# google-deepmind/meltingpot

Measured on AMD Instinct MI355X. Metric: agent-steps/sec (env_batch x players / wall s), clean_up @4096 worlds, higher is better.
Workload: dtype u8

## Files before the change

include/mp_engine.h:

```cpp
#ifndef MP_ENGINE_H_
#define MP_ENGINE_H_

#include <stdint.h>

#ifdef __cplusplus
extern "C" {
#endif
#pragma GCC visibility push(default)

#define MP_ABI_VERSION 8

enum {
  MP_OK = 0,
  MP_ERR_INVALID = -1,
  MP_ERR_PACK = -2,
  MP_ERR_NO_DEVICE = -3,
  MP_ERR_HIP = -4,
  MP_ERR_UNSUPPORTED = -5
};

typedef enum {
  MP_EVENT_ZAP = 1,
  MP_EVENT_EDIBLE_CONSUMED = 2,
  MP_EVENT_PLAYER_CLEANED = 3,
  MP_EVENT_CLAIMED_RESOURCE = 4,
  MP_EVENT_DESTROYED_RESOURCE = 5,
  MP_EVENT_SANCTIONING = 6,
  MP_EVENT_REMOVAL_DUE_TO_SANCTIONING = 7,
  MP_EVENT_SET_SANCTIONING_LEVEL = 8,
  MP_EVENT_AVATAR_STARTED = 9,
  MP_EVENT_COIN_CONSUMED = 10,
  MP_EVENT_INTERACTION = 11,
  MP_EVENT_COLLECTED_RESOURCE = 12,
  MP_EVENT_MINING = 13,
  MP_EVENT_EXTRACTION = 14,
  MP_EVENT_EXTRACTION_PAIR = 15,
  MP_EVENT_RECEIVER_ACCEPTED_ITEM = 17,
  MP_EVENT_ITEM_DROPPED_INTO_POT = 18,
  MP_EVENT_COOKED_FOOD_COLLECTED = 19,
  MP_EVENT_EATING_MUSHROOM = 20,
  MP_EVENT_GIFT = 16
} MpEventType;
#define MP_EVENT_ROWS 128

typedef enum {
  MP_OBS_RGB = 0,
  MP_OBS_WORLD_RGB = 1,
  MP_OBS_REWARD = 2,
  MP_OBS_READY_TO_SHOOT = 3,
  MP_OBS_AUX0 = 4,
  MP_OBS_STEP_TYPE = 5,
  MP_OBS_DISCOUNT = 6,
  MP_OBS_COLLECTIVE_REWARD = 7,
  MP_OBS_POSITION = 8,
  MP_OBS_ORIENTATION = 9,
  MP_OBS_EVENTS = 10,
  MP_OBS_AUX1 = 11,
  MP_OBS_AUX2 = 12,
  MP_OBS_AUX3 = 13,
  MP_OBS_AUX4 = 14,
  MP_OBS_ZAP_MATRIX = 15,
  MP_OBS_LAYER = 16,
  MP_OBS_INVENTORY = 17,
  MP_OBS_INTERACTION_INVENTORIES = 18,
  MP_OBS_MATRIX_CUMULANTS = 19,
  MP_OBS_INTERACTION_REWARDS = 20,
  MP_OBS_RGB_POOL2 = 21,
  MP_OBS_RGB_POOL4 = 22,
  MP_OBS_RGB_POOL8 = 23,
  MP_OBS_KINDS = 24
} MpObsKind;

typedef struct MpEngine MpEngine;

typedef struct {
  uint32_t struct_size;
  int32_t batch_worlds;
  int32_t waves;
  int32_t feeders;
  int32_t max_groups;
  int32_t scratch_cells;
  int32_t no_composite_cache;
  int32_t max_composites;
  int32_t verbose;
  int32_t late_feeder_prio;
  int32_t ring_batches;
  int32_t static_pct;
  int32_t world_waves;
  int32_t store_sc1;
  int32_t head;
  int32_t no_next_orders;
  int32_t record_pad;
  int32_t pace;
  int32_t team;
  int32_t generic_kernel;
} MpDevOptions;

typedef struct {
  uint32_t struct_size;
  int32_t device;
  int32_t num_worlds;
  int32_t auto_reset;
  uint64_t world_offset;
  uint64_t base_seed;
  void* stream;
  int32_t num_players;
  int32_t debug_observations;
  int32_t unfused;
  int32_t literal_base_seed;
  const MpDevOptions* dev;
  const int32_t* roles;
  int32_t world_pool;
} MpConfig;

typedef struct {
  int32_t abi_version;
  int32_t substrate;
  int32_t num_worlds, num_players, num_actions;
  int32_t map_h, map_w, num_layers, sprite_size;
  int32_t view_h, view_w;
  int32_t max_frames;
  int32_t world_state_bytes;
  int32_t fused;
  int32_t num_resources;
  int32_t num_action_fields;
  int32_t plan_batch_worlds, plan_ring_batches, plan_owned_batches, plan_pooled_batches,
          plan_groups, plan_store_sc1 ;
  int32_t plan_feeders, plan_waves;
  int32_t ring_slots, ring_next;
  int32_t plan_pace, visible_layers;
  int32_t plan_team, plan_late_priority;
  int64_t retired_va_bytes, retired_va_limit;
} MpInfo;

int mp_abi_version(void);

const char* mp_last_error(void);

int mp_create(const void* pack, uint64_t pack_len, const MpConfig* cfg,
              MpEngine** out);

void mp_destroy(MpEngine* eng);

int mp_info(const MpEngine* eng, MpInfo* out);

enum { MP_KERNEL_GENERIC = 0, MP_KERNEL_STOCK = 1 };
typedef struct {
  uint32_t struct_size;
  int32_t variant;
  const void* pack;
  uint64_t pack_len;
  const MpConfig* cfg;
  char* fields;
  uint64_t fields_cap;
} MpKernelVariant;

int mp_set_stream(MpEngine* eng, void* stream);

int mp_bind_output(MpEngine* eng, MpObsKind kind, void* device_ptr);

int mp_bind_output_ring(MpEngine* eng, MpObsKind kind, void* base,
                        uint64_t slot_stride_bytes, int32_t slots);

int mp_reset(MpEngine* eng, const uint64_t* seeds, const uint8_t* mask);

int mp_step(MpEngine* eng, const int32_t* actions_device);

int mp_step_host(MpEngine* eng, const int32_t* actions_host);

int mp_step_fields(MpEngine* eng, const int32_t* fields_device);

int mp_step_fields_host(MpEngine* eng, const int32_t* fields_host);

int mp_observe(MpEngine* eng, MpObsKind kind, void* dst_device);

uint64_t mp_obs_bytes(const MpEngine* eng, MpObsKind kind);

int mp_dump(MpEngine* eng, uint8_t* grid, int32_t* avat, int32_t* glob);

uint64_t mp_snapshot_bytes(const MpEngine* eng);
int mp_snapshot(MpEngine* eng, void* host_buf, uint64_t bytes);
int mp_restore(MpEngine* eng, const void* host_buf, uint64_t bytes);

enum { MP_STATES_FINGERPRINT = 1, MP_STATES_SAVE = 2, MP_STATES_LOAD = 3 };
typedef struct {
  uint32_t struct_size;
  int32_t op;
  uint64_t fingerprint;
  const int32_t* worlds;
  const int32_t* src;
  void* bank;
  uint64_t bank_bytes;
  int32_t count;
  int32_t bank_rows;
} MpWorldStates;

typedef struct {
  uint32_t struct_size;
  int32_t kind;
  uint64_t fingerprint;
  const void* bank;
  const int32_t* rows;
  void* dst;
  uint64_t dst_bytes;
  int32_t bank_rows;
  int32_t count;
  uint64_t reserved;
} MpStatesObserve;

typedef struct {
  char name[16];
  int32_t offset;
  int32_t elem_bytes;
  int32_t count;
  int32_t reserved;
} MpStateField;
typedef struct {
  uint32_t struct_size;
  uint32_t layout_version;
  const void* pack;
  uint64_t pack_len;
  const MpConfig* cfg;
  int32_t map_h, map_w, num_layers, num_players, num_states;
  int32_t grid_planes, grid_bytes, grid_pad, world_stride, tail_bytes;
  int32_t max_frames, avatar_layer, substrate, player_block;
  int32_t reserved[2];
  uint64_t fingerprint;
  MpStateField* fields;
  int32_t fields_cap;
  int32_t num_fields;
} MpStateLayout;

enum { MP_CHECK_ROWS = 1, MP_CHECK_HOST = 2, MP_CHECK_FILTER = 3 };
typedef struct {
  uint32_t struct_size;
  int32_t op;
  uint64_t fingerprint;
  const void* pack;
  uint64_t pack_len;
  const MpConfig* cfg;
  const void* bank;
  int32_t bank_rows;
  int32_t count;
  const int32_t* rows;
  void* out;
  uint64_t out_bytes;
  uint64_t reserved;
} MpStatesCheck;
// ... 77 lines not shown
```

meltingpot_amd/csrc/frame_kernel.h:

```cpp
#pragma once
#include <stdlib.h>
#include <string.h>

#include <type_traits>

#include "../../include/mp_pack.h"
#include "step_clean_up.h"
#include "step_coins.h"
#include "step_commons.h"
#include "step_coop.h"
#include "step_gift.h"
#include "step_mushroom.h"
#include "step_cook.h"
#include "step_matrix.h"
#include "step_territory.h"
#include "step_load.h"

template <bool kStep> constexpr bool nt_stores() { return kStep; }

namespace {

constexpr int kMaxLayers = 12;
constexpr int kSpriteStride = 272;
constexpr int kHeadBytes = 64;
// ... 560 lines not shown
          dst[ch] = (uint8_t)((sum[ch] + (uint32_t)(kPool * kPool / 2)) / (uint32_t)(kPool * kPool));
      }
      if (!arrive_and_wait(&ctrl->blob_waves, 2u * (uint32_t)n_render_waves)) return;
    } else if constexpr (kWPool != 0) {
      auto pool_atlas = [&](auto kp_tag, uint8_t* ptab) {
        constexpr int kP = decltype(kp_tag)::value;
        constexpr int kN = 8 / kP, kQ = kN * kN;
        const int items = t.n_images * kQ;
        for (int i = tid; i < items; i += n_render_waves * 64) {
          const int img = i / kQ, q = i - img * kQ, qy = q / kN, qx = q - qy * kN;
          const uint8_t* src = atlas + img * kSpriteStride + qy * kP * 32 + qx * kP * 3;
          uint32_t sum[3] = {0u, 0u, 0u};
#pragma unroll
          for (int y = 0; y < kP; ++y)
#pragma unroll
            for (int x = 0; x < kP * 3; ++x) sum[x % 3] += src[y * 32 + x];
          uint8_t* dst = ptab + img * pool_img_bytes(kP) + q * 3;
#pragma unroll
          for (int ch = 0; ch < 3; ++ch)
            dst[ch] = (uint8_t)((sum[ch] + (uint32_t)(kP * kP / 2)) / (uint32_t)(kP * kP));
        }
      };
      uint8_t* ptab = smem + lo.scratch + (uint32_t)kWaves * (uint32_t)pool_scratch_bytes<kPool, kWPool>(t);
      if constexpr (kPool != 0) pool_atlas(std::integral_constant<int, kPool>(), ptab);
      if constexpr (kWPool != 0 && kWPool != kPool)
        pool_atlas(std::integral_constant<int, kWPool>(), ptab + (kPool ? pool_tab_bytes(t, kPool) : 0));
      if (!arrive_and_wait(&ctrl->blob_waves, 2u * (uint32_t)n_render_waves)) return;
    }
  }
  FRAME_STAGE(3, npb);

  auto batch_first_world = [&](int k, bool& stalled) -> int {
    if (k < ks) {
      const int w0 = w_first + k * kstep;
      return w0 < w_end ? w0 : -1;
    }
    const int ring = k % kClaimRing, chain = k % A;
    uint64_t wait_t0 = 0;
    for (uint32_t polls = 0;; ++polls) {
      if (lds_acquire(&ctrl->claim_tag[ring]) == (uint32_t)(k + 1)) {
        const uint32_t w0 = ctrl->claim_w[ring];
        return w0 == kNoBatch ? -1 : (int)w0;
      }
      if (lds_acquire(&ctrl->chain_end[chain]) <= (uint32_t)k) return -1;
      if (waited_too_long(polls, wait_t0)) {
        report_stall(t, lane, FAULT_CLAIM, (uint32_t)wave, (uint32_t)k,
                     lds_acquire(&ctrl->claim_tag[ring]), (uint32_t)(k + 1));
        stalled = true;
        return -1;
      }
      __builtin_amdgcn_s_sleep(1);
    }
  };
  auto all_chains_ended = [&](int k) -> bool {
    uint32_t last = 0;
    for (int ch = 0; ch < A; ++ch) {
      const uint32_t e = lds_acquire(&ctrl->chain_end[ch]);
      last = e > last ? e : last;
    }
    return last <= (uint32_t)k;
  };

  const int role_wave = wave;
  if (role_wave >= kWaves - F) {
    const int f = wave - (kWaves - F);
    struct { int32_t B, NB, F, ks, N, nbt, A, pool_first, b_mod_f, wstride, pool, parity,
                     late_prio, records, step_tables, recs, w_first, kstep, w_end;
             uint32_t npb_all; } fc = {
        B, NB, F, ks, N, nbt, A, pool_first, kc.b_mod_f, wstride, plan.pool, plan.parity,
        plan.late_prio, lo.records, lo.step_tables, lo.recs, w_first, kstep, w_end, npb_all};
    pin_scalars(fc);
    auto batch_first_world = [&](int k, bool& stalled) -> int {
      if (k < fc.ks) {
        const int w0 = fc.w_first + k * fc.kstep;
        return w0 < fc.w_end ? w0 : -1;
      }
      const int ring = k % kClaimRing, chain = k % fc.A;
      uint64_t wait_t0 = 0;
      for (uint32_t polls = 0;; ++polls) {
        if (lds_acquire(&ctrl->claim_tag[ring]) == (uint32_t)(k + 1)) {
          const uint32_t w0 = ctrl->claim_w[ring];
          return w0 == kNoBatch ? -1 : (int)w0;
        }
        if (lds_acquire(&ctrl->chain_end[chain]) <= (uint32_t)k) return -1;
        if (waited_too_long(polls, wait_t0)) {
          report_stall(t, lane, FAULT_CLAIM, (uint32_t)wave, (uint32_t)k,
                       lds_acquire(&ctrl->claim_tag[ring]), (uint32_t)(k + 1));
          stalled = true;
          return -1;
        }
        __builtin_amdgcn_s_sleep(1);
      }
    };
    auto all_chains_ended = [&](int k) -> bool {
      uint32_t last = 0;
      for (int ch = 0; ch < fc.A; ++ch) {
        const uint32_t e = lds_acquire(&ctrl->chain_end[ch]);
        last = e > last ? e : last;
      }
      return last <= (uint32_t)k;
    };
    __builtin_amdgcn_s_setprio(3);
    uint8_t* my_scratch = smem + lo.step_scratch + f * plan.slot_scratch;
    FRAME_STAGE(10, 0);
    bool first_world = true;
    int kb = 0, gen = 0, r0 = 0, m = 0;
    auto next_batch = [&]() {
      ++kb; r0 += fc.B; m += fc.b_mod_f;
      if (m >= fc.F) m -= fc.F;
      if (kb == fc.NB) { kb = 0; r0 = 0; m = 0; ++gen; }
    };
    for (int k = 0;; ++k, next_batch()) {
      const int mine = f >= m ? f - m : f - m + fc.F;
      if (mine >= fc.B) continue;
      FRAME_STAGE(4, k);
      bool stalled = false;
      const int w0 = batch_first_world(k, stalled);
      if (stalled) return;
      if (w0 < 0) {
        if (all_chains_ended(k)) break;
        __builtin_amdgcn_s_sleep(8);
        continue;
      }
      int nw = fc.N - w0;
      if (nw > fc.B) nw = fc.B;
      uint64_t wait_t0 = 0;
      for (uint32_t polls = 0;
           gen > 0 && lds_acquire(&ctrl->done[kb]) < (uint32_t)gen * fc.npb_all; ++polls) {
        if (waited_too_long(polls, wait_t0)) {
          report_stall(t, lane, FAULT_BUFFER_FREE, (uint32_t)wave, (uint32_t)k,
                       lds_acquire(&ctrl->done[kb]), (uint32_t)gen * fc.npb_all);
          return;
        }
        __builtin_amdgcn_s_sleep(2);
      }
      for (int sl = mine; sl < fc.B; sl += fc.F) {
        FRAME_STAGE(5, sl);
        const bool claims = sl == 0 && k + fc.A >= fc.ks && fc.pool > 0;
        uint32_t claimed = 0;
        if (claims && lane == 0)
          claimed = __hip_atomic_fetch_add(&t.claim[fc.parity], 1u, __ATOMIC_RELAXED,
                                           __HIP_MEMORY_SCOPE_AGENT);
        const int w = w0 + sl;
        if (sl < nw) {
          uint8_t* rec = smem + fc.records + (r0 + sl) * fc.wstride;
          if constexpr (kStep) {
            int lane_w = lane;
            asm volatile("" : "+v"(lane_w));
            stepk::World wd = stepk::make_world(t, rec, smem + fc.step_tables, my_scratch,
                                                args.state, w, lane_w);
            wd.publish = &ctrl->slot_batch[r0 + sl];
            wd.publish_value = (uint32_t)(k + 1);
            wd.next_orders = args.next_orders;
            bool have_rec = false;
            if (head_pending) {
              head_pending = false;
              dma_wait();
              have_rec = w == pre_w && r0 + sl == pre_slot;
              if (!arrive_and_wait(&ctrl->table_waves, (uint32_t)fc.F)) return;
              FRAME_STAGE(11, sl);
            }
            int act_id;
            if (have_rec && args.mode == STEP_MODE_STEP)
              act_id = lane_w < P ? reinterpret_cast<const int*>(smem + fc.recs + wave * 64 * 16)[lane_w] : 0;
            else
              act_id = stepk::fetch_action_id(t, args.actions, args.mode, w, lane_w);
            if (!have_rec) stepk::load_record(t, rec, wd.gw, lane_w);
            FRAME_STAGE(12, sl);
            if (claims) {
              if (lane == 0) {
                const uint32_t id = (uint32_t)fc.pool_first + claimed;
                const int kn = k + fc.A, ring = kn % kClaimRing;
                const bool have = id < (uint32_t)fc.nbt;
                ctrl->claim_w[ring] = have ? id * (uint32_t)fc.B : kNoBatch;
                if (!have)
                  __hip_atomic_store(&ctrl->chain_end[kn % fc.A], (uint32_t)kn, __ATOMIC_RELEASE,
                                     __HIP_MEMORY_SCOPE_WORKGROUP);
                __hip_atomic_store(&ctrl->claim_tag[ring], (uint32_t)(kn + 1), __ATOMIC_RELEASE,
                                   __HIP_MEMORY_SCOPE_WORKGROUP);
              }
            }
            stepk::begin_step(wd.sc, lane_w);
            stepk::wsync();
            const stepk::Action act = stepk::lookup_action(t, wd, act_id, args.mode);
            stepk::step_or_load(t, c, sites, wd, act, args);
            if (args.out.layer) {
              stepk::wsync();
              stepk::write_layer(t, rec, args.out, w, lane_w);
            }
          } else {
            stepk::load_record(t, rec, args.state + (size_t)w * fc.wstride, lane);
          }
        }
        if (claims && (!kStep || sl >= nw)) {
          if (lane == 0) {
            const uint32_t id = (uint32_t)fc.pool_first + claimed;
            const int kn = k + fc.A, ring = kn % kClaimRing;
            const bool have = id < (uint32_t)fc.nbt;
            ctrl->claim_w[ring] = have ? id * (uint32_t)fc.B : kNoBatch;
            if (!have)
              __hip_atomic_store(&ctrl->chain_end[kn % fc.A], (uint32_t)kn, __ATOMIC_RELEASE,
                                 __HIP_MEMORY_SCOPE_WORKGROUP);
            __hip_atomic_store(&ctrl->claim_tag[ring], (uint32_t)(kn + 1), __ATOMIC_RELEASE,
                               __HIP_MEMORY_SCOPE_WORKGROUP);
          }
        }
        __builtin_amdgcn_fence(__ATOMIC_RELEASE, "workgroup");
        if (lane == 0)
          __hip_atomic_store(&ctrl->slot_batch[r0 + sl], (uint32_t)(k + 1), __ATOMIC_RELEASE,
                             __HIP_MEMORY_SCOPE_WORKGROUP);
        FRAME_STAGE(6, sl);
        if (first_world) {
          first_world = false;
          switch (fc.late_prio) {
            case 0: __builtin_amdgcn_s_setprio(0); break;
            case 1: __builtin_amdgcn_s_setprio(1); break;
            case 2: __builtin_amdgcn_s_setprio(2); break;
            default: break;
          }
        }
      }
    }
    FRAME_STAGE(15, 0);
    return;
  }

  uint8_t* __restrict__ out = wv ? out_w : out_a;
  CellRec* recs = reinterpret_cast<CellRec*>(smem + lo.recs) + wave * 64;
  uint8_t* ovlist = smem + lo.ovlist + wave * 64;
  int nsprites = t.nsprites;
  asm volatile("" : "+s"(nsprites));
  const uint32_t magic_rows = kv.magic_rows;
  const uint32_t magic_p = kc.magic_p;
  const uint32_t magic_spw = kv.magic_spw;
  const int py = lane & 7, sub = lane >> 3;
  uint8_t* atlas_row = atlas + py * 32;
  const uint32_t scratch_off =
      (kPool || kWPool) ? (uint32_t)(lo.scratch - lo.atlas) + (uint32_t)(wave * pool_scratch_bytes<kPool, kWPool>(t))
            : (uint32_t)(lo.scratch - lo.atlas) + (uint32_t)(wave * t.scratch_cells) * 256u;
  constexpr int kPN = kPool ? 8 / kPool : 1;
  constexpr int kWPN = kWPool ? 8 / kWPool : 1;
  const uint32_t vpn = (kWPool != 0 && wv) ? (uint32_t)kWPN : (uint32_t)kPN;
  const uint32_t prow = (uint32_t)row_cells * (vpn * 3u), pstrip = prow * vpn;
  const uint32_t my_poff = (uint32_t)sr * pstrip + cx * (vpn * 3u);
  const uint8_t* ptab = smem + lo.scratch + (uint32_t)kWaves * (uint32_t)pool_scratch_bytes<kPool, kWPool>(t) +
                        ((kWPool != 0 && wv && kWPool != kPool && kPool != 0) ? (uint32_t)pool_tab_bytes(t, kPool) : 0u);

  const uint32_t span_bytes = (uint32_t)R * 8u * row_bytes;
  const int n_iters = (int)((span_bytes + 1023u) >> 10);
  const int n_full = (int)(span_bytes >> 10);
  uint32_t keys[12];
#pragma unroll
  for (int it = 0; it < 12; ++it) {
    uint32_t kk = 0;
#pragma unroll
    for (int h = 0; h < 2; ++h) {
      const uint32_t pp = (uint32_t)(it * 64 + lane) * 16u + 8u * h;
      uint32_t key = 63u << 8;
      if (pp < span_bytes) {
        const uint32_t row = fast_div(pp, row_bytes, 1.0f / (float)row_bytes);
        const uint32_t colb = pp - row * row_bytes;
        const uint32_t ccx = fast_div(colb, 24u, 1.0f / 24.0f);
        key = (((row >> 3) * (uint32_t)row_cells + ccx) << 8) | ((row & 7u) * 32u + (colb - ccx * 24u));
      }
      kk |= key << (16 * h);
    }
    keys[it] = kk;
  }


  auto render_pass = [&](const uint32_t s0, const uint32_t nstrips, const uint8_t* wlds,
                         uint8_t* out_block) {
    uint8_t* const g0 = (kPool || kWPool) ? out_block + (size_t)s0 * pstrip : nullptr;
    uint8_t* const pst = (kPool || kWPool) ? atlas + scratch_off + ((uint32_t)(uintptr_t)g0 & 15u) : nullptr;
    int n_partial, n_ov;
    {
      const uint32_t strip = s0 + sr;
      const bool live = sr < R && strip < nstrips;
      const uint32_t sidx = live ? strip : 0u;
      const uint32_t img = magic_div(sidx, magic_rows);
      const uint32_t cy = sidx - img * strip_rows;
      uint32_t lw = img, viewer = P, vo = 0;
      if (!wv) {
        lw = magic_div(img, magic_p);
        viewer = img - lw * P;
      }
      const uint8_t* grid = wlds + lw * wstride;
      const uint8_t* head = grid + t.grid_pad;
      int cell;
      uint32_t oob_img = 0;
      if (wv) {
        cell = (int)(cy * W + cx);
      } else {
        const uint32_t alive = head[48 + viewer], ori = head[32 + viewer];
        const int hx = head[viewer], hy = head[16 + viewer];
        oob_img = oobimg[viewer];
        const bool on_grid = alive != 0u;
        vo = on_grid ? ori : 0u;
        const int dx = (int)cx - t.vl, dy = (int)cy - t.vf;
        const int ax = vo == 0u ? dx : vo == 1u ? -dy : vo == 2u ? -dx : dy;
        const int ay = vo == 0u ? dy : vo == 1u ? dx : vo == 2u ? -dy : -dx;
        int x = hx + ax, y = hy + ay;
        bool inside;
        if (t.topology == 1) {
          x += x < 0 ? W : 0; x -= x >= W ? W : 0;
          y += y < 0 ? H : 0; y -= y >= H ? H : 0;
          inside = true;
        } else {
          inside = x >= 0 && x < W && y >= 0 && y < H;
        }
        cell = on_grid && inside ? y * W + x : -1;
      }
      const uint16_t* rinfo_v = rinfo + viewer * (uint32_t)nsprites;
      CellRec r;
      r.base = 0; r.ov0 = 0; r.ov1 = 0; r.ov2 = 0;
      uint32_t base_img = 0;
      bool done = !live || cell < 0;
      if (cell == -1) base_img = oob_img;
      const uint16_t* tf = stab + (((0u - vo) & 3u) << 8);
      const uint8_t* gp = grid + (cell >= 0 ? cell : 0);
      uint32_t base_e = base_img;
      auto resolve = [&](auto nv_tag) {
        constexpr int NV = decltype(nv_tag)::value;
        uint32_t offs[6] = {kv.plane_off[0], kv.plane_off[1], kv.plane_off[2],
                            kv.plane_off[3], kv.plane_off[4], kv.plane_off[5]};
        uint32_t avp = kv.av_planes;
#pragma unroll
        for (int i = 0; i < (NV + 1) / 2; ++i) asm volatile("" : "+s"(offs[i]));
        asm volatile("" : "+s"(avp));
        uint32_t ent[NV];
        uint32_t seen = 0;
#pragma unroll
        for (int k = 0; k < NV; ++k) ent[k] = gp[(offs[k >> 1] >> (16 * (k & 1))) & 0xffffu];
#pragma unroll
        for (int k = 0; k < NV; ++k) { ent[k] = tf[ent[k]]; seen |= ent[k]; }
// ... 480 lines not shown
```

meltingpot_amd/csrc/mp_engine.hip:

```cpp
#include <chrono>
#include <map>
#include <mutex>
#include "../../include/mp_engine.h"

#include <stdarg.h>
#include <stddef.h>
#include <sys/types.h>
#include <stdio.h>
#include <string.h>

#include <algorithm>
#include <string>
#include <vector>

#include "pack_decode.h"
#include "stock.h"
#include "step_common.h"
#include "step_many.h"
#include "state_obs.h"
#include "state_check.h"

void launch_step(const DevTables& t, const SubstrateTables& s, const stepk::StepArgs& args,
                 hipStream_t stream);
int prepare_step();
void launch_layer_view(const DevTables& t, const uint8_t* state, int32_t* out, int num_worlds,
                       hipStream_t stream);

constexpr int kFaultWords = 64 + 4 * 16 * 64 * 2;
FramePlan plan_frame(const DevTables& t, const SubstrateTables& s, int num_worlds,
                     bool with_step, int views, int num_cus, const MpDevOptions* dev,
                     int pool_k = 1,
                     int world_k = 1);
int frame_lds_bytes(const DevTables& t, const FramePlan& p, int pool_k = 1, int world_k = 1,
                    int views = 2);
int render_blob_bytes(const DevTables& t);
int prepare_frame();
void build_render_blob(const DevTables& t, const uint8_t* images, const uint16_t* img_slot,
                       const uint32_t* pair_table, const int32_t* state_sprite,
                       const int8_t* state_player, const int32_t* view_sprite_map,
                       const uint8_t* sprite_flags8, const int32_t* state_orient,
                       uint8_t* blob);
uint32_t render_visible_layers(const DevTables& t, const uint8_t* blob, const int32_t* state_layer);
void launch_frame(const DevTables& t, const SubstrateTables* s, const stepk::StepArgs& args,
                  uint8_t* out_a, uint8_t* out_w, const FramePlan& p, hipStream_t stream,
                  int pool_k = 1, int world_k = 1);

thread_local std::string g_error;

int fail(int code, const char* fmt, ...) {
  char buf[512];
  va_list ap;
  va_start(ap, fmt);
  vsnprintf(buf, sizeof buf, fmt, ap);
  va_end(ap);
  g_error = buf;
  return code;
}

#define HIP_TRY(expr)                                                       \
  do {                                                                      \
    hipError_t e_ = (expr);                                                 \
    if (e_ != hipSuccess)                                                   \
      return fail(MP_ERR_HIP, "%s failed: %s", #expr, hipGetErrorString(e_)); \
  } while (0)

struct MpEngine {
  int device = 0;
  int N = 0;
  int auto_reset = 0;
  hipStream_t stream = nullptr;
  int substrate = 0;
  DevTables t{};
  SubstrateTables sub{};
  int inventory_types() const {
    return substrate == MPK_SUBSTRATE_THE_MATRIX ? sub.mx.R
           : substrate == MPK_SUBSTRATE_GIFT_REFINEMENTS ? sub.gr.ntypes : 0;
  }
  std::vector<uint8_t> pack;
  uint8_t* d_pack = nullptr;
  uint8_t* d_extra = nullptr;
  uint8_t* d_stepblob = nullptr;
  uint8_t* d_debug = nullptr;
  uint32_t* h_fault = nullptr;
  uint8_t* d_state = nullptr;
  uint8_t* d_scalars = nullptr;
  size_t scalars_bytes = 0, debug_bytes = 0;
  StepOutputs own{};
  void* bound[MP_OBS_KINDS] = {};
  struct RingKind { uint8_t* base = nullptr; uint64_t stride = 0; };
  RingKind ring[MP_OBS_KINDS];
  int ring_slots = 0;
  uint64_t ring_cursor = 0;
  bool ring_hold = false;
  bool layer_hold = false;
  std::vector<FramePlan> ring_plan[3];
  void point_ring(int slot, bool pixels_only = false) {
    for (int k = 0; k < MP_OBS_KINDS; ++k)
      if (ring[k].base && (!pixels_only || is_pixel_kind(k)))
        bound[k] = ring[k].base + (uint64_t)slot * ring[k].stride;
  }
  bool ring_has_pixels() const {
    for (int k = 0; k < MP_OBS_KINDS; ++k)
      if (ring[k].base && is_pixel_kind(k)) return true;
    return false;
  }
  static int pool_of(int kind) {
    return kind == MP_OBS_RGB_POOL2 ? 2 : kind == MP_OBS_RGB_POOL4 ? 4 : kind == MP_OBS_RGB_POOL8 ? 8 : 1;
  }
  static bool is_pixel_kind(int kind) {
    return kind == MP_OBS_RGB || kind == MP_OBS_WORLD_RGB || pool_of(kind) > 1;
  }
  int agent_kind() const {
    for (int k : {MP_OBS_RGB_POOL2, MP_OBS_RGB_POOL4, MP_OBS_RGB_POOL8})
      if (bound[k]) return k;
    return MP_OBS_RGB;
  }
  uint8_t* agent_view() const { return (uint8_t*)bound[agent_kind()]; }
  int pool_k() const { return pool_of(agent_kind()); }
  int world_pool = 1;
  FramePlan pool_plan[3][2][3] = {};
  bool pool_ok[3] = {};
  static int pool_index(int k) { return k == 2 ? 0 : k == 4 ? 1 : 2; }
  FramePlan& frame_plan(int stepping, int views, int k) {
    return k > 1 ? pool_plan[pool_index(k)][stepping][views] : plan[stepping][views];
  }
  int32_t* d_actions = nullptr;
  int32_t* d_fields = nullptr;
  uint8_t* d_mask = nullptr;
  uint64_t* d_seeds = nullptr;
  unsigned long long* d_ctr = nullptr;
  static constexpr int kHostSlots = 4;
  int32_t* h_actions[kHostSlots] = {};
  hipEvent_t h_copied[kHostSlots] = {};
  uint64_t host_steps = 0;
  FramePlan plan[2][3] = {};
  int frame_launches = 0;
  uint32_t* d_claim = nullptr;
  int num_cus = 0;
  int next_orders = 1;
  bool has_dev = false;
  bool touched = false;
  bool has_state = false;
  uint64_t fingerprint = 0;
  int unfused = 0;
  bool fuse(bool world_view) const {
    (void)world_view;
    return unfused != 1;
  }
  uint8_t* d_atlas = nullptr;
  uint8_t* d_obs_rows = nullptr;
  uint64_t obs_rows_bytes = 0;
  uint8_t* d_obs_stash = nullptr;
  uint64_t obs_stash_bytes = 0;
  int32_t* d_layer_lut = nullptr;
  state_check::CheckTables check = {};
  state_check::CheckTables* d_check = nullptr;
  StepOutputs outputs() const {
    StepOutputs o = own;
    if (bound[MP_OBS_REWARD]) o.reward = (double*)bound[MP_OBS_REWARD];
    if (bound[MP_OBS_READY_TO_SHOOT]) o.ready = (double*)bound[MP_OBS_READY_TO_SHOOT];
    if (bound[MP_OBS_AUX0]) o.aux0 = (double*)bound[MP_OBS_AUX0];
    if (bound[MP_OBS_STEP_TYPE]) o.step_type = (int32_t*)bound[MP_OBS_STEP_TYPE];
    if (bound[MP_OBS_DISCOUNT]) o.discount = (double*)bound[MP_OBS_DISCOUNT];
    if (bound[MP_OBS_COLLECTIVE_REWARD]) o.collective = (double*)bound[MP_OBS_COLLECTIVE_REWARD];
    if (bound[MP_OBS_POSITION]) o.position = (int32_t*)bound[MP_OBS_POSITION];
    if (bound[MP_OBS_ORIENTATION]) o.orientation = (int32_t*)bound[MP_OBS_ORIENTATION];
    if (bound[MP_OBS_EVENTS]) o.events = (int32_t*)bound[MP_OBS_EVENTS];
    for (int k = 0; k < 4; ++k)
      if (bound[MP_OBS_AUX1 + k]) o.dbg[k] = (double*)bound[MP_OBS_AUX1 + k];
    if (bound[MP_OBS_ZAP_MATRIX]) o.zap_matrix = (double*)bound[MP_OBS_ZAP_MATRIX];
    if (bound[MP_OBS_INVENTORY]) o.inventory = (double*)bound[MP_OBS_INVENTORY];
    if (bound[MP_OBS_INTERACTION_INVENTORIES])
      o.interaction = (double*)bound[MP_OBS_INTERACTION_INVENTORIES];
    if (bound[MP_OBS_MATRIX_CUMULANTS]) o.cumulants = (double*)bound[MP_OBS_MATRIX_CUMULANTS];
    if (bound[MP_OBS_INTERACTION_REWARDS])
      o.interaction_rewards = (double*)bound[MP_OBS_INTERACTION_REWARDS];
    if (bound[MP_OBS_LAYER] && !layer_hold) { o.layer = (int32_t*)bound[MP_OBS_LAYER]; o.layer_lut = d_layer_lut; }
    return o;
  }
};

namespace {

__global__ __launch_bounds__(1024) void k_box_fill(uint8_t* out, uint64_t bytes, uint64_t own,
                                                   uint32_t span, int order) {
  __shared__ uint32_t next;
  if (threadIdx.x == 0) next = 0;
  __syncthreads();
  const uint32_t lane = threadIdx.x & 63u;
  const uint64_t g = blockIdx.x, G = gridDim.x;
  typedef uint32_t u32x4 __attribute__((ext_vector_type(4)));
  for (;;) {
    uint32_t t = 0;
    if (lane == 0) t = atomicAdd(&next, 1u);
    t = (uint32_t)__builtin_amdgcn_readfirstlane((int)t);
    uint64_t begin, end;
    if (order == 0) {
      uint64_t lim = (g + 1) * own;
      if (lim > bytes) lim = bytes;
      begin = g * own + (uint64_t)t * span;
      if (begin >= lim) break;
      end = begin + span < lim ? begin + span : lim;
    } else {
      begin = ((uint64_t)t * G + g) * span;
      if (begin >= bytes) break;
      end = begin + span < bytes ? begin + span : bytes;
    }
    const uint64_t sp = reinterpret_cast<uint64_t>(out + begin);
    uint8_t* base = reinterpret_cast<uint8_t*>(
        ((uint64_t)(uint32_t)__builtin_amdgcn_readfirstlane((uint32_t)(sp >> 32)) << 32) |
        (uint64_t)(uint32_t)__builtin_amdgcn_readfirstlane((uint32_t)sp));
    const uint32_t n = (uint32_t)(end - begin);
    for (uint32_t off = lane * 16u; off < n; off += 1024u)
      asm volatile("global_store_dwordx4 %0, %1, %2 nt" :: "v"(off), "v"(u32x4{t, off, 2u, 3u}), "s"(base));
  }
}

__global__ void k_probe_actions(int32_t* actions, int n, int nact, uint32_t salt) {
  const int i = blockIdx.x * blockDim.x + threadIdx.x;
  if (i >= n) return;
  uint32_t x = (uint32_t)i * 2654435761u + salt;
  x ^= x >> 16; x *= 0x7feb352du; x ^= x >> 15; x *= 0x846ca68bu; x ^= x >> 16;
  actions[i] = (int32_t)(x % (uint32_t)nact);
}

__global__ void k_set_seeds(uint8_t* state, int stride, int grid_pad, int n,
                            const uint64_t* seeds, const uint8_t* mask) {
  const int w = blockIdx.x * blockDim.x + threadIdx.x;
  if (w >= n || (mask && !mask[w])) return;
  WorldTail* tail = reinterpret_cast<WorldTail*>(state + (size_t)w * stride + grid_pad);
  tail->seed = seeds[w];
  tail->episode = 0;
  tail->orders_step = 0;
}

__global__ void k_sum_counters(const uint8_t* state, int stride, int grid_pad, int n,
                               unsigned long long* out) {
  unsigned long long acc[MP_CTR_COUNT];
  for (int k = 0; k < MP_CTR_COUNT; ++k) acc[k] = 0;
  for (int w = blockIdx.x * blockDim.x + threadIdx.x; w < n; w += gridDim.x * blockDim.x) {
    const WorldTail* tail = reinterpret_cast<const WorldTail*>(state + (size_t)w * stride + grid_pad);
    for (int k = 0; k < MP_CTR_COUNT; ++k) acc[k] += tail->ctr[k];
    acc[MP_CTR_REWARD_SUM] += (unsigned long long)(long long)tail->reward_fx;
  }
  for (int k = 0; k < MP_CTR_COUNT; ++k) {
    for (int off = 32; off > 0; off >>= 1) acc[k] += __shfl_xor(acc[k], off);
    if ((threadIdx.x & 63) == 0 && acc[k]) atomicAdd(&out[k], acc[k]);
  }
}

__global__ __launch_bounds__(256) void k_save_worlds(DevTables t, const uint8_t* __restrict__ state, int n,
                                                     const int32_t* __restrict__ worlds, int count,
                                                     uint8_t* __restrict__ dst) {
  const int lane = threadIdx.x & 63;
  const int row = blockIdx.x * 4 + __builtin_amdgcn_readfirstlane((int)threadIdx.x >> 6);
  if (row >= count) return;
  const int w = worlds ? __builtin_amdgcn_readfirstlane(worlds[row]) : row;
  if (w < 0 || w >= n) {
    if (lane == 0) {
      t.fault[FAULT_STATE_INDEX + 1] = (uint32_t)w;
      t.fault[FAULT_STATE_INDEX + 2] = 2u;
      t.fault[FAULT_STATE_INDEX] = (uint32_t)row + 1u;
    }
    return;
  }
  const int nvec = t.world_stride >> 4;
  const uint4* src = reinterpret_cast<const uint4*>(state + (size_t)w * t.world_stride);
  uint4* out = reinterpret_cast<uint4*>(dst + (size_t)row * t.world_stride);
  for (int i0 = 0; i0 < nvec; i0 += 8 * 64) {
    uint4 v[8];
#pragma unroll
    for (int k = 0; k < 8; ++k) {
      const int i = i0 + k * 64 + lane;
      v[k] = src[i < nvec ? i : nvec - 1];
    }
#pragma unroll
    for (int k = 0; k < 8; ++k) stepk::issued(v[k]);
#pragma unroll
    for (int k = 0; k < 8; ++k) {
      const int i = i0 + k * 64 + lane;
      if (i < nvec) out[i] = v[k];
    }
  }
}

int sync_and_check(MpEngine* e, const char* who) {
  HIP_TRY(hipStreamSynchronize(e->stream));
  const volatile uint32_t* f = e->h_fault;
  if (f[0] != 0)
    return fail(MP_ERR_HIP,
                "%s: the frame kernel's pipeline stalled (site %u, workgroup %u, wave %u, batch %u, "
                "seen %u, wanted %u); its outputs are incomplete",
                who, f[0], f[1], f[2], f[3], f[4], f[5]);
  if (f[8] != 0) {
    const uint32_t world = f[8] - 1;
    e->h_fault[8] = 0;
    return fail(MP_ERR_HIP,
                "%s: world %u paid an interaction reward outside every resultIndicatorColorInterval "
                "(the reference asserts there, the_matrix/components.lua:282-290); the indicator "
                "shows the first colour", who, world);
  }
  if (f[kFaultCheckWorld] != 0) {
    const uint32_t world = f[kFaultCheckWorld] - 1, row = f[kFaultCheckWorld + 1], rule = f[kFaultCheckWorld + 2],
                   offset_word = f[kFaultCheckWorld + 3];
    e->h_fault[kFaultCheckWorld] = 0;
    if ((f[FAULT_STATE_INDEX + 2] & 255u) == kFaultCheckRefused) e->h_fault[FAULT_STATE_INDEX] = 0;
    return fail(MP_ERR_INVALID,
                "%s: checked MP_STATES_LOAD: row %d, which src[%u] names, is not a well-formed record "
                "(rule %u, offset word 0x%x); world %u was left as it was", who, (int)row, world, rule,
                offset_word, world);
  }
  if (f[FAULT_STATE_INDEX] != 0) {
    const uint32_t at = f[FAULT_STATE_INDEX] - 1, index = f[FAULT_STATE_INDEX + 1];
    const bool load = f[FAULT_STATE_INDEX + 2] == 1;
    const bool observe = f[FAULT_STATE_INDEX + 2] == kFaultObserveRow;
    const uint32_t what = f[FAULT_STATE_INDEX + 2];
    e->h_fault[FAULT_STATE_INDEX] = 0;
    if (what == kFaultCheckRow)
      return fail(MP_ERR_INVALID,
                  "%s: MpStatesCheck: rows[%u] = %d is not a row of the bank; element %u of out is (-1, %d)",
                  who, at, (int)index, at, (int)index);
    if (observe)
      return fail(MP_ERR_INVALID,
                  "%s: MpStatesObserve: rows[%u] = %d is not a row of the bank; element %u of the "
                  "destination was left as it was", who, at, (int)index, at);
    return load ? fail(MP_ERR_INVALID,
                       "%s: MP_STATES_LOAD: src[%u] = %d is neither -1 nor a row of the bank; world %u "
                       "was left as it was", who, at, (int)index, at)
                : fail(MP_ERR_INVALID,
                       "%s: MP_STATES_SAVE: worlds[%u] = %d is not a world of this engine; row %u was "
                       "left as it was", who, at, (int)index, at);
  }
  return MP_OK;
}

void draw(MpEngine* e, uint8_t* rgb, uint8_t* wrgb, int pool_k = 1) {
  stepk::StepArgs args = {};
  args.state = e->d_state; args.num_worlds = e->N;
  FramePlan p = e->frame_plan(0, rgb && wrgb ? 2 : wrgb ? 1 : 0, rgb ? pool_k : 1);
  p.parity = e->frame_launches++ & 1;
  launch_frame(e->t, nullptr, args, rgb, wrgb, p, e->stream, rgb ? pool_k : 1, e->world_pool);
}

int submit(MpEngine* e, int mode, const int32_t* actions, const uint8_t* mask,
           const uint8_t* bank = nullptr, const int32_t* src = nullptr, int bank_rows = 0,
           const StepManyLaunch* many = nullptr) {
  stepk::StepArgs args;
  args.state = e->d_state; args.actions = actions; args.reset_mask = mask;
  args.bank = bank; args.src = src; args.bank_rows = bank_rows;
  args.mode = mode; args.auto_reset = e->auto_reset; args.num_worlds = e->N;
  args.next_orders = e->next_orders;
  const bool ringing = e->ring_slots > 0 && !e->ring_hold;
  const int slot = e->ring_slots > 0 ? (int)(e->ring_cursor % (uint64_t)e->ring_slots) : 0;
  if (ringing) { e->point_ring(slot); ++e->ring_cursor; }
  args.out = e->outputs();
  uint8_t* rgb = e->agent_view();
  uint8_t* wrgb = (uint8_t*)e->bound[MP_OBS_WORLD_RGB];
  const int pk = rgb ? e->pool_k() : 1;
  const int views = rgb && wrgb ? 2 : wrgb ? 1 : 0;
  if (many || (!rgb && !wrgb) || !e->fuse(rgb == nullptr)) {
    if (many)
      launch_step_many(e->t, e->sub, args, *many, e->stream);
    else
      launch_step(e->t, e->sub, args, e->stream);
    if (rgb) draw(e, rgb, nullptr, pk);
    if (wrgb) draw(e, nullptr, wrgb);
  } else {
    FramePlan p = ringing && e->ring_plan[views].size() == (size_t)e->ring_slots
                      ? e->ring_plan[views][(size_t)slot] : e->frame_plan(1, views, pk);
    p.parity = e->frame_launches++ & 1;
    launch_frame(e->t, &e->sub, args, rgb, wrgb, p, e->stream, pk, e->world_pool);
  }
  HIP_TRY(hipGetLastError());
  return MP_OK;
}

void retired_va(int64_t* bytes, int64_t* limit);
bool in_mapped_view(const void* p);

int check_bank(MpEngine* e, const void* ptr, uint64_t bytes, const char* who);

int check_device_pointer(MpEngine* e, const void* ptr, const char* who) {
  if (in_mapped_view(ptr)) return MP_OK;
  hipPointerAttribute_t attr = {};
  const hipError_t rc = hipPointerGetAttributes(&attr, ptr);
  if (rc != hipSuccess) {
    (void)hipGetLastError();
    hipDeviceptr_t base = nullptr;
    size_t size = 0;
    if (hipMemGetAddressRange(&base, &size, (hipDeviceptr_t)ptr) == hipSuccess && base && size) return MP_OK;
    (void)hipGetLastError();
    return fail(MP_ERR_INVALID, "%s: %p is not memory the device can write (%s); bind a device buffer",
                who, ptr, hipGetErrorString(rc));
  }
  if (attr.type == hipMemoryTypeUnregistered)
    return fail(MP_ERR_INVALID, "%s: %p is plain host memory; bind a device buffer", who, ptr);
  if ((attr.type == hipMemoryTypeDevice || attr.type == hipMemoryTypeArray) && attr.device != e->device)
    return fail(MP_ERR_INVALID, "%s: %p lives on device %d, the engine on device %d", who, ptr,
                attr.device, e->device);
  return MP_OK;
}

int check_bank(MpEngine* e, const void* ptr, uint64_t bytes, const char* who) {
  if (int rc = check_device_pointer(e, ptr, who)) return rc;
  if (in_mapped_view(ptr)) {
    if (!in_mapped_view((const char*)ptr + bytes - 1))
      return fail(MP_ERR_INVALID, "%s: [%p, +%llu bytes) leaves the mapped view it starts in", who, ptr,
                  (unsigned long long)bytes);
    return MP_OK;
  }
  hipPointerAttribute_t attr = {};
  const hipError_t rc = hipPointerGetAttributes(&attr, ptr);
  (void)hipGetLastError();
  if (rc == hipSuccess && attr.type == hipMemoryTypeHost)
    return fail(MP_ERR_INVALID, "%s: %p is host memory; world states live in device memory", who, ptr);
  hipDeviceptr_t base = nullptr;
  size_t size = 0;
  if (hipMemGetAddressRange(&base, &size, (hipDeviceptr_t)ptr) != hipSuccess || !base) {
    (void)hipGetLastError();
    return fail(MP_ERR_INVALID, "%s: %p is not in a device allocation the runtime knows", who, ptr);
  }
  if ((uint64_t)((const char*)ptr - (const char*)base) + bytes > (uint64_t)size)
    return fail(MP_ERR_INVALID, "%s: [%p, +%llu bytes) runs past the end of its allocation (%p, %zu bytes)",
                who, ptr, (unsigned long long)bytes, base, size);
  return MP_OK;
}

int check_agent_view(MpEngine* e, int kind, const void* ptr, const char* who) {
  if (kind != MP_OBS_RGB && MpEngine::pool_of(kind) == 1) return MP_OK;
  for (int k : {MP_OBS_RGB, MP_OBS_RGB_POOL2, MP_OBS_RGB_POOL4, MP_OBS_RGB_POOL8})
    if (k != kind && e->bound[k])
      return fail(MP_ERR_INVALID, "%s: kind %d is bound; one per-agent view (MP_OBS_RGB or one "
                  "MP_OBS_RGB_POOL*) at a time — unbind it first", who, k);
  if (MpEngine::pool_of(kind) > 1 && ((uintptr_t)ptr & 15) != 0)
    return fail(MP_ERR_INVALID, "%s: a pooled view's buffer must be 16-byte aligned (%p)", who, ptr);
  return MP_OK;
}

int check_world_view(MpEngine* e, int kind, const void* ptr, const char* who) {
  if (kind == MP_OBS_WORLD_RGB && e->world_pool > 1 && ((uintptr_t)ptr & 15) != 0)
    return fail(MP_ERR_INVALID, "%s: a pooled WORLD.RGB buffer (MpConfig.world_pool = %d) must be "
                "16-byte aligned (%p)", who, e->world_pool, ptr);
  return MP_OK;
}

void drop_ring_kind(MpEngine* e, int kind) {
  if (!e->ring[kind].base) return;
  e->ring[kind] = MpEngine::RingKind();
  for (auto& v : e->ring_plan) v.clear();
  bool any = false;
  for (int k = 0; k < MP_OBS_KINDS; ++k) any = any || e->ring[k].base;
  if (!any) { e->ring_slots = 0; e->ring_cursor = 0; }
}

uint64_t state_fingerprint(const std::vector<uint8_t>& pack, const DevTables& t) {
  uint64_t h = 0xcbf29ce484222325ull;
  auto mix = [&](const void* p, size_t n) {
    for (size_t i = 0; i < n; ++i) { h ^= ((const uint8_t*)p)[i]; h *= 0x100000001b3ull; }
  };
  const uint32_t words[4] = {MP_RECORD_LAYOUT_VERSION, (uint32_t)t.P, (uint32_t)t.grid_pad,
                             (uint32_t)t.world_stride};
  mix(words, sizeof(words));
  const uint64_t n = pack.size();
  mix(&n, sizeof(n));
  mix(pack.data(), pack.size());
  return h;
}

#define DEV_ALLOC(ptr, bytes) HIP_TRY(hipMalloc((void**)&(ptr), (bytes)))

int upload_pack(MpEngine* e, const MpConfig& cfg, DecodedPack* d) {
  DEV_ALLOC(e->d_pack, e->pack.size());
  if (int rc = decode_pack(e->pack, cfg, e->d_pack, d)) return rc;
  HIP_TRY(hipMemcpy(e->d_pack, e->pack.data(), e->pack.size(), hipMemcpyHostToDevice));
  DEV_ALLOC(e->d_extra, d->extra.size());
  HIP_TRY(hipMemcpy(e->d_extra, d->extra.data(), d->extra.size(), hipMemcpyHostToDevice));
  DEV_ALLOC(e->d_stepblob, d->step_blob.size());
  HIP_TRY(hipMemcpy(e->d_stepblob, d->step_blob.data(), d->step_blob.size(), hipMemcpyHostToDevice));
  e->t = d->t;
  e->sub = d->sub;
  e->substrate = d->sub.substrate;
  e->t.sprite_flags8 = e->d_extra;
  e->t.step_blob = e->d_stepblob;
  return MP_OK;
}

int alloc_fault_words(MpEngine* e) {
  HIP_TRY(hipHostMalloc((void**)&e->h_fault, kFaultWords * sizeof(uint32_t), hipHostMallocMapped));
  memset(e->h_fault, 0, kFaultWords * sizeof(uint32_t));
  HIP_TRY(hipHostGetDevicePointer((void**)&e->t.fault, e->h_fault, 0));
  DEV_ALLOC(e->d_claim, (2 + 2 * 1024) * sizeof(uint32_t));
  HIP_TRY(hipMemset(e->d_claim, 0, (2 + 2 * 1024) * sizeof(uint32_t)));
  e->t.claim = e->d_claim;
  return MP_OK;
}

int init_state(MpEngine* e, const MpConfig& cfg) {
  const DevTables& t = e->t;
  const size_t state_bytes = (size_t)e->N * t.world_stride;
  DEV_ALLOC(e->d_state, state_bytes);
  std::vector<uint8_t> init(state_bytes, 0);
  for (int w = 0; w < e->N; ++w) {
    WorldTail* tail = reinterpret_cast<WorldTail*>(init.data() + (size_t)w * t.world_stride + t.grid_pad);
    const uint64_t gw = cfg.world_offset + (uint64_t)w;
// ... 212 lines not shown
  for (const Stack& sk : stacks)
    for (int f = 0; f < 4; ++f) {
      int base = sk.l[0].sprite < 0 ? 0 : a.slots[(size_t)sk.l[0].sprite * 4 + ((f + sk.l[0].orient) & 3)];
      for (int k = 1; k < sk.n; ++k) {
        const int ov = a.slots[(size_t)sk.l[k].sprite * 4 + ((f + sk.l[k].orient) & 3)];
        int comp = a.lookup((uint32_t)base, (uint32_t)ov);
        if (comp < 0) {
          if (k < sk.n - 1 || a.n_composites >= max_composites || a.used_slots >= kPairSlots / 2 ||
              a.count >= 1023)
            break;
          uint8_t img[256];
          a.blend(base, ov, (flags[sk.l[k].sprite] & MPK_SPRITE_PARTIAL) != 0, img);
          const int before = a.count;
          comp = a.add_image(img, 0);
          a.n_composites += a.count - before;
          a.insert((uint32_t)base, (uint32_t)ov, (uint32_t)comp);
          ++a.used_slots;
        }
        base = comp;
      }
    }
}

int build_atlas(MpEngine* e, const MpDevOptions* dev, const DecodedPack& d) {
  DevTables& t = e->t;
  const int32_t* flags = table<int32_t>(e->pack.data(), "sprite_flags");
  Atlas a;
  a.add_sprites(table<uint8_t>(e->pack.data(), "sprite_rgba"), flags, t.nsprites * 4);
  t.scratch_cells = (dev && dev->scratch_cells > 0) ? dev->scratch_cells : 8;
  if (!(dev && dev->no_composite_cache)) fill_composites(e, dev, flags, collect_stacks(e, flags), a);
  if (a.count > 1023) return fail(MP_ERR_PACK, "mp_create: %d distinct sprite images", a.count);
  t.n_images = a.count;
  t.pair_probe = a.pair_probe;
  const void* hp = e->pack.data();
  const int nimg = t.nsprites * 4;
  const size_t img_bytes = (size_t)a.count * 256, slot_bytes = ((size_t)nimg * 2 + 15) & ~(size_t)15,
               pair_bytes = (size_t)kPairSlots * 4, blob_bytes = (size_t)render_blob_bytes(t);
  std::vector<uint8_t> flags8((size_t)t.nsprites);
  for (int s = 0; s < t.nsprites; ++s)
    flags8[(size_t)s] = (uint8_t)(((flags[s] & MPK_SPRITE_OPAQUE) ? 1 : 0) |
                                  ((flags[s] & MPK_SPRITE_PARTIAL) ? 2 : 0) |
                                  ((flags[s] & MPK_SPRITE_EMPTY) ? 4 : 0));
  const int8_t* splayer = reinterpret_cast<const int8_t*>(d.extra.data() + 256);
  const int32_t* vmap = table<int32_t>(hp, "view_sprite_map");
  std::vector<int32_t> vmap_p((size_t)(t.P + 1) * t.nsprites);
  for (int v = 0; v <= t.P; ++v)
    memcpy(vmap_p.data() + (size_t)v * t.nsprites,
           vmap + (size_t)(v < t.P ? v : t.P_pack) * t.nsprites, (size_t)t.nsprites * 4);
  std::vector<uint8_t> buf(img_bytes + slot_bytes + pair_bytes + blob_bytes, 0);
  memcpy(buf.data(), a.images.data(), img_bytes);
  memcpy(buf.data() + img_bytes, a.slots.data(), (size_t)nimg * 2);
  memcpy(buf.data() + img_bytes + slot_bytes, a.pair_table.data(), pair_bytes);
  uint8_t* blob = buf.data() + img_bytes + slot_bytes + pair_bytes;
  build_render_blob(t, a.images.data(), a.slots.data(), a.pair_table.data(),
                    table<int32_t>(hp, "state_sprite"), splayer, vmap_p.data(), flags8.data(),
                    table<int32_t>(hp, "state_orient"), blob);
  t.vis_layers = render_visible_layers(t, blob, table<int32_t>(hp, "state_layer"));
  HIP_TRY(hipMalloc((void**)&e->d_atlas, buf.size()));
  HIP_TRY(hipMemcpy(e->d_atlas, buf.data(), buf.size(), hipMemcpyHostToDevice));
  t.atlas_compact = e->d_atlas;
  t.img_slot = reinterpret_cast<const uint16_t*>(e->d_atlas + img_bytes);
  t.pair_table = reinterpret_cast<const uint32_t*>(e->d_atlas + img_bytes + slot_bytes);
  t.render_blob = e->d_atlas + img_bytes + slot_bytes + pair_bytes;
  if (dev && dev->verbose)
    fprintf(stderr, "mp_engine: composite cache: %d images, %d table entries, probe %d\n",
            a.n_composites, a.used_slots, a.pair_probe);
  return MP_OK;
}

int upload_layer_lut(MpEngine* e) {
  const DevTables& t = e->t;
  const void* hp = e->pack.data();
  const int32_t* ssprite = table<int32_t>(hp, "state_sprite");
  const int32_t* vmap = table<int32_t>(hp, "view_sprite_map");
  std::vector<int32_t> lut((size_t)t.P * kLayerLutRow, 0);
  for (int p = 0; p < t.P; ++p) {
    const int32_t* remap = vmap + (size_t)p * t.nsprites;
    int32_t* row = lut.data() + (size_t)p * kLayerLutRow;
    for (int s = 1; s < t.nstates && s < 256; ++s)
      row[s] = ssprite[s] >= 0 ? 1 + remap[ssprite[s]] : 0;
    row[256] = 1 + remap[0];
  }
  HIP_TRY(hipMalloc((void**)&e->d_layer_lut, lut.size() * 4));
  HIP_TRY(hipMemcpy(e->d_layer_lut, lut.data(), lut.size() * 4, hipMemcpyHostToDevice));
  return MP_OK;
}

uint64_t pack_hash(const std::vector<uint8_t>& pack) {
  uint64_t h = 0xcbf29ce484222325ull;
  for (uint8_t b : pack) { h ^= b; h *= 0x100000001b3ull; }
  return h;
}

int select_kernels(const std::vector<uint8_t>& pack, const DecodedPack& d, const MpDevOptions* dev) {
  if (dev && dev->generic_kernel) return MP_KERNEL_GENERIC;
  if (d.sub.substrate == MPK_SUBSTRATE_CLEAN_UP && pack_hash(pack) == MP_STOCK_CLEAN_UP_PACK_HASH &&
      StockCleanUp::matches(d.t, d.sub.cu))
    return MP_KERNEL_STOCK;
  return MP_KERNEL_GENERIC;
}

int plan_views(MpEngine* e, const MpDevOptions* dev) {
  const DevTables& t = e->t;
  for (int v = 0; v < 6; ++v) {
    FramePlan& pl = e->plan[v & 1][v >> 1];
    pl = plan_frame(t, e->sub, e->N, (v & 1) != 0, v >> 1, e->num_cus, dev);
    if (frame_lds_bytes(t, pl) > 160 * 1024)
      return fail(MP_ERR_PACK, "mp_create: renderer needs %d B of LDS", frame_lds_bytes(t, pl));
  }
  if (e->world_pool > 1)
    for (int v = 2; v < 6; ++v) {
      FramePlan& pl = e->plan[v & 1][v >> 1];
      pl = plan_frame(t, e->sub, e->N, (v & 1) != 0, v >> 1, e->num_cus, dev, 1, e->world_pool);
      const int need = frame_lds_bytes(t, pl, 1, e->world_pool, v >> 1);
      if (need > 160 * 1024)
        return fail(MP_ERR_UNSUPPORTED, "mp_create: WORLD.RGB pooled by %d (MpConfig.world_pool) needs "
                    "%d B of LDS", e->world_pool, need);
    }
  for (int i = 0; i < 3; ++i) {
    const int k = 2 << i;
    e->pool_ok[i] = t.sprite_size == 8;
    for (int v = 0; v < 6 && e->pool_ok[i]; ++v) {
      if ((v >> 1) == 1) continue;
      FramePlan& pl = e->pool_plan[i][v & 1][v >> 1];
      pl = plan_frame(t, e->sub, e->N, (v & 1) != 0, v >> 1, e->num_cus, dev, k, e->world_pool);
      if (frame_lds_bytes(t, pl, k, e->world_pool, v >> 1) > 160 * 1024) e->pool_ok[i] = false;
    }
  }
  if (step_worlds_per_group(t, e->sub) < 1)
    return fail(MP_ERR_PACK, "mp_create: the step kernels need %d B of LDS", step_lds_bytes(t, e->sub, 1));
  if (int rc = prepare_frame())
    return fail(MP_ERR_HIP, "mp_create: hipFuncSetAttribute(max dynamic LDS) failed: %d", rc);
  if (int rc = prepare_step())
    return fail(MP_ERR_HIP, "mp_create: hipFuncSetAttribute(max dynamic LDS) of the step kernels failed: %d", rc);
  if (int rc = prepare_step_many())
    return fail(MP_ERR_HIP, "mp_create: hipFuncSetAttribute(max dynamic LDS) of the K-step kernels failed: %d", rc);
  if (dev && dev->verbose)
    for (int v = 0; v < 6; ++v) {
      const FramePlan& pl = e->plan[v & 1][v >> 1];
      fprintf(stderr, "mp_engine: %d sprite images; frame plan %s, %s: %d buffers x %d worlds, %d of %d waves feed"
              " (%d draw the world view), %d groups own %d batches each + %d pooled, %d B LDS\n",
              t.n_images, (v & 1) ? "stepping + drawing" : "drawing",
              (v >> 1) == 0 ? "agents view" : (v >> 1) == 1 ? "world view" : "both views",
              pl.NB, pl.B, pl.feeders, pl.nwaves, pl.world_waves, pl.groups, pl.ks, pl.pool,
              frame_lds_bytes(t, pl, 1, e->world_pool, v >> 1));
    }
  return MP_OK;
}

int create_on_device(MpEngine* e, const MpConfig& cfg, DecodedPack* d) {
  const MpDevOptions* dev = cfg.dev;
  e->has_dev = dev != nullptr;
  e->next_orders = !(dev && dev->no_next_orders);
  e->device = cfg.device;
  e->N = cfg.num_worlds;
  e->auto_reset = cfg.auto_reset;
  e->stream = (hipStream_t)cfg.stream;
  e->unfused = cfg.unfused;
  e->world_pool = cfg.world_pool > 1 ? cfg.world_pool : 1;
  int cus = 0;
  if (hipDeviceGetAttribute(&cus, hipDeviceAttributeMultiprocessorCount, cfg.device) != hipSuccess ||
      cus <= 0)
    return fail(MP_ERR_NO_DEVICE, "mp_create: device %d does not report its compute units", cfg.device);
  e->num_cus = cus;
  int rc;
  if ((rc = upload_pack(e, cfg, d))) return rc;
  e->sub.stock = select_kernels(e->pack, *d, dev);
  if ((rc = alloc_fault_words(e)) || (rc = init_state(e, cfg)) ||
      (rc = alloc_outputs(e, cfg)) || (rc = build_atlas(e, dev, *d)) || (rc = upload_layer_lut(e)))
    return rc;
  return plan_views(e, dev);
}

int upload_check_tables(MpEngine* e) {
  HIP_TRY(hipMalloc((void**)&e->d_check, sizeof(state_check::CheckTables)));
  HIP_TRY(hipMemcpy(e->d_check, &e->check, sizeof(state_check::CheckTables), hipMemcpyHostToDevice));
  return MP_OK;
}

struct HostStage {
  MpConfig cfg = {};
  MpDevOptions dev = {};
  std::vector<uint8_t> pack;
  DecodedPack d;
};

int host_stage(const void* pack, uint64_t pack_len, const MpConfig* cfg, HostStage* h) {
  if (!cfg || (cfg->struct_size != sizeof(MpConfig) && cfg->struct_size != offsetof(MpConfig, world_pool)))
    return fail(MP_ERR_INVALID, "mp_create: bad MpConfig (struct_size)");
  memcpy(&h->cfg, cfg, cfg->struct_size);
  if (cfg->struct_size < sizeof(MpConfig)) h->cfg.world_pool = 1;
  cfg = &h->cfg;
  if (cfg->dev) {
    if (cfg->dev->struct_size != sizeof(MpDevOptions) &&
        cfg->dev->struct_size != offsetof(MpDevOptions, generic_kernel))
      return fail(MP_ERR_INVALID, "mp_create: bad MpDevOptions (struct_size)");
    memcpy(&h->dev, cfg->dev, cfg->dev->struct_size);
    h->dev.struct_size = sizeof(MpDevOptions);
    h->cfg.dev = &h->dev;
  }
  if (cfg->num_worlds <= 0)
    return fail(MP_ERR_INVALID, "mp_create: num_worlds must be positive");
  if (cfg->unfused < 0 || cfg->unfused > 2)
    return fail(MP_ERR_INVALID, "mp_create: MpConfig.unfused must be 0, 1 or 2 (got %d)", cfg->unfused);
  if (cfg->world_pool != 0 && cfg->world_pool != 1 && cfg->world_pool != 2 && cfg->world_pool != 4 &&
      cfg->world_pool != 8)
    return fail(MP_ERR_INVALID, "mp_create: MpConfig.world_pool must be 0, 1, 2, 4 or 8 (got %d)",
                cfg->world_pool);
  const int32_t* hdr = nullptr;
  if (int rc = check_header(pack, pack_len, *cfg, &hdr)) return rc;
  h->pack.assign((const uint8_t*)pack, (const uint8_t*)pack + pack_len);
  if (int rc = apply_roles(h->pack, *cfg)) return rc;
  if (int rc = decode_pack(h->pack, *cfg, h->pack.data(), &h->d)) return rc;
  if (cfg->world_pool > 1 && h->d.t.sprite_size != 8)
    return fail(MP_ERR_UNSUPPORTED, "mp_create: MpConfig.world_pool needs 8 x 8 sprites (the pack's are %d x %d)",
                h->d.t.sprite_size, h->d.t.sprite_size);
  return MP_OK;
}

void literal(std::string* out, int32_t v) { *out += std::to_string(v); }
void literal(std::string* out, uint32_t v) { *out += std::to_string(v) + "u"; }
void literal(std::string* out, uint64_t v) {
  char b[32];
  snprintf(b, sizeof b, "0x%llxull", (unsigned long long)v);
  *out += b;
}
void literal(std::string* out, double v) {
  char b[48];
  snprintf(b, sizeof b, "%a", v);
  *out += b;
}

}

extern "C" {

int mp_abi_version(void) { return MP_ABI_VERSION; }

const char* mp_last_error(void) { return g_error.c_str(); }

uint64_t mp_obs_bytes(const MpEngine* e, MpObsKind kind) {
  if (!e) return 0;
  const uint64_t N = (uint64_t)e->N, P = (uint64_t)e->t.P, S = (uint64_t)e->t.sprite_size;
  switch (kind) {
    case MP_OBS_RGB:
      return N * P * (e->t.vf + e->t.vb + 1) * S * (e->t.vl + e->t.vr + 1) * S * 3;
    case MP_OBS_WORLD_RGB: {
      const uint64_t k = (uint64_t)e->world_pool;
      return N * (e->t.H * S / k) * (e->t.W * S / k) * 3;
    }
    case MP_OBS_RGB_POOL2: case MP_OBS_RGB_POOL4: case MP_OBS_RGB_POOL8: {
      const uint64_t k = (uint64_t)MpEngine::pool_of(kind);
      if (!e->pool_ok[MpEngine::pool_index((int)k)]) return 0;
      return N * P * ((e->t.vf + e->t.vb + 1) * S / k) * ((e->t.vl + e->t.vr + 1) * S / k) * 3;
    }
    case MP_OBS_REWARD: case MP_OBS_READY_TO_SHOOT: case MP_OBS_AUX0: return N * P * 8;
    case MP_OBS_STEP_TYPE: return N * 4;
    case MP_OBS_DISCOUNT: case MP_OBS_COLLECTIVE_REWARD: return N * 8;
    case MP_OBS_POSITION: return N * P * 8;
    case MP_OBS_ORIENTATION: return N * P * 4;
    case MP_OBS_EVENTS: return N * MP_EVENT_ROWS * 16;
    case MP_OBS_AUX1: case MP_OBS_AUX2: case MP_OBS_AUX3: case MP_OBS_AUX4:
      return e->substrate == MPK_SUBSTRATE_CLEAN_UP ? N * P * 8 : 0;
    case MP_OBS_ZAP_MATRIX:
      return (e->substrate == MPK_SUBSTRATE_CLEAN_UP ||
              e->substrate == MPK_SUBSTRATE_COMMONS_HARVEST) ? N * P * P * 8 : 0;
    case MP_OBS_LAYER:
      return N * P * (e->t.vf + e->t.vb + 1) * (e->t.vl + e->t.vr + 1) * e->t.L * 4;
    case MP_OBS_INVENTORY:
      return N * P * e->inventory_types() * 8;
    case MP_OBS_INTERACTION_INVENTORIES:
      return e->substrate == MPK_SUBSTRATE_THE_MATRIX ? N * P * 2 * e->sub.mx.R * 8 : 0;
    case MP_OBS_MATRIX_CUMULANTS:
      return e->substrate == MPK_SUBSTRATE_THE_MATRIX ? N * P * (1 + 3 * e->sub.mx.R) * 8 : 0;
    case MP_OBS_INTERACTION_REWARDS:
      return e->substrate == MPK_SUBSTRATE_THE_MATRIX ? N * P * 2 * 8 : 0;
    default: return 0;
  }
}

int mp_create(const void* pack, uint64_t pack_len, const MpConfig* cfg,
              MpEngine** out) {
  if (!out) return fail(MP_ERR_INVALID, "mp_create: out is NULL");
  *out = nullptr;
  HostStage h;
  if (int rc = host_stage(pack, pack_len, cfg, &h)) return rc;
  cfg = &h.cfg;
  std::vector<uint8_t>& copy = h.pack;
  DecodedPack& d = h.d;

  int ndev = 0;
  if (hipGetDeviceCount(&ndev) != hipSuccess || ndev <= 0)
    return fail(MP_ERR_NO_DEVICE,
                "mp_create: no HIP device; the engine has no CPU path");
  if (cfg->device < 0 || cfg->device >= ndev)
    return fail(MP_ERR_INVALID, "mp_create: device %d out of range (%d devices)",
                cfg->device, ndev);
  HIP_TRY(hipSetDevice(cfg->device));

  MpEngine* e = new MpEngine();
  build_check_tables(d, &e->check);
  e->pack = std::move(copy);
  int rc = create_on_device(e, *cfg, &d);
  if (rc == MP_OK) rc = upload_check_tables(e);
  if (rc != MP_OK) {
    mp_destroy(e);
    return rc;
  }
  e->fingerprint = state_fingerprint(e->pack, e->t);
  *out = e;
  return MP_OK;
}

void mp_destroy(MpEngine* e) {
  if (!e) return;
  (void)hipSetDevice(e->device);
  (void)hipStreamSynchronize(e->stream);
  if (e->h_fault) (void)hipHostFree(e->h_fault);
  void* bufs[] = {e->d_pack, e->d_extra, e->d_stepblob, e->d_debug, e->d_state, e->d_scalars,
                  e->d_actions, e->d_fields, e->d_mask, e->d_seeds, e->d_atlas, e->d_ctr, e->d_claim,
                  e->d_layer_lut, e->d_obs_rows, e->d_obs_stash, e->d_check};
  for (void* b : bufs)
    if (b) (void)hipFree(b);
  for (int i = 0; i < MpEngine::kHostSlots; ++i)
    if (e->h_actions[i]) { (void)hipHostFree(e->h_actions[i]); (void)hipEventDestroy(e->h_copied[i]); }
  delete e;
}

int mp_info(const MpEngine* e, MpInfo* out) {
  if (!e || !out) return fail(MP_ERR_INVALID, "mp_info: NULL argument");
  memset(out, 0, sizeof *out);
  out->abi_version = MP_ABI_VERSION;
  out->substrate = e->substrate;
  out->num_worlds = e->N; out->num_players = e->t.P; out->num_actions = e->t.nact;
  out->map_h = e->t.H; out->map_w = e->t.W; out->num_layers = e->t.L;
  out->sprite_size = e->t.sprite_size;
  out->view_h = e->t.vf + e->t.vb + 1; out->view_w = e->t.vl + e->t.vr + 1;
  out->max_frames = e->t.max_frames;
  out->world_state_bytes = e->t.world_stride;
  out->fused = e->fuse(!e->agent_view() && e->bound[MP_OBS_WORLD_RGB]) ? 1 : 0;
  out->num_resources = e->inventory_types();
  out->num_action_fields = e->t.nfields;
  {
    const bool a = e->agent_view() != nullptr, w = e->bound[MP_OBS_WORLD_RGB] != nullptr;
    const int views = a && w ? 2 : w ? 1 : 0;
    const FramePlan& p = e->ring_slots > 0 && e->ring_plan[views].size() == (size_t)e->ring_slots
                             ? e->ring_plan[views][(size_t)(e->ring_cursor % (uint64_t)e->ring_slots)]
// ... 1433 lines not shown
```

meltingpot_amd/csrc/step_clean_up.h:

```cpp
#ifndef MP_STEP_CLEAN_UP_H_
#define MP_STEP_CLEAN_UP_H_

#include "step_common.h"

#ifdef MP_STEP_TIMING
#include <stdio.h>
#define TSTAMP(i) ts_[i] = __builtin_readcyclecounter()
#else
#define TSTAMP(i)
#endif

namespace stepk {

constexpr int kSiteRegs = 4;

struct CleanUpSites { int apple[kSiteRegs], dirt[kSiteRegs], water[kSiteRegs]; };

__device__ inline CleanUpSites load_sites(const CleanUpTables& c, int lane) {
  CleanUpSites s;
#pragma unroll
  for (int k = 0; k < kSiteRegs; ++k) {
    const int i = k * 64 + lane;
    s.apple[k] = i < c.n_apple ? c.apple_cells[i] : -1;
    s.dirt[k] = i < c.n_dirt ? c.dirt_cells[i] : -1;
    s.water[k] = i < c.n_water ? c.water_cells[i] : -1;
  }
  return s;
}

__device__ inline void step_world(const DevTables& t, const CleanUpTables& c,
                                  const CleanUpSites& sites, const World& wd, const Action& act,
                                  const StepArgs& args) {
  const int lane = wd.lane, w = wd.w;
  const StepOutputs& out = args.out;
#ifdef MP_STEP_TIMING
  unsigned long long ts_[12] = {0};
#endif
  TSTAMP(0);
  Scratch* sc = wd.sc;
  uint8_t* mark = wd.mark;
  uint8_t* grid = wd.rec;
  WorldTail* tail = reinterpret_cast<WorldTail*>(wd.rec + t.grid_pad);
  const int P = t.P, HW = t.H * t.W, W = t.W;
  const bool is_av = lane < P;
  auto at = [&](int layer, int cell) -> uint8_t& { return grid[layer * HW + cell]; };

  const OrderStreams kOrders = {RS_SHUFFLE_MOVE, RS_SHUFFLE_ZAP, RS_SHUFFLE_RESPAWN, 0, 3};

  const int what = dispatch(t, tail, lane, w, args.reset_mask, args.mode, args.auto_reset, out);
  if (what == 0) return;
  TSTAMP(1);

  Av a;
  double aux0 = 0.0;
  double dbg_cleaned = 0.0, dbg_ate = 0.0, dbg_zapped = 0.0, dbg_others_ate = 0.0;
  int step_type;
  const int alive_state = is_av ? t.alive_state[lane] : 0;
  double* zmat = out.zap_matrix ? out.zap_matrix + (size_t)w * P * P : nullptr;
  if (zmat) for (int i = lane; i < P * P; i += 64) zmat[i] = 0.0;

  if (what == 1) {
    const uint32_t k0 = (uint32_t)tail->seed, k1 = (uint32_t)(tail->seed >> 32);
    const uint32_t ep = tail->episode;
    wsync();
    const int gvec = t.grid_pad >> 4;
    for (int i = lane; i < gvec; i += 64)
      reinterpret_cast<uint4*>(grid)[i] = reinterpret_cast<const uint4*>(t.init_grid)[i];
    if (lane == 0) {
      tail->episode = ep + 1;
      tail->step = 0; tail->frame = 1; tail->done = 0; tail->cont = 1;
      tail->started = 1;
      tail->aux_count = c.n_dirt_init;
      tail->group_change = 0;
      tail->ctr[2]++;
    }
    if (lane < MP_MAX_PLAYERS) { tail->flag0[lane] = 0; tail->flag1[lane] = 0; }
    wsync();
    apply_map_choices(t, grid, lane, ep, k0, k1);
    spawn_avatars(t, grid, lane, ep, k0, k1, a);
    if (is_av) push_event(sc, MP_EVENT_AVATAR_STARTED, 0, 0);
#pragma unroll
    for (int q = 0; q < kSiteRegs; ++q) {
      if (sites.water[q] < 0) continue;
      const uint32_t k = philox_bounded(
          philox4x32_10((uint32_t)(q * 64 + lane), RS_ANIM_START, 0u, ep, k0, k1), 4u);
      at(c.water_layer, sites.water[q]) = (uint8_t)(c.s_water_packed >> (8u * k));
    }
    step_type = 0;
  } else {
    const uint32_t k0 = (uint32_t)tail->seed, k1 = (uint32_t)(tail->seed >> 32);
    const uint32_t ep = tail->episode - 1;
    const int step = tail->step + 1, frame = tail->frame;
    const int dirt_count0 = tail->aux_count;
    const uint64_t apple_thr = c.apple_thr[dirt_count0];
    int flag0 = 0, flag1 = 0;
    load_avatars(tail, lane, a);
    if (lane < MP_MAX_PLAYERS) { flag0 = tail->flag0[lane]; flag1 = tail->flag1[lane]; }
    wsync();
    auto draw = [&](int stream, uint32_t index) {
      return philox4x32_10(index, (uint32_t)stream, (uint32_t)step, ep, k0, k1);
    };
    const int a_move = act.move, a_turn = act.turn, a_zap = act.fire0, a_clean = act.fire1,
              bad = act.bad;
    clear_bytes(grid, c.zap.layer * HW, HW, lane);
    clear_bytes(grid, c.clean_layer * HW, HW, lane);
    TSTAMP(2);

    if (step > c.dirt_delay) {
      const Philox4 d = draw(RS_DIRT_SPAWN, 0);
      if (philox_u53(d) < c.thr_dirt_spawn) {
        unsigned long long m[kSiteRegs];
        int n = 0;
#pragma unroll
        for (int q = 0; q < kSiteRegs; ++q) {
          m[q] = __ballot(sites.dirt[q] >= 0 &&
                          at(c.dirt_wait_layer, sites.dirt[q] >= 0 ? sites.dirt[q] : 0) == c.s_dirt_wait);
          n += __popcll(m[q]);
        }
        if (n > 0) {
          const int k = (int)philox_bounded(d, (uint32_t)n);
          const int site = kth_site(m[0], m[1], m[2], m[3], k);
          const int q = site >> 6;
          const int cell = rdlane(q == 0 ? sites.dirt[0] : q == 1 ? sites.dirt[1]
                                  : q == 2 ? sites.dirt[2] : sites.dirt[3], site & 63);
          if (lane == 0 && at(c.dirt_layer, cell) == 0) {
            at(c.dirt_wait_layer, cell) = 0;
            at(c.dirt_layer, cell) = (uint8_t)c.s_dirt;
          }
        }
      }
    }
    TSTAMP(3);
    if (apple_thr != 0) {
#pragma unroll
      for (int q = 0; q < kSiteRegs; ++q) {
        const int cell = sites.apple[q];
        if (cell < 0) continue;
        if (philox_u53(draw(RS_APPLE_GROW, (uint32_t)(q * 64 + lane))) < apple_thr)
          if (at(c.apple_layer, cell) == 0) at(c.apple_layer, cell) = (uint8_t)c.s_apple;
      }
    }

    TSTAMP(4);
    int orders[4];
    step_orders(tail, lane, P, kOrders, (uint32_t)step, ep, k0, k1, orders);
    const int order_move = orders[0], order_zap = orders[1], order_resp = orders[2];
    bool fire_zap = false, fire_clean = false, want_respawn = false;
    if (is_av) {
      if (a.alive && c.zap.cooldown >= 0) {
        if (a.ztimer > 0) a.ztimer--;
        else if (a_zap == 1) { a.ztimer = c.zap.cooldown; fire_zap = true; }
      }
      if (a.alive && c.clean_cooldown >= 0) {
        if (a.ctimer > 0) a.ctimer--;
        else if (a_clean == 1) { a.ctimer = c.clean_cooldown; fire_clean = true; }
      }
      want_respawn = !a.alive && (frame - a.achange) >= c.zap.respawn_frames;
    }
    const bool water_advance = (frame - tail->group_change) >= c.anim_frames;
    int cont = tail->cont;
    if (frame >= c.ee_min_frames && (step + 1) % c.ee_interval == 0)
      if (philox_u53(draw(RS_EPISODE_END, 0)) < c.thr_episode_end) cont = 0;
    {
      const int total = __popcll(__ballot(is_av && flag0 != 0));
      aux0 = (double)(total - (flag0 != 0 ? 1 : 0));
      const int total_ate = __popcll(__ballot(is_av && flag1 != 0));
      dbg_others_ate = (double)(total_ate - (flag1 != 0 ? 1 : 0));
    }
    int cleaned = 0, ate = 0;

    TSTAMP(5);
    const bool wants = resolve_moves(t, wd, a, a_move, a_turn, order_move, alive_state);
    int ate_cell = -1;
    if (wants && at(c.apple_layer, a.y * W + a.x) == c.s_apple) {
      a.reward += c.eat_reward; ate = 1; ate_cell = a.y * W + a.x;
      push_event(sc, MP_EVENT_EDIBLE_CONSUMED, lane + 1, 0);
    }
    wsync();

    TSTAMP(6);
    int nzapped = 0, ncleaned = 0;
    fire_beams(t, wd, tail, a, fire_zap, beam_lane(c.zap.shape, lane), c.zap.hit, true,
               c.zap.layer, c.zap.s_hit, c.zap.remove_hit != 0,
               [](int, int) { return 0; },
               [](int, int, int, bool, int, bool) {}, -1, zmat, &nzapped);
    zap_rewards(t, sc, lane, a, fire_zap, order_zap, c.zap.shape.n, c.zap.penalty,
                c.zap.reward);
    TSTAMP(7);
    const BeamLane clean_lane = beam_lane(c.clean_shape, lane);
    fire_beams(t, wd, tail, a, fire_clean, clean_lane, c.clean_hit, false,
               c.clean_layer, c.s_clean_hit, false,
               [&](int s, int) { return s == c.s_dirt ? 3 : 0; },
               [&](int b0, int per, int nc, bool reached, int cell, bool dhit) {
                 (void)reached;
                 if (dhit) {
                   mark[cell] = 1;
                   push_event(sc, MP_EVENT_PLAYER_CLEANED, b0 + clean_lane.bl + 1, 0);
                 }
                 const unsigned long long db = __ballot(dhit);
                 if (db == 0) return;
                 if (lane == 0) tail->ctr[5] += __popcll(db);
                 if (lane >= b0 && lane < b0 + per && lane < P) {
                   const int n = __popcll((db >> ((lane - b0) * nc)) & ((1ull << nc) - 1ull));
                   ncleaned += n;
                   if (n) cleaned = 1;
                 }
               });

    TSTAMP(8);
    const int rcell = resolve_respawns(t, wd, tail, a, want_respawn, order_resp, alive_state,
                                       (uint32_t)step, frame, ep, k0, k1);
    if (rcell >= 0 && at(c.apple_layer, rcell) == c.s_apple) {
      a.reward += c.eat_reward; ate = 1; ate_cell = rcell;
      push_event(sc, MP_EVENT_EDIBLE_CONSUMED, lane + 1, 0);
    }
    if (water_advance) {
#pragma unroll
      for (int q = 0; q < kSiteRegs; ++q) {
        const int cell = sites.water[q];
        if (cell < 0) continue;
        const uint32_t s = at(c.water_layer, cell);
        uint32_t k = 0;
#pragma unroll
        for (uint32_t f = 1; f < 4; ++f) if (s == ((c.s_water_packed >> (8u * f)) & 255u)) k = f;
        at(c.water_layer, cell) = (uint8_t)(c.s_water_packed >> (8u * ((k + 1u) & 3u)));
      }
    }
    wsync();

    TSTAMP(9);
    if (ate_cell >= 0) at(c.apple_layer, ate_cell) = 0;
    apply_zapped(t, wd, a, rcell >= 0, frame);
    wsync();
    int dirt_count = 0;
    {
#pragma unroll
      for (int q = 0; q < kSiteRegs; ++q) {
        if (q * 64 >= c.n_dirt) break;
        bool dirty = false;
        const int cell = sites.dirt[q];
        if (cell >= 0) {
          if (mark[cell]) {
            mark[cell] = 0;
            if (at(c.dirt_layer, cell) == c.s_dirt && at(c.dirt_wait_layer, cell) == 0) {
              at(c.dirt_layer, cell) = 0;
              at(c.dirt_wait_layer, cell) = (uint8_t)c.s_dirt_wait;
            }
          }
          dirty = at(c.dirt_layer, cell) == c.s_dirt;
        }
        dirt_count += __popcll(__ballot(dirty));
      }
    }
    const unsigned long long badb = __ballot(bad != 0);
    const int done = !(cont && step < t.max_frames);
    if (lane == 0) {
      tail->step = step;
      tail->frame = frame + 1;
      tail->cont = cont;
      tail->done = done;
      tail->aux_count = dirt_count;
      if (water_advance) tail->group_change = frame;
      tail->ctr[0]++; tail->ctr[1] += (uint32_t)P; tail->ctr[7] += __popcll(badb);
    }
    if (lane < MP_MAX_PLAYERS) { tail->flag0[lane] = (uint8_t)cleaned; tail->flag1[lane] = (uint8_t)ate; }
    step_type = done ? 2 : 1;
    dbg_cleaned = (double)ncleaned; dbg_ate = (double)ate; dbg_zapped = (double)nzapped;
  }

  TSTAMP(10);
  if (is_av) {
    const size_t o = (size_t)w * P + lane;
    if (out.dbg[0]) out.dbg[0][o] = dbg_cleaned;
    if (out.dbg[1]) out.dbg[1][o] = dbg_ate;
    if (out.dbg[2]) out.dbg[2][o] = dbg_zapped;
    if (out.dbg[3]) out.dbg[3][o] = dbg_others_ate;
  }
  finish(t, wd, tail, a, aux0, c.zap.cooldown, step_type, out, kOrders);
  TSTAMP(11);
#ifdef MP_STEP_TIMING
  if (lane == 0 && (w == 7 || w == 2000) && what == 2)
    printf("w %d: dispatch %llu clear %llu dirt %llu apple %llu upd %llu moves %llu zap %llu clean %llu resp %llu flush2 %llu finish %llu total %llu\n",
           w, ts_[1] - ts_[0], ts_[2] - ts_[1], ts_[3] - ts_[2], ts_[4] - ts_[3], ts_[5] - ts_[4],
           ts_[6] - ts_[5], ts_[7] - ts_[6], ts_[8] - ts_[7], ts_[9] - ts_[8], ts_[10] - ts_[9],
           ts_[11] - ts_[10], ts_[11] - ts_[0]);
#endif
}

}

#endif
```

meltingpot_amd/csrc/step_common.h:

```cpp
#ifndef MP_STEP_COMMON_H_
#define MP_STEP_COMMON_H_

#include "mp_common.h"

namespace stepk {


__device__ inline void wsync() {
  __builtin_amdgcn_fence(__ATOMIC_RELEASE, "workgroup");
  __builtin_amdgcn_wave_barrier();
  __builtin_amdgcn_fence(__ATOMIC_ACQUIRE, "workgroup");
}

__device__ inline int rdlane(int v, int l) { return __builtin_amdgcn_readlane(v, l); }
__device__ inline double rdlane(double v, int l) {
  const unsigned long long u = (unsigned long long)__double_as_longlong(v);
  const unsigned lo = (unsigned)__builtin_amdgcn_readlane((int)(unsigned)u, l);
  const unsigned hi = (unsigned)__builtin_amdgcn_readlane((int)(unsigned)(u >> 32), l);
  return __longlong_as_double((long long)(((unsigned long long)hi << 32) | lo));
}

__device__ inline int dir_dx(int o) { return (o == 1) - (o == 3); }
__device__ inline int dir_dy(int o) { return (o == 2) - (o == 0); }

struct BeamLane { int nc, lat, fw; uint32_t pred; int per, bl, j; };
__device__ inline BeamLane beam_lane(const BeamShape& shape, int lane) {
  BeamLane r;
  r.nc = shape.n; r.per = shape.per;
  r.bl = (int)(((uint32_t)lane * shape.magic) >> 16);
  const int j = lane - r.bl * r.nc;
  r.j = j;
  uint32_t v = 0;
#pragma unroll
  for (int q = 0; q < 16; ++q) v |= shape.cell[q] & (0u - (uint32_t)(j == q));
  r.lat = (int)(int8_t)(v & 255u); r.fw = (int)(int8_t)((v >> 8) & 255u); r.pred = v >> 16;
  return r;
}

constexpr int kSinfoBytes = 256 * 4;
__host__ __device__ inline int spawn_bytes(int n_spawn) { return (n_spawn * 2 + 15) & ~15; }
__host__ __device__ inline int tables_bytes(const DevTables& t) {
  return kSinfoBytes + spawn_bytes(t.n_spawn) + ((t.nact * 4 + 15) & ~15);
}

struct Scratch {
  int8_t victim[MP_MAX_PLAYERS][16];
  uint32_t zapped_mask;
  uint32_t ev_count;
  uint32_t ev[MP_EVENT_ROWS - 1];
  uint32_t flags[2];
  uint32_t pad[1];
};
static_assert(sizeof(Scratch) % 16 == 0, "Scratch keeps mark[] 16-byte aligned");

__host__ __device__ inline int mark_bytes(const DevTables& t) { return (t.H * t.W + 15) & ~15; }
__host__ __device__ inline int scratch_bytes(const DevTables& t) {
  return (int)sizeof(Scratch) + mark_bytes(t);
}
struct World {
  uint8_t* rec;
  const uint32_t* sinfo;
  const uint16_t* spawn;
  const int8_t* action_rows;
  Scratch* sc;
  uint8_t* mark;
  uint8_t* extra;
  uint8_t* gw;
  int w, lane;
  uint32_t* publish;
  uint32_t publish_value;
  int next_orders;
};

__device__ inline World make_world(const DevTables& t, uint8_t* rec, const uint8_t* tables,
                                   uint8_t* scratch, uint8_t* state, int w, int lane) {
  World wd;
  wd.rec = rec;
  wd.sinfo = reinterpret_cast<const uint32_t*>(tables);
  wd.spawn = reinterpret_cast<const uint16_t*>(tables + kSinfoBytes);
  wd.action_rows = reinterpret_cast<const int8_t*>(tables + kSinfoBytes + spawn_bytes(t.n_spawn));
  wd.sc = reinterpret_cast<Scratch*>(scratch);
  wd.mark = scratch + sizeof(Scratch);
  wd.extra = wd.mark + mark_bytes(t);
  wd.gw = state + (size_t)w * t.world_stride;
  wd.w = w; wd.lane = lane;
  wd.publish = nullptr; wd.publish_value = 0; wd.next_orders = 0;
  return wd;
}

__device__ inline void push_event(Scratch* sc, int type, int a, int b) {
  const uint32_t i = atomicAdd(&sc->ev_count, 1u);
  if (i < MP_EVENT_ROWS - 1) sc->ev[i] = ((uint32_t)type << 16) | ((uint32_t)a << 8) | (uint32_t)b;
}

struct Av {
  int x = 0, y = 0, ori = 0, alive = 0, ztimer = 0, ctimer = 0, achange = 0;
  double reward = 0.0;
};

__device__ inline bool step_cell(const DevTables& t, int& x, int& y, int dx, int dy) {
  x += dx; y += dy;
  if (t.topology == 1) {
    x = ((x % t.W) + t.W) % t.W; y = ((y % t.H) + t.H) % t.H;
    return true;
  }
  return x >= 0 && x < t.W && y >= 0 && y < t.H;
}

__device__ inline int kth_site(unsigned long long m0, unsigned long long m1,
                               unsigned long long m2, unsigned long long m3, int k) {
  int base = 0;
  unsigned long long m = m0;
  int pc = __popcll(m0);
  if (k >= pc) { k -= pc; m = m1; base = 64; pc = __popcll(m1);
    if (k >= pc) { k -= pc; m = m2; base = 128; pc = __popcll(m2);
      if (k >= pc) { k -= pc; m = m3; base = 192; } } }
  for (int i = 0; i < k; ++i) m &= m - 1;
  return base + __ffsll((long long)m) - 1;
}

struct Action { int move = 0, turn = 0, fire0 = 0, fire1 = 0, bad = 0; };
constexpr int kFieldsTag = 0x40000000;
__device__ inline int fetch_action_id(const DevTables& t, const int32_t* actions, int mode,
                                      int w, int lane) {
  if ((mode & 1) || lane >= t.P) return 0;
  if (mode == STEP_MODE_FIELDS) {
    const int32_t* f = actions + ((size_t)w * t.P + lane) * t.nfields;
    int v[4];
#pragma unroll
    for (int a = 0; a < 4; ++a) v[a] = a < t.nfields ? f[a] : 0;
    uint32_t row = 0;
    bool ok = true;
#pragma unroll
    for (int a = 0; a < 4; ++a) {
      const int lo = (int)(int8_t)(t.field_lo >> (8 * a)), hi = (int)(int8_t)(t.field_hi >> (8 * a));
      ok = ok && (a >= t.nfields || (v[a] >= lo && v[a] <= hi));
      row |= ((uint32_t)v[a] & 255u) << (8 * a);
    }
    return ok ? (int)(row & 0x3fffffffu) | kFieldsTag : -1;
  }
  return actions[(size_t)w * t.P + lane];
}
__device__ inline Action lookup_action(const DevTables& t, const World& wd, int act, int mode) {
  Action r;
  if ((mode & 1) || wd.lane >= t.P) return r;
  uint32_t row;
  if (mode == STEP_MODE_FIELDS) {
    if (act < 0) { r.bad = 1; return r; }
    row = (uint32_t)act & 0x3fffffffu;
  } else {
    if (act < 0 || act >= t.nact) { act = 0; r.bad = 1; }
    row = *reinterpret_cast<const uint32_t*>(wd.action_rows + 4 * act);
  }
  r.move = (int)(int8_t)(row & 255u); r.turn = (int)(int8_t)((row >> 8) & 255u);
  r.fire0 = (int)(int8_t)((row >> 16) & 255u); r.fire1 = (int)(int8_t)(row >> 24);
  return r;
}

__device__ inline void shuffled_orders(int lane, int P, int s0, int s1, int s2, int s3, int n,
                                       uint32_t step, uint32_t ep, uint32_t k0, uint32_t k1,
                                       int (&out)[4]) {
  const int g = lane >> 4, pos = lane & 15;
  const int stream = g == 0 ? s0 : g == 1 ? s1 : g == 2 ? s2 : s3;
  int j = pos;
  if (g < n && pos + 1 < P)
    j = pos + (int)philox_bounded(
        philox4x32_10((uint32_t)pos, (uint32_t)stream, step, ep, k0, k1), (uint32_t)(P - pos));
  unsigned long long perm = 0xFEDCBA9876543210ull;
  const int row = lane & 48;
  int ji = __shfl(j, row);
  for (int i = 0; i + 1 < P; ++i) {
    const int jn = __shfl(j, row | ((i + 1) & 15));
    const unsigned long long x = ((perm >> (4 * i)) ^ (perm >> (4 * ji))) & 15ull;
    perm ^= (x << (4 * i)) | (x << (4 * ji));
    ji = jn;
  }
  const int mine = (int)((perm >> (4 * pos)) & 15ull);
#pragma unroll
  for (int q = 0; q < 4; ++q) out[q] = __shfl(mine, 16 * q + pos);
}

struct OrderStreams { int s0, s1, s2, s3, n; };

__device__ inline void step_orders(const WorldTail* tail, int lane, int P, const OrderStreams& os,
                                   uint32_t step, uint32_t ep, uint32_t k0, uint32_t k1,
                                   int (&out)[4]) {
  if (step != 0u && __builtin_amdgcn_readfirstlane((int)tail->orders_step) == (int)step) {
    const uint32_t v = tail->next_orders[lane & 15];
#pragma unroll
    for (int q = 0; q < 4; ++q) out[q] = (int)((v >> (4 * q)) & 15u);
    return;
  }
  shuffled_orders(lane, P, os.s0, os.s1, os.s2, os.s3, os.n, step, ep, k0, k1, out);
}

__device__ inline void issued(uint4& v) {
  asm volatile("" : "+v"(v.x), "+v"(v.y), "+v"(v.z), "+v"(v.w));
}

__device__ inline void load_record(const DevTables& t, uint8_t* rec, const uint8_t* gw, int lane) {
  const int nvec = t.world_stride >> 4;
  const uint4* src = reinterpret_cast<const uint4*>(gw);
  uint4* dst = reinterpret_cast<uint4*>(rec);
  for (int i0 = 0; i0 < nvec; i0 += 8 * 64) {
    uint4 v[8];
#pragma unroll
    for (int k = 0; k < 8; ++k) {
      const int i = i0 + k * 64 + lane;
      v[k] = src[i < nvec ? i : nvec - 1];
    }
#pragma unroll
    for (int k = 0; k < 8; ++k) issued(v[k]);
#pragma unroll
    for (int k = 0; k < 8; ++k) {
      const int i = i0 + k * 64 + lane;
      if (i < nvec) dst[i] = v[k];
    }
  }
}

__device__ inline void load_tables(const DevTables& t, uint8_t* tables, int tid, int nthreads) {
  const int nvec = tables_bytes(t) >> 4;
  for (int i = tid; i < nvec; i += 2 * nthreads) {
    uint4 a = reinterpret_cast<const uint4*>(t.step_blob)[i];
    uint4 b = reinterpret_cast<const uint4*>(t.step_blob)[min(i + nthreads, nvec - 1)];
    issued(a); issued(b);
    reinterpret_cast<uint4*>(tables)[i] = a;
    if (i + nthreads < nvec) reinterpret_cast<uint4*>(tables)[i + nthreads] = b;
  }
}

__device__ inline void clear_marks(const DevTables& t, uint8_t* mark, int lane) {
  const int nvec = mark_bytes(t) >> 4;
  for (int i = lane; i < nvec; i += 64) reinterpret_cast<uint4*>(mark)[i] = uint4{0, 0, 0, 0};
}

__device__ inline void begin_step(Scratch* sc, int lane) {
  if (lane == 0) { sc->ev_count = 0; sc->zapped_mask = 0; sc->flags[0] = 0; sc->flags[1] = 0; }
}

__device__ inline void clear_bytes(uint8_t* rec, int off, int n, int lane) {
  if (((off | n) & 1) == 0) {
    for (int i = 2 * lane; i < n; i += 128) *reinterpret_cast<uint16_t*>(rec + off + i) = 0;
  } else {
    for (int i = lane; i < n; i += 64) rec[off + i] = 0;
  }
}

__device__ inline void load_avatars(const WorldTail* tail, int lane, Av& a) {
  if (lane < MP_MAX_PLAYERS) {
    a.x = tail->ax[lane]; a.y = tail->ay[lane]; a.ori = tail->aori[lane];
    a.alive = tail->aalive[lane]; a.ztimer = tail->ztimer[lane];
    a.ctimer = tail->ctimer[lane]; a.achange = tail->achange[lane];
  }
}

__device__ inline void apply_map_choices(const DevTables& t, uint8_t* grid, int lane,
                                         uint32_t ep, uint32_t k0, uint32_t k1) {
  const int HW = t.H * t.W;
  for (int i = lane; i < t.n_optional; i += 64) {
    const int4 o = reinterpret_cast<const int4*>(t.optional)[i];
    grid[(o.y & 255) * HW + o.x] = 0;
  }
  wsync();
  for (int i = lane; i < t.n_optional; i += 64) {
    const int4 o = reinterpret_cast<const int4*>(t.optional)[i];
    const int cid = o.z & 0xffff, base = o.z >> 16;
    int n = t.choice_n[cid];
    uint32_t epw = ep;
    if (n < 0) { n = -n; epw = 0xffffffffu; }
    const int k = (int)philox_bounded(
        philox4x32_10((uint32_t)cid, RS_MAP_CHOICE, 0u, epw, k0, k1), (uint32_t)n) - base;
    if (k >= 0 && k < 32 && ((o.w >> k) & 1)) grid[(o.y & 255) * HW + o.x] = (uint8_t)(o.y >> 8);
  }
  wsync();
}

__device__ inline void spawn_avatars(const DevTables& t, uint8_t* grid, int lane,
                                     uint32_t ep, uint32_t k0, uint32_t k1, Av& a,
                                     int alive_state = -1) {
  const int P = t.P, HW = t.H * t.W;
  const bool is_av = lane < P;
  const int my_group = is_av ? t.avatar_init_group[lane] : -1;
  int my_cell = 0;
  for (int g = 0; g < t.n_init_groups; ++g) {
    const int base = t.init_spawn_ptr[g];
    int ns = t.init_spawn_ptr[g + 1] - base;
    const unsigned long long members = __ballot(my_group == g);
    const int want = __popcll(members);
    int item = lane < ns ? t.init_spawn_cells[base + lane] : 0;
    int item_hi = 64 + lane < ns ? t.init_spawn_cells[base + 64 + lane] : 0;
    if (t.optional_spawn) {
      bool present = false;
      if (lane < ns)
        for (int l = 0; l < t.L; ++l) {
          const int s = grid[l * HW + item];
          if (s != 0 && (t.state_groups[s] & t.init_spawn_mask[g]) != 0) present = true;
        }
      const unsigned long long pm = __ballot(present);
      const int dst = __popcll(pm & ((1ull << lane) - 1ull));
      int packed = 0;
      for (int i = 0; i < ns; ++i) {
        const int ci = __shfl(item, i), di = __shfl(dst, i);
        if (((pm >> i) & 1ull) && lane == di) packed = ci;
      }
      item = packed;
      ns = __popcll(pm);
    }
    int j = lane;
    if (lane < want && lane < ns)
      j = lane + (int)philox_bounded(
          philox4x32_10((uint32_t)(lane + 256 * g), RS_START_SPAWN, 0u, ep, k0, k1),
          (uint32_t)(ns - lane));
    for (int i = 0; i < want; ++i) {
      const int ji = __shfl(j, i);
      const int vi = __shfl(item, i);
      const int vj = ji < 64 ? __shfl(item, ji) : __shfl(item_hi, ji - 64);
      if (ji == i) continue;
      if (lane == i) item = vj;
      if (ji < 64) { if (lane == ji) item = vi; }
      else if (lane == ji - 64) item_hi = vi;
    }
    const int rank = __popcll(members & ((1ull << lane) - 1ull));
    const int got = __shfl(item, my_group == g ? rank : 0);
    if (my_group == g) my_cell = got;
  }
  a = Av();
  if (is_av) {
    a.ori = (int)philox_bounded(
        philox4x32_10((uint32_t)lane, RS_START_ORIENT, 0u, ep, k0, k1), 4u);
    a.x = my_cell % t.W; a.y = my_cell / t.W; a.alive = 1;
    grid[t.avatar_layer * HW + my_cell] =
        (uint8_t)(alive_state >= 0 ? alive_state : t.alive_state[lane]);
  }
}

__device__ inline bool resolve_moves(const DevTables& t, const World& wd, Av& a, int a_move,
                                     int a_turn, int order_move, int alive_state,
                                     int follow_layer = -1, bool has_follower = true) {
  uint8_t* grid = wd.rec;
  const int lane = wd.lane;
  const int P = t.P, HW = t.H * t.W, W = t.W;
  const bool is_av = lane < P;
  if (is_av && a_turn != 0) a.ori = (a.ori + a_turn + 4) & 3;
  const bool wants = is_av && a.alive && a_move != 0;
  int tx = a.x, ty = a.y;
  bool target_free = false;
  wsync();
  if (wants) {
    const int dir = (a.ori + a_move - 1) & 3;
    if (step_cell(t, tx, ty, dir_dx(dir), dir_dy(dir))) {
      const int s = grid[t.avatar_layer * HW + ty * W + tx];
      target_free = s == 0 || (wd.sinfo[s] >> 24) != 0;
      if (follow_layer >= 0 && has_follower && s == 0 && grid[follow_layer * HW + ty * W + tx] != 0)
        target_free = false;
    }
  }
  const int old_cell = a.y * W + a.x;
  bool moved = false;
  const int try_move = (int)(wants && target_free);
  if (__ballot(try_move != 0) != 0) {
    for (int r = 0; r < P; ++r) {
      const int p = rdlane(order_move, r);
      if (rdlane(try_move, p) == 0) continue;
      const int ptx = rdlane(tx, p), pty = rdlane(ty, p);
      const bool occupied = __ballot(is_av && a.alive && a.x == ptx && a.y == pty) != 0;
      if (lane == p && !occupied) { a.x = ptx; a.y = pty; moved = true; }
    }
  }
  int follower = 0;
  const bool follows = moved && follow_layer >= 0 && has_follower;
  if (follows) follower = grid[follow_layer * HW + old_cell];
  if (moved) {
    grid[t.avatar_layer * HW + old_cell] = 0;
    if (follows) grid[follow_layer * HW + old_cell] = 0;
  }
  wsync();
  if (moved) {
    grid[t.avatar_layer * HW + a.y * W + a.x] = (uint8_t)alive_state;
    if (follows) grid[follow_layer * HW + a.y * W + a.x] = (uint8_t)follower;
  }
  wsync();
  return wants;
}

template <class ExtraBlock, class OnCells>
__device__ inline void fire_beams(const DevTables& t, const World& wd, WorldTail* tail,
                                  const Av& a, bool fire, const BeamLane& shape, int hit,
                                  bool zap, int beam_layer, int s_beam, bool remove_hit,
                                  ExtraBlock extra_block, OnCells on_cells, int only = -1,
                                  double* zmat = nullptr, int* nzapped = nullptr) {
  uint8_t* grid = wd.rec;
  Scratch* sc = wd.sc;
  const int lane = wd.lane;
  const int P = t.P, HW = t.H * t.W, W = t.W, L = t.L;
  const int nc = shape.nc;
  const int per = shape.per;
  const int firing = (int)(fire && a.alive);
  if (__ballot(firing != 0 && (only < 0 || lane == only)) == 0ull) {
    wsync();
    return;
  }
  for (int b0 = 0; b0 < P; b0 += per) {
    const int bl = shape.bl, j = shape.j, b = b0 + bl;
    const bool lane_ok = bl < per && b < P;
    const int bs = lane_ok ? b : 0;
    const bool bfire = __shfl(firing, bs) != 0 && lane_ok && (only < 0 || b == only);
    const int bx = __shfl(a.x, bs), by = __shfl(a.y, bs), bo = __shfl(a.ori, bs);
    const int lat = shape.lat, fw = shape.fw;
    const int rdir = (bo + 1) & 3;
    int x = bx, y = by;
    const bool inb = step_cell(t, x, y, lat * dir_dx(rdir) + fw * dir_dx(bo),
                               lat * dir_dy(rdir) + fw * dir_dy(bo));
    const int cell = inb ? y * W + x : 0;
    bool blocked = false, extra_hit = false;
    int hit_player = -1;
    if (bfire && inb) {
      for (int l0 = 0; l0 < L; l0 += 4) {
        uint32_t st[4], info[4];
#pragma unroll
        for (int k = 0; k < 4; ++k) st[k] = l0 + k < L ? grid[(l0 + k) * HW + cell] : 0u;
#pragma unroll
        for (int k = 0; k < 4; ++k) info[k] = wd.sinfo[st[k]];
#pragma unroll
        for (int k = 0; k < 4; ++k) {
          const int s = (int)st[k];
          if (s == 0) continue;
          if ((info[k] >> hit) & 1u) blocked = true;
          const int pl = (int)(info[k] >> 24) - 1;
          if (pl >= 0 && zap) { hit_player = pl; blocked = true; }
          const int xb = extra_block(s, cell);
          if (xb & 1) blocked = true;
          if (xb & 2) extra_hit = true;
          if (xb >> 8) hit_player = (xb >> 8) - 1;
        }
      }
    }
    const unsigned long long stops = __ballot(bfire && (!inb || blocked));
    const uint32_t mine = (uint32_t)(stops >> (bl * nc)) & ((1u << nc) - 1u);
    const bool reached = bfire && inb && (mine & shape.pred) == 0;
    if (reached) grid[beam_layer * HW + cell] = (uint8_t)s_beam;
    const bool zhit = reached && hit_player >= 0;
    if (zhit && remove_hit) atomicOr(&sc->zapped_mask, 1u << hit_player);
    if (zhit && zap) push_event(sc, MP_EVENT_ZAP, b + 1, hit_player + 1);
    if (zhit && zap && zmat) zmat[hit_player * P + b] = 1.0;
    if (lane_ok) sc->victim[b][j] = (int8_t)(zhit ? hit_player : -1);
    const unsigned long long zb = __ballot(zhit);
    if (lane == 0 && zb != 0) tail->ctr[4] += __popcll(zb);
    if (nzapped && lane >= b0 && lane < b0 + per && lane < P)
      *nzapped += __popcll((zb >> ((lane - b0) * nc)) & ((1ull << nc) - 1ull));
    on_cells(b0, per, nc, reached, cell, reached && extra_hit);
  }
  wsync();
}

__device__ inline void zap_rewards(const DevTables& t, const Scratch* sc, int lane, Av& a,
                                   bool fire_zap, int order_zap, int nc, double penalty,
                                   double reward) {
  if (penalty == 0.0 && reward == 0.0) return;
  const int firing = (int)fire_zap;
  for (int r = 0; r < t.P; ++r) {
    const int owner = rdlane(order_zap, r);
    if (rdlane(firing, owner) == 0) continue;
    for (int q = 0; q < nc; ++q) {
      const int victim = sc->victim[owner][q];
      if (victim < 0) continue;
      if (lane == victim) a.reward += penalty;
      if (lane == owner) a.reward += reward;
    }
  }
}

__device__ inline int resolve_respawns(const DevTables& t, const World& wd, WorldTail* tail,
                                       Av& a, bool want_respawn, int order_resp,
                                       int alive_state, uint32_t step, int frame, uint32_t ep,
                                       uint32_t k0, uint32_t k1) {
  uint8_t* grid = wd.rec;
  const int lane = wd.lane;
  const int P = t.P, HW = t.H * t.W, W = t.W;
  const bool is_av = lane < P;
  if (__ballot(want_respawn) == 0) return -1;
  int rcell = 0, rori = 0;
  bool rfree = false;
  if (want_respawn) {
    const Philox4 d = philox4x32_10((uint32_t)lane, RS_RESPAWN, step, ep, k0, k1);
    rcell = wd.spawn[philox_bounded(d, (uint32_t)t.n_spawn)];
    rori = (int)(d.x3 & 3u);
    const int s = grid[t.avatar_layer * HW + rcell];
    rfree = s == 0 || (wd.sinfo[s] >> 24) != 0;
  }
  bool respawned = false;
  const int try_it = (int)(want_respawn && rfree);
  for (int r = 0; r < P; ++r) {
    const int p = rdlane(order_resp, r);
    if (rdlane(try_it, p) == 0) continue;
    const int pc = rdlane(rcell, p);
    const bool occupied = __ballot(is_av && a.alive && a.y * W + a.x == pc) != 0;
    if (lane == p && !occupied) {
      a.alive = 1; a.x = pc % W; a.y = pc / W; a.achange = frame; a.ori = rori;
      respawned = true;
    }
  }
  if (respawned) grid[t.avatar_layer * HW + rcell] = (uint8_t)alive_state;
  const unsigned long long rb = __ballot(respawned);
  if (lane == 0 && rb != 0) tail->ctr[6] += __popcll(rb);
  return respawned ? rcell : -1;
}

__device__ inline void apply_zapped(const DevTables& t, const World& wd, Av& a, bool respawned,
                                    int frame) {
  const uint32_t zapped = wd.sc->zapped_mask;
  if (wd.lane < t.P && a.alive && !respawned && ((zapped >> wd.lane) & 1u)) {
    wd.rec[t.avatar_layer * t.H * t.W + a.y * t.W + a.x] = 0;
    a.alive = 0; a.achange = frame;
  }
}

__device__ inline void finish(const DevTables& t, const World& wd, WorldTail* tail, const Av& a,
                              double aux0, int zap_cooldown, int step_type,
                              const StepOutputs& out, const OrderStreams& os) {
  const int P = t.P, lane = wd.lane, w = wd.w;
  if (lane < MP_MAX_PLAYERS) {
    tail->ax[lane] = (uint8_t)a.x; tail->ay[lane] = (uint8_t)a.y;
    tail->aori[lane] = (uint8_t)a.ori; tail->aalive[lane] = (uint8_t)a.alive;
    tail->ztimer[lane] = (uint8_t)a.ztimer; tail->ctimer[lane] = (uint8_t)a.ctimer;
    tail->achange[lane] = a.achange;
  }
  if (wd.publish) {
    __builtin_amdgcn_fence(__ATOMIC_RELEASE, "workgroup");
    if (lane == 0)
      __hip_atomic_store(wd.publish, wd.publish_value, __ATOMIC_RELEASE, __HIP_MEMORY_SCOPE_WORKGROUP);
  }
  if (lane < P) {
    const size_t o = (size_t)w * P + lane;
    out.reward[o] = a.reward;
    const double v = 1.0 - (double)a.ztimer / (double)zap_cooldown;
    out.ready[o] = a.alive ? (v > 0.0 ? v : 0.0) : 0.0;
    out.aux0[o] = aux0;
    out.position[o * 2 + 0] = a.x;
    out.position[o * 2 + 1] = a.y;
    out.orientation[o] = a.ori;
  }
  double sum = 0.0;
  for (int p = 0; p < P; ++p) sum += rdlane(a.reward, p);
  if (lane == 0) {
    out.collective[w] = sum;
    out.step_type[w] = step_type;
    out.discount[w] = step_type == 1 ? 1.0 : 0.0;
    tail->reward_fx += (int32_t)(sum * 1024.0);
  }
  wsync();
  {
    const Scratch* sc = wd.sc;
    const uint32_t total = sc->ev_count;
    const uint32_t n = total < MP_EVENT_ROWS - 1 ? total : MP_EVENT_ROWS - 1;
    int4* rows = reinterpret_cast<int4*>(out.events) + (size_t)w * MP_EVENT_ROWS;
    if (lane == 0) rows[0] = int4{(int)n, (int)(total - n), 0, 0};
    for (uint32_t i = (uint32_t)lane; i < n; i += 64) {
      const uint32_t e = sc->ev[i];
      rows[1 + i] = int4{(int)(e >> 16), (int)((e >> 8) & 255u), (int)(e & 255u), 0};
    }
  }
  if (wd.next_orders && os.n > 0 && !__builtin_amdgcn_readfirstlane(tail->done)) {
    const uint32_t next = (uint32_t)__builtin_amdgcn_readfirstlane(tail->step) + 1u;
    const uint32_t ep = (uint32_t)__builtin_amdgcn_readfirstlane((int)tail->episode) - 1u;
    const uint64_t seed = tail->seed;
    int o[4];
    shuffled_orders(lane, P, os.s0, os.s1, os.s2, os.s3, os.n, next, ep,
                    (uint32_t)seed, (uint32_t)(seed >> 32), o);
    if (lane < MP_MAX_PLAYERS)
      tail->next_orders[lane] = (uint16_t)(o[0] | (o[1] << 4) | (o[2] << 8) | (o[3] << 12));
    if (lane == 0) tail->orders_step = next;
  } else if (lane == 0) {
    tail->orders_step = 0u;
  }
  wsync();
  const int nvec = t.world_stride >> 4;
  for (int i0 = 0; i0 < nvec; i0 += 8 * 64) {
    uint4 v[8];
#pragma unroll
    for (int k = 0; k < 8; ++k) {
      const int i = i0 + k * 64 + lane;
      v[k] = reinterpret_cast<const uint4*>(wd.rec)[i < nvec ? i : nvec - 1];
    }
#pragma unroll
    for (int k = 0; k < 8; ++k) issued(v[k]);
#pragma unroll
    for (int k = 0; k < 8; ++k) {
      const int i = i0 + k * 64 + lane;
      if (i < nvec) reinterpret_cast<uint4*>(wd.gw)[i] = v[k];
    }
  }
}

__device__ inline uint32_t magic_of(uint32_t d) { return d > 1 ? 0xffffffffu / d + 1u : 0u; }
__device__ inline uint32_t div_by(uint32_t n, uint32_t magic) { return magic ? __umulhi(n, magic) : n; }

__device__ inline void write_layer(const DevTables& t, const uint8_t* rec, const StepOutputs& out,
                                   int w, int lane) {
  const uint32_t L = (uint32_t)t.L, VW = (uint32_t)(t.vl + t.vr + 1), VH = (uint32_t)(t.vf + t.vb + 1);
  const uint32_t n = (uint32_t)t.P * VH * VW * L;
  const uint32_t mL = magic_of(L), mVW = magic_of(VW), mVH = magic_of(VH);
  const uint32_t mW = magic_of((uint32_t)t.W), mH = magic_of((uint32_t)t.H);
  const int ox = t.W * ((t.vl + t.W - 1) / t.W), oy = t.H * ((t.vf + t.H - 1) / t.H);
  const bool torus = t.topology == 1;
  const int W = t.W, H = t.H, HW = t.H * t.W;
  const WorldTail* tail = reinterpret_cast<const WorldTail*>(rec + t.grid_pad);
  const int32_t* lut = out.layer_lut;
  auto value = [&](uint32_t e) -> int32_t {
    const uint32_t cell = div_by(e, mL), l = e - cell * L;
    const uint32_t r = div_by(cell, mVW), vx = cell - r * VW;
    const uint32_t p = div_by(r, mVH), vy = r - p * VH;
    int x = (int)tail->ax[p] + (int)vx - t.vl, y = (int)tail->ay[p] + (int)vy - t.vf;
    bool in;
    if (torus) {
      const uint32_t xx = (uint32_t)(x + ox), yy = (uint32_t)(y + oy);
      x = (int)(xx - div_by(xx, mW) * (uint32_t)W);
      y = (int)(yy - div_by(yy, mH) * (uint32_t)H);
      in = true;
    } else {
      in = x >= 0 && x < W && y >= 0 && y < H;
    }
    const int s = in && tail->aalive[p] ? (int)rec[(int)l * HW + y * W + x] : 256;
    return lut[p * kLayerLutRow + (uint32_t)s];
  };
  int32_t* blk = out.layer + (size_t)w * n;
  const uint32_t mis = (uint32_t)(reinterpret_cast<uintptr_t>(blk) >> 2) & 3u;
  const uint32_t head = ((4u - mis) & 3u) < n ? ((4u - mis) & 3u) : n;
  if ((uint32_t)lane < head) blk[lane] = value((uint32_t)lane);
  const uint32_t nq = (n - head) >> 2;
  int4* q = reinterpret_cast<int4*>(blk + head);
  for (uint32_t c0 = 0; c0 < nq; c0 += 4 * 64) {
    int4 v[4];
#pragma unroll
    for (int k = 0; k < 4; ++k) {
      const uint32_t c = c0 + (uint32_t)(k * 64 + lane);
      const uint32_t e = head + 4u * (c < nq ? c : nq - 1u);
      v[k] = int4{value(e), value(e + 1), value(e + 2), value(e + 3)};
    }
#pragma unroll
    for (int k = 0; k < 4; ++k) {
      const uint32_t c = c0 + (uint32_t)(k * 64 + lane);
      if (c < nq) q[c] = v[k];
    }
  }
  const uint32_t rest = head + 4u * nq + (uint32_t)lane;
  if (rest < n) blk[rest] = value(rest);
}

__device__ inline int dispatch(const DevTables& t, const WorldTail* tail, int lane, int w,
                               const uint8_t* reset_mask, int mode, int auto_reset,
                               const StepOutputs& out) {
  if (mode == STEP_MODE_RESET) return (reset_mask ? reset_mask[w] != 0 : true) ? 1 : 0;
  if (!tail->started) return 0;
  if (tail->done && auto_reset) return 1;
  if (tail->done) {
    if (lane < t.P) out.reward[w * t.P + lane] = 0.0;
    if (lane == 0) {
      out.collective[w] = 0.0; out.step_type[w] = 2; out.discount[w] = 0.0;
      reinterpret_cast<int4*>(out.events)[(size_t)w * MP_EVENT_ROWS] = int4{0, 0, 0, 0};
    }
    return 0;
  }
  return 2;
}

struct StepArgs {
  uint8_t* state;
  const int32_t* actions;
  const uint8_t* reset_mask;
  int mode, auto_reset, num_worlds;
  int next_orders;
  StepOutputs out;
  const uint8_t* bank;
  const int32_t* src;
  int bank_rows;
};

template <class Tables>
__host__ __device__ inline int extra_bytes(const Tables&) { return 0; }
template <class Tables>
__device__ inline void init_extra(const DevTables&, const Tables&, uint8_t*, int) {}

}

#endif
```

meltingpot_amd/csrc/step_kernels.hip:

```cpp
#include "../../include/mp_pack.h"
#include "step_clean_up.h"
#include "step_coins.h"
#include "step_commons.h"
#include "step_coop.h"
#include "step_gift.h"
#include "step_mushroom.h"
#include "step_cook.h"
#include "step_matrix.h"
#include "step_territory.h"
#include "step_load.h"

namespace {

using namespace stepk;

constexpr int kWorldsPerGroup = 4;

template <class Tables, class Sites>
__device__ inline void run_one_world(const DevTables& t, const Tables& c, const StepArgs& args,
                                     int extra) {
  extern __shared__ __attribute__((aligned(16))) uint8_t smem[];
  const int lane = threadIdx.x & 63;
  const int wave = __builtin_amdgcn_readfirstlane((int)threadIdx.x >> 6);
  const int w = blockIdx.x * ((int)blockDim.x >> 6) + wave;
  uint8_t* tables = smem;
  const int per_world = t.world_stride + scratch_bytes(t) + extra;
  uint8_t* mine = smem + tables_bytes(t) + wave * per_world;
  const bool live = w < args.num_worlds;
#ifdef MP_STEP_TIMING
  const unsigned long long t_entry = __builtin_readcyclecounter();
#endif
  World wd = make_world(t, mine, tables, mine + t.world_stride, args.state, live ? w : 0, lane);
  wd.next_orders = args.next_orders;
  int act_id = 0;
  Sites sites = Sites();
  if (live) {
    act_id = fetch_action_id(t, args.actions, args.mode, w, lane);
    sites = load_sites(c, lane);
    load_record(t, wd.rec, wd.gw, lane);
  }
  load_tables(t, tables, (int)threadIdx.x, (int)blockDim.x);
  clear_marks(t, wd.mark, lane);
  begin_step(wd.sc, lane);
  __syncthreads();
  if (!live) return;
#ifdef MP_STEP_TIMING
  if (lane == 0 && (w == 7 || w == 2000) && args.mode == STEP_MODE_STEP)
    printf("w %d: entry -> record in LDS %llu cycles\n", w, __builtin_readcyclecounter() - t_entry);
#endif
  const Action act = lookup_action(t, wd, act_id, args.mode);
  init_extra(t, c, wd.extra, lane);
  step_or_load(t, c, sites, wd, act, args);
  if (args.out.layer) {
    wsync();
    write_layer(t, wd.rec, args.out, w, lane);
  }
}

__global__ __launch_bounds__(kWorldsPerGroup * 64) void k_step_clean_up(DevTables t, CleanUpTables c, StepArgs args) {
  run_one_world<CleanUpTables, CleanUpSites>(t, c, args, 0);
}
__global__ __launch_bounds__(kWorldsPerGroup * 64) void k_step_commons(DevTables t, CommonsTables c, StepArgs args) {
  run_one_world<CommonsTables, CommonsSites>(t, c, args, 0);
}
__global__ __launch_bounds__(kWorldsPerGroup * 64) void k_step_coins(DevTables t, CoinsTables c, StepArgs args) {
  run_one_world<CoinsTables, CoinsSites>(t, c, args, 0);
}
__global__ __launch_bounds__(kWorldsPerGroup * 64) void k_step_coop(DevTables t, CoopTables c, StepArgs args) {
  run_one_world<CoopTables, CoopSites>(t, c, args, 0);
}
__global__ __launch_bounds__(kWorldsPerGroup * 64) void k_step_gift(DevTables t, GiftTables c, StepArgs args) {
  run_one_world<GiftTables, GiftSites>(t, c, args, 0);
}
__global__ __launch_bounds__(kWorldsPerGroup * 64) void k_step_cook(DevTables t, CookTables c, StepArgs args) {
  run_one_world<CookTables, CookSites>(t, c, args, 0);
}
__global__ __launch_bounds__(kWorldsPerGroup * 64) void k_step_mushroom(DevTables t, MushroomTables c, StepArgs args) {
  run_one_world<MushroomTables, MushroomSites>(t, c, args, extra_bytes(c));
}
__global__ __launch_bounds__(kWorldsPerGroup * 64) void k_step_matrix(DevTables t, MatrixTables c, StepArgs args) {
  run_one_world<MatrixTables, MatrixSites>(t, c, args, 0);
}
__global__ __launch_bounds__(kWorldsPerGroup * 64) void k_step_territory(DevTables t, TerritoryTables c, StepArgs args) {
  run_one_world<TerritoryTables, TerritorySites>(t, c, args, extra_bytes(c));
}

__global__ void k_layer_view(DevTables t, const uint8_t* __restrict__ state,
                             int32_t* __restrict__ out, int num_worlds) {
  const int VW = t.vl + t.vr + 1, VH = t.vf + t.vb + 1, HW = t.H * t.W;
  const long long i = (long long)blockIdx.x * blockDim.x + threadIdx.x;
  if (i >= (long long)num_worlds * t.P * VH * VW) return;
  const int vx = (int)(i % VW), vy = (int)((i / VW) % VH);
  const int p = (int)((i / (VW * VH)) % t.P), w = (int)(i / ((long long)VW * VH * t.P));
  const uint8_t* rec = state + (size_t)w * t.world_stride;
  const WorldTail* tail = reinterpret_cast<const WorldTail*>(rec + t.grid_pad);
  const int32_t* remap = t.view_sprite_map + (size_t)p * t.nsprites;
  int32_t* dst = out + (size_t)i * t.L;
  int x = tail->ax[p] + (vx - t.vl), y = tail->ay[p] + (vy - t.vf);
  bool in = true;
  if (t.topology == 1) { x = ((x % t.W) + t.W) % t.W; y = ((y % t.H) + t.H) % t.H; }
  else in = x >= 0 && x < t.W && y >= 0 && y < t.H;
  if (!in || !tail->aalive[p]) {
    for (int l = 0; l < t.L; ++l) dst[l] = 1 + remap[0];
    return;
  }
  for (int l = 0; l < t.L; ++l) {
    const int s = rec[l * HW + y * t.W + x];
    const int sprite = s ? t.state_sprite[s] : -1;
    dst[l] = sprite >= 0 ? 1 + remap[sprite] : 0;
  }
}

}

void launch_layer_view(const DevTables& t, const uint8_t* state, int32_t* out, int num_worlds,
                       hipStream_t stream) {
  const long long n = (long long)num_worlds * t.P * (t.vl + t.vr + 1) * (t.vf + t.vb + 1);
  hipLaunchKernelGGL(k_layer_view, dim3((unsigned)((n + 255) / 256)), dim3(256), 0, stream, t,
                     state, out, num_worlds);
}

int step_lds_bytes(const DevTables& t, const SubstrateTables& s, int wpg) {
  const int extra = s.substrate == MPK_SUBSTRATE_TERRITORY ? stepk::extra_bytes(s.tr)
                    : s.substrate == MPK_SUBSTRATE_EXTERNALITY_MUSHROOMS ? stepk::extra_bytes(s.em) : 0;
  return stepk::tables_bytes(t) + wpg * (t.world_stride + stepk::scratch_bytes(t) + extra);
}

int step_worlds_per_group(const DevTables& t, const SubstrateTables& s) {
  for (int wpg = kWorldsPerGroup; wpg >= 1; wpg >>= 1)
    if (step_lds_bytes(t, s, wpg) <= 160 * 1024) return wpg;
  return 0;
}

int prepare_step() {
  const void* k[9] = {
      reinterpret_cast<const void*>(&k_step_clean_up), reinterpret_cast<const void*>(&k_step_commons),
      reinterpret_cast<const void*>(&k_step_coins), reinterpret_cast<const void*>(&k_step_territory),
      reinterpret_cast<const void*>(&k_step_matrix), reinterpret_cast<const void*>(&k_step_coop),
      reinterpret_cast<const void*>(&k_step_gift), reinterpret_cast<const void*>(&k_step_cook),
      reinterpret_cast<const void*>(&k_step_mushroom)};
  for (const void* f : k)
    if (hipFuncSetAttribute(f, hipFuncAttributeMaxDynamicSharedMemorySize, 160 * 1024) != hipSuccess)
      return 1;
  return 0;
}

void launch_step(const DevTables& t, const SubstrateTables& s, const stepk::StepArgs& args,
                 hipStream_t stream) {
  const int wpg = step_worlds_per_group(t, s);
  const size_t lds = (size_t)step_lds_bytes(t, s, wpg);
  const dim3 grid((args.num_worlds + wpg - 1) / wpg), block(wpg * 64);
  switch (s.substrate) {
    case MPK_SUBSTRATE_CLEAN_UP:
      hipLaunchKernelGGL(k_step_clean_up, grid, block, lds, stream, t, s.cu, args);
      break;
    case MPK_SUBSTRATE_COMMONS_HARVEST:
      hipLaunchKernelGGL(k_step_commons, grid, block, lds, stream, t, s.ch, args);
      break;
    case MPK_SUBSTRATE_COINS:
      hipLaunchKernelGGL(k_step_coins, grid, block, lds, stream, t, s.co, args);
      break;
    case MPK_SUBSTRATE_TERRITORY:
      hipLaunchKernelGGL(k_step_territory, grid, block, lds, stream, t, s.tr, args);
      break;
    case MPK_SUBSTRATE_THE_MATRIX:
      hipLaunchKernelGGL(k_step_matrix, grid, block, lds, stream, t, s.mx, args);
      break;
    case MPK_SUBSTRATE_COOP_MINING:
      hipLaunchKernelGGL(k_step_coop, grid, block, lds, stream, t, s.cm, args);
      break;
    case MPK_SUBSTRATE_GIFT_REFINEMENTS:
      hipLaunchKernelGGL(k_step_gift, grid, block, lds, stream, t, s.gr, args);
      break;
    case MPK_SUBSTRATE_COLLABORATIVE_COOKING:
      hipLaunchKernelGGL(k_step_cook, grid, block, lds, stream, t, s.cc, args);
      break;
    case MPK_SUBSTRATE_EXTERNALITY_MUSHROOMS:
      hipLaunchKernelGGL(k_step_mushroom, grid, block, lds, stream, t, s.em, args);
      break;
  }
}
```

meltingpot_amd/csrc/step_many.hip:

```cpp
#include "../../include/mp_pack.h"
#include "step_clean_up.h"
#include "step_coins.h"
#include "step_commons.h"
#include "step_coop.h"
#include "step_gift.h"
#include "step_mushroom.h"
#include "step_cook.h"
#include "step_matrix.h"
#include "step_territory.h"
#include "step_load.h"
#include "step_many.h"

namespace {

using namespace stepk;

constexpr int kWorldsPerGroup = 4;

template <class T>
__device__ inline T* row_of(uint8_t* base, long long bytes, int k, T* in_place) {
  return base ? reinterpret_cast<T*>(base + (long long)k * bytes) : in_place;
}

template <bool Rows, bool States, class Tables, class Sites>
__device__ inline void run_many(const DevTables& t, const Tables& c, const StepArgs& args0,
                                const ManyArgs& m, const StepRows* rp, int extra,
                                const StateRows* sp = nullptr) {
  extern __shared__ __attribute__((aligned(16))) uint8_t smem[];
  const int lane = threadIdx.x & 63;
  const int wave = __builtin_amdgcn_readfirstlane((int)threadIdx.x >> 6);
  const int w = blockIdx.x * ((int)blockDim.x >> 6) + wave;
  uint8_t* tables = smem;
  const int per_world = t.world_stride + scratch_bytes(t) + extra;
  uint8_t* mine = smem + tables_bytes(t) + wave * per_world;
  const bool live = w < args0.num_worlds;
  World wd = make_world(t, mine, tables, mine + t.world_stride, args0.state, live ? w : 0, lane);
  wd.next_orders = args0.next_orders;
  int act_id = 0;
  Sites sites = Sites();
  if (live) {
    act_id = fetch_action_id(t, args0.actions, args0.mode, w, lane);
    sites = load_sites(c, lane);
    load_record(t, wd.rec, wd.gw, lane);
  }
  load_tables(t, tables, (int)threadIdx.x, (int)blockDim.x);
  clear_marks(t, wd.mark, lane);
  begin_step(wd.sc, lane);
  __syncthreads();
  if (!live) return;
  init_extra(t, c, wd.extra, lane);
  StepArgs args = args0;
  const int K = m.steps;
  for (int k = 0; k < K; ++k) {
    int next_id = 0;
    if (k + 1 < K)
      next_id = fetch_action_id(t, args0.actions + (long long)(k + 1) * m.actions_step, args0.mode, w, lane);
    if (k) {
      wsync();
      begin_step(wd.sc, lane);
      wsync();
    }
    int lane_k = lane;
    asm volatile("" : "+v"(lane_k));
    wd.lane = lane_k;
    if constexpr (Rows) {
      const StepRows& r = *rp;
      const WorldTail* tl = reinterpret_cast<const WorldTail*>(wd.rec + t.grid_pad);
      const bool frozen = __builtin_amdgcn_readfirstlane((int)(tl->started && tl->done)) && !args0.auto_reset;
      const StepOutputs prev = args.out;
      args.out.ready = row_of(r.fin[0], r.fin_bytes[0], k, args0.out.ready);
      args.out.aux0 = row_of(r.fin[1], r.fin_bytes[1], k, args0.out.aux0);
      args.out.position = row_of(r.fin[2], r.fin_bytes[2], k, args0.out.position);
      args.out.orientation = row_of(r.fin[3], r.fin_bytes[3], k, args0.out.orientation);
      if (frozen && lane_k < t.P) {
        const size_t o = (size_t)w * t.P + lane_k;
        if (r.fin[0]) args.out.ready[o] = prev.ready[o];
        if (r.fin[1]) args.out.aux0[o] = prev.aux0[o];
        if (r.fin[2]) {
          args.out.position[o * 2 + 0] = prev.position[o * 2 + 0];
          args.out.position[o * 2 + 1] = prev.position[o * 2 + 1];
        }
        if (r.fin[3]) args.out.orientation[o] = prev.orientation[o];
      }
    }
    args.out.reward = row_of(m.row[0], m.row_bytes[0], k, args0.out.reward);
    args.out.collective = row_of(m.row[1], m.row_bytes[1], k, args0.out.collective);
    args.out.step_type = row_of(m.row[2], m.row_bytes[2], k, args0.out.step_type);
    args.out.discount = row_of(m.row[3], m.row_bytes[3], k, args0.out.discount);
    args.out.events = row_of(m.row[4], m.row_bytes[4], k, args0.out.events);
    const Action act = lookup_action(t, wd, act_id, args0.mode);
    step_world(t, c, sites, wd, act, args);
    act_id = next_id;
    if constexpr (Rows) {
      const StepRows& r = *rp;
      if (States || r.layer || r.n_level) {
        wsync();
        const WorldTail* tl = reinterpret_cast<const WorldTail*>(wd.rec + t.grid_pad);
        if (__builtin_amdgcn_readfirstlane((int)tl->started)) {
          for (int i = 0; i < r.n_level; ++i) {
            const long long n = r.level[i].count;
            const double* src = r.level[i].src + (size_t)w * n;
            double* dst = reinterpret_cast<double*>(r.level[i].row + (long long)k * r.level[i].bytes) + (size_t)w * n;
            for (int j = lane_k; j < n; j += 64) dst[j] = src[j];
          }
          if (r.layer) {
            StepOutputs lo = args0.out;
            lo.layer = reinterpret_cast<int32_t*>(r.layer + (long long)k * r.layer_bytes);
            lo.layer_lut = r.layer_lut;
            write_layer(t, wd.rec, lo, w, lane_k);
          }
          if constexpr (States)
            store_record(t, wd.rec, sp->row + (long long)k * sp->bytes + (size_t)w * t.world_stride, lane_k);
        }
      }
    }
  }
  wsync();
  const WorldTail* tail = reinterpret_cast<const WorldTail*>(wd.rec + t.grid_pad);
  if (__builtin_amdgcn_readfirstlane((int)tail->started)) {
    const size_t o = (size_t)w * t.P + lane;
    if (m.row[0] && lane < t.P) args0.out.reward[o] = args.out.reward[o];
    if (lane == 0) {
      if (m.row[1]) args0.out.collective[w] = args.out.collective[w];
      if (m.row[2]) args0.out.step_type[w] = args.out.step_type[w];
      if (m.row[3]) args0.out.discount[w] = args.out.discount[w];
    }
    if (m.row[4]) {
      const int4* src = reinterpret_cast<const int4*>(args.out.events) + (size_t)w * MP_EVENT_ROWS;
      int4* dst = reinterpret_cast<int4*>(args0.out.events) + (size_t)w * MP_EVENT_ROWS;
      int n = 0;
      if (lane == 0) { const int4 h = src[0]; dst[0] = h; n = h.x; }
      n = __builtin_amdgcn_readfirstlane(n);
      n = n < 0 ? 0 : n > MP_EVENT_ROWS - 1 ? MP_EVENT_ROWS - 1 : n;
      for (int i = lane; i < n; i += 64) dst[1 + i] = src[1 + i];
    }
    if constexpr (Rows) {
      const StepRows& r = *rp;
      if (lane < t.P) {
        if (r.fin[0]) args0.out.ready[o] = args.out.ready[o];
        if (r.fin[1]) args0.out.aux0[o] = args.out.aux0[o];
        if (r.fin[2]) {
          args0.out.position[o * 2 + 0] = args.out.position[o * 2 + 0];
          args0.out.position[o * 2 + 1] = args.out.position[o * 2 + 1];
        }
        if (r.fin[3]) args0.out.orientation[o] = args.out.orientation[o];
      }
    }
  }
  if (args0.out.layer) write_layer(t, wd.rec, args0.out, w, lane);
}

#define MP_STEP_MANY_KERNEL(name, TablesT, SitesT, extra)                                            \
  __global__ __launch_bounds__(kWorldsPerGroup * 64) void name(DevTables t, TablesT c, StepArgs args, \
                                                               ManyArgs m) {                         \
    run_many<false, false, TablesT, SitesT>(t, c, args, m, nullptr, extra);                          \
  }
MP_STEP_MANY_KERNEL(k_step_many_clean_up, CleanUpTables, CleanUpSites, 0)
MP_STEP_MANY_KERNEL(k_step_many_commons, CommonsTables, CommonsSites, 0)
MP_STEP_MANY_KERNEL(k_step_many_coins, CoinsTables, CoinsSites, 0)
MP_STEP_MANY_KERNEL(k_step_many_coop, CoopTables, CoopSites, 0)
MP_STEP_MANY_KERNEL(k_step_many_gift, GiftTables, GiftSites, 0)
MP_STEP_MANY_KERNEL(k_step_many_cook, CookTables, CookSites, 0)
MP_STEP_MANY_KERNEL(k_step_many_mushroom, MushroomTables, MushroomSites, extra_bytes(c))
MP_STEP_MANY_KERNEL(k_step_many_matrix, MatrixTables, MatrixSites, 0)
MP_STEP_MANY_KERNEL(k_step_many_territory, TerritoryTables, TerritorySites, extra_bytes(c))
#undef MP_STEP_MANY_KERNEL

#define MP_STEP_ROWS_KERNEL(name, TablesT, SitesT, extra)                                            \
  __global__ __launch_bounds__(kWorldsPerGroup * 64) void name(DevTables t, TablesT c, StepArgs args, \
                                                               ManyArgs m, StepRows r) {             \
    run_many<true, false, TablesT, SitesT>(t, c, args, m, &r, extra);                                \
  }
MP_STEP_ROWS_KERNEL(k_step_rows_clean_up, CleanUpTables, CleanUpSites, 0)
MP_STEP_ROWS_KERNEL(k_step_rows_commons, CommonsTables, CommonsSites, 0)
MP_STEP_ROWS_KERNEL(k_step_rows_coins, CoinsTables, CoinsSites, 0)
MP_STEP_ROWS_KERNEL(k_step_rows_coop, CoopTables, CoopSites, 0)
MP_STEP_ROWS_KERNEL(k_step_rows_gift, GiftTables, GiftSites, 0)
MP_STEP_ROWS_KERNEL(k_step_rows_cook, CookTables, CookSites, 0)
MP_STEP_ROWS_KERNEL(k_step_rows_mushroom, MushroomTables, MushroomSites, extra_bytes(c))
MP_STEP_ROWS_KERNEL(k_step_rows_matrix, MatrixTables, MatrixSites, 0)
MP_STEP_ROWS_KERNEL(k_step_rows_territory, TerritoryTables, TerritorySites, extra_bytes(c))
#undef MP_STEP_ROWS_KERNEL

#define MP_STEP_STATES_KERNEL(name, TablesT, SitesT, extra)                                          \
  __global__ __launch_bounds__(kWorldsPerGroup * 64) void name(DevTables t, TablesT c, StepArgs args, \
                                                               ManyArgs m, StepRows r, StateRows s) { \
    run_many<true, true, TablesT, SitesT>(t, c, args, m, &r, extra, &s);                             \
  }
MP_STEP_STATES_KERNEL(k_step_states_clean_up, CleanUpTables, CleanUpSites, 0)
MP_STEP_STATES_KERNEL(k_step_states_commons, CommonsTables, CommonsSites, 0)
MP_STEP_STATES_KERNEL(k_step_states_coins, CoinsTables, CoinsSites, 0)
MP_STEP_STATES_KERNEL(k_step_states_coop, CoopTables, CoopSites, 0)
MP_STEP_STATES_KERNEL(k_step_states_gift, GiftTables, GiftSites, 0)
MP_STEP_STATES_KERNEL(k_step_states_cook, CookTables, CookSites, 0)
MP_STEP_STATES_KERNEL(k_step_states_mushroom, MushroomTables, MushroomSites, extra_bytes(c))
MP_STEP_STATES_KERNEL(k_step_states_matrix, MatrixTables, MatrixSites, 0)
MP_STEP_STATES_KERNEL(k_step_states_territory, TerritoryTables, TerritorySites, extra_bytes(c))
#undef MP_STEP_STATES_KERNEL

}

int prepare_step_many() {
  const void* km[27] = {
#define MP_BOTH(level)                                                                             \
  reinterpret_cast<const void*>(&k_step_many_##level), reinterpret_cast<const void*>(&k_step_rows_##level), \
      reinterpret_cast<const void*>(&k_step_states_##level)
      MP_BOTH(clean_up), MP_BOTH(commons), MP_BOTH(coins), MP_BOTH(territory), MP_BOTH(matrix),
      MP_BOTH(coop), MP_BOTH(gift), MP_BOTH(cook), MP_BOTH(mushroom)};
#undef MP_BOTH
  for (const void* f : km)
    if (hipFuncSetAttribute(f, hipFuncAttributeMaxDynamicSharedMemorySize, 160 * 1024) != hipSuccess)
      return 1;
// ... 32 lines not shown
```

meltingpot_amd/engine.py:

```python

from __future__ import annotations

import ctypes
import os
from typing import Dict, Optional, Sequence

import numpy as np

from meltingpot_amd import _build

OBS_RGB = 0
OBS_WORLD_RGB = 1
OBS_REWARD = 2
OBS_READY_TO_SHOOT = 3
OBS_AUX0 = 4
OBS_STEP_TYPE = 5
OBS_DISCOUNT = 6
OBS_COLLECTIVE_REWARD = 7
OBS_POSITION = 8
OBS_ORIENTATION = 9
OBS_EVENTS = 10
OBS_AUX1 = 11
OBS_AUX2 = 12
OBS_AUX3 = 13
OBS_AUX4 = 14
OBS_ZAP_MATRIX = 15
OBS_LAYER = 16
OBS_INVENTORY = 17
OBS_INTERACTION_INVENTORIES = 18
OBS_MATRIX_CUMULANTS = 19
OBS_INTERACTION_REWARDS = 20
OBS_RGB_POOL2 = 21
OBS_RGB_POOL4 = 22
OBS_RGB_POOL8 = 23
OBS_RGB_POOL = {2: OBS_RGB_POOL2, 4: OBS_RGB_POOL4, 8: OBS_RGB_POOL8}
PIXEL_KINDS = (OBS_RGB, OBS_WORLD_RGB, OBS_RGB_POOL2, OBS_RGB_POOL4, OBS_RGB_POOL8)


def pool_rgb(images, k: int) -> np.ndarray:
  a = np.asarray(images)
  if k == 1:
    return a.astype(np.uint8, copy=True)
  *lead, h, w, c = a.shape
  if h % k or w % k:
    raise ValueError(f"an image of {h} x {w} does not pool by {k}")
  s = a.astype(np.uint32).reshape(*lead, h // k, k, w // k, k, c).sum(axis=(-4, -2))
  return ((s + (k * k) // 2) // (k * k)).astype(np.uint8)


def matrix_cumulant_names(num_resources: int):
  names = ["INTERACTED_THIS_STEP"]
  for k in range(1, num_resources + 1):
    names += [f"COLLECTED_RESOURCE_{k}", f"DESTROYED_RESOURCE_{k}",
              f"ARGMAX_INTERACTION_INVENTORY_WAS_{k}"]
  return names
EVENT_ROWS = 128
EVENT_TYPES = {
    1: ("zap", ("source", "target")),
    2: ("edible_consumed", ("player_index",)),
    3: ("player_cleaned", ("player_index",)),
    4: ("claimed_resource", ("player_index",)),
    5: ("destroyed_resource", ("player_index",)),
    6: ("sanctioning", ("source", "target")),
    7: ("removal_due_to_sanctioning", ("source", "target")),
    8: ("set_sanctioning_level", ("player_index", "level")),
    9: ("AvatarStarted", ()),
    10: ("coin_consumed", ("player_index", "types")),
    11: ("interaction", ("row_player_idx", "col_player_idx")),
    12: ("collected_resource", ("player_index", "class")),
    13: ("mining", ("player", "ore_type")),
    14: ("extraction", ("player", "ore_type")),
    15: ("extraction_pair", ("player_a", "player_b", "ore_type")),
    16: ("gift", ("gifter_index", "gifter_role", "receipient_index", "receipient_role",
                  "source_type", "received_amount")),
    20: ("eating_mushroom", ("player_index", "mushroom_type")),
    17: ("receiver_accepted_item", ("player_index", "item")),
    18: ("item_dropped_into_pot", ("player_index", "item")),
    19: ("cooked_food_collected_from_pot", ("player_index", "cooked_item")),
}
COOKING_ITEMS = ("empty", "tomato", "dish", "soup")
MUSHROOM_TYPES = ("fullInternalityZeroExternality", "halfInternalityHalfExternality",
                  "zeroInternalityFullExternality", "negativeInternalityNegativeExternality")

COUNTER_NAMES = ("world_steps", "agent_steps", "episodes", "reward_sum_x1024",
                 "zaps", "aux0", "respawns", "bad_actions")

MP_ERR_INVALID = -1
MP_ERR_NO_DEVICE = -3
MP_ABI_VERSION = 8

ABI_SYMBOLS = (
    "mp_abi_version", "mp_last_error", "mp_create", "mp_destroy", "mp_info",
    "mp_set_stream", "mp_bind_output", "mp_reset", "mp_step", "mp_step_host",
    "mp_step_fields", "mp_step_fields_host",
    "mp_observe", "mp_obs_bytes", "mp_dump", "mp_snapshot_bytes",
    "mp_snapshot", "mp_restore", "mp_counters", "mp_sync", "mp_fault_words",
    "mp_alloc_output", "mp_free_output", "mp_tune", "mp_place_output",
    "mp_bind_output_ring", "mp_set_retired_va_limit",
    "mp_torch_alloc", "mp_torch_free", "mp_box_fill")

KERNEL_GENERIC, KERNEL_STOCK = 0, 1


class MpDevOptions(ctypes.Structure):
  _fields_ = [("struct_size", ctypes.c_uint32)] + [(n, ctypes.c_int32) for n in (
      "batch_worlds", "waves", "feeders", "max_groups", "scratch_cells",
      "no_composite_cache", "max_composites", "verbose", "late_feeder_prio",
      "ring_batches", "static_pct", "world_waves", "store_sc1", "head", "no_next_orders",
      "record_pad", "pace", "team", "generic_kernel")]


class MpConfig(ctypes.Structure):
  _fields_ = [
      ("struct_size", ctypes.c_uint32),
      ("device", ctypes.c_int32),
      ("num_worlds", ctypes.c_int32),
      ("auto_reset", ctypes.c_int32),
      ("world_offset", ctypes.c_uint64),
      ("base_seed", ctypes.c_uint64),
      ("stream", ctypes.c_void_p),
      ("num_players", ctypes.c_int32),
      ("debug_observations", ctypes.c_int32),
      ("unfused", ctypes.c_int32),
      ("literal_base_seed", ctypes.c_int32),
      ("dev", ctypes.POINTER(MpDevOptions)),
      ("roles", ctypes.POINTER(ctypes.c_int32)),
      ("world_pool", ctypes.c_int32),
  ]


class MpInfo(ctypes.Structure):
  _fields_ = [(n, ctypes.c_int32) for n in (
      "abi_version", "substrate", "num_worlds", "num_players", "num_actions",
      "map_h", "map_w", "num_layers", "sprite_size", "view_h", "view_w",
      "max_frames", "world_state_bytes", "fused", "num_resources",
      "num_action_fields", "plan_batch_worlds", "plan_ring_batches", "plan_owned_batches",
      "plan_pooled_batches", "plan_groups", "plan_store_sc1", "plan_feeders", "plan_waves",
      "ring_slots", "ring_next", "plan_pace", "visible_layers", "plan_team", "plan_late_priority")] + [("retired_va_bytes", ctypes.c_int64),
                                      ("retired_va_limit", ctypes.c_int64)]


class MpPlacement(ctypes.Structure):
  _fields_ = [("candidates", ctypes.c_int32), ("picked", ctypes.c_int32),
              ("us", ctypes.c_float * 32), ("stepped", ctypes.c_int32),
              ("requested", ctypes.c_int32), ("out_of_memory", ctypes.c_int32),
              ("early_exit", ctypes.c_int32), ("setup_ms", ctypes.c_float)]


class MpBoxFill(ctypes.Structure):
  _fields_ = [("bytes", ctypes.c_uint64), ("memset_us", ctypes.c_float),
              ("product_order_us", ctypes.c_float), ("front_4k_us", ctypes.c_float),
              ("groups", ctypes.c_int32), ("waves", ctypes.c_int32), ("span_bytes", ctypes.c_uint32)]


MP_STATES_FINGERPRINT, MP_STATES_SAVE, MP_STATES_LOAD = 1, 2, 3


class MpKernelVariant(ctypes.Structure):
  _fields_ = [("struct_size", ctypes.c_uint32), ("variant", ctypes.c_int32),
              ("pack", ctypes.c_void_p), ("pack_len", ctypes.c_uint64),
              ("cfg", ctypes.POINTER(MpConfig)), ("fields", ctypes.c_void_p),
              ("fields_cap", ctypes.c_uint64)]


class MpWorldStates(ctypes.Structure):
  _fields_ = [("struct_size", ctypes.c_uint32), ("op", ctypes.c_int32),
              ("fingerprint", ctypes.c_uint64), ("worlds", ctypes.c_void_p),
              ("src", ctypes.c_void_p), ("bank", ctypes.c_void_p), ("bank_bytes", ctypes.c_uint64),
              ("count", ctypes.c_int32), ("bank_rows", ctypes.c_int32)]


def world_states_request(L, handle, op: int, **fields) -> MpWorldStates:
  req = MpWorldStates(ctypes.sizeof(MpWorldStates), op)
  for k, v in fields.items():
    setattr(req, k, v)
  call = L.mp_restore if op == MP_STATES_LOAD else L.mp_snapshot
  _check(L, call(handle, ctypes.addressof(req), ctypes.sizeof(req)),
         "mp_restore (MP_STATES_LOAD)" if op == MP_STATES_LOAD else "mp_snapshot (MpWorldStates)")
  return req


class MpStatesObserve(ctypes.Structure):
  _fields_ = [("struct_size", ctypes.c_uint32), ("kind", ctypes.c_int32),
              ("fingerprint", ctypes.c_uint64), ("bank", ctypes.c_void_p), ("rows", ctypes.c_void_p),
              ("dst", ctypes.c_void_p), ("dst_bytes", ctypes.c_uint64), ("bank_rows", ctypes.c_int32),
              ("count", ctypes.c_int32), ("reserved", ctypes.c_uint64)]


STATE_OBS_KINDS = PIXEL_KINDS + (OBS_LAYER, OBS_READY_TO_SHOOT, OBS_POSITION, OBS_ORIENTATION,
                                 OBS_INVENTORY)


def states_observe_request(L, handle, **fields) -> MpStatesObserve:
  req = MpStatesObserve(ctypes.sizeof(MpStatesObserve))
  for k, v in fields.items():
    setattr(req, k, v)
  _check(L, L.mp_snapshot(handle, ctypes.addressof(req), ctypes.sizeof(req)),
         "mp_snapshot (MpStatesObserve)")
  return req


class MpStateField(ctypes.Structure):
  _fields_ = [("name", ctypes.c_char * 16), ("offset", ctypes.c_int32), ("elem_bytes", ctypes.c_int32),
              ("count", ctypes.c_int32), ("reserved", ctypes.c_int32)]


_LAYOUT_INTS = ("map_h", "map_w", "num_layers", "num_players", "num_states", "grid_planes", "grid_bytes",
                "grid_pad", "world_stride", "tail_bytes", "max_frames", "avatar_layer", "substrate",
                "player_block")


class MpStateLayout(ctypes.Structure):
  _fields_ = ([("struct_size", ctypes.c_uint32), ("layout_version", ctypes.c_uint32),
               ("pack", ctypes.c_void_p), ("pack_len", ctypes.c_uint64), ("cfg", ctypes.POINTER(MpConfig))] +
              [(n, ctypes.c_int32) for n in _LAYOUT_INTS] + [("reserved", ctypes.c_int32 * 2)] +
              [("fingerprint", ctypes.c_uint64), ("fields", ctypes.POINTER(MpStateField)),
               ("fields_cap", ctypes.c_int32), ("num_fields", ctypes.c_int32)])


MP_CHECK_ROWS, MP_CHECK_HOST, MP_CHECK_FILTER = 1, 2, 3


class MpStatesCheck(ctypes.Structure):
  _fields_ = [("struct_size", ctypes.c_uint32), ("op", ctypes.c_int32), ("fingerprint", ctypes.c_uint64),
              ("pack", ctypes.c_void_p), ("pack_len", ctypes.c_uint64), ("cfg", ctypes.POINTER(MpConfig)),
              ("bank", ctypes.c_void_p), ("bank_rows", ctypes.c_int32), ("count", ctypes.c_int32),
              ("rows", ctypes.c_void_p), ("out", ctypes.c_void_p), ("out_bytes", ctypes.c_uint64),
              ("reserved", ctypes.c_uint64)]


RULE_OK = 0
RULE_STATE_RANGE = 1
RULE_STATE_LAYER = 2
RULE_TAIL_RANGE = 3
RULE_AVATAR_CELL = 4
RULE_AVATAR_STRAY = 5
RULE_ORDERS = 6
RULE_LEVEL = 7
RULE_NAMES = {RULE_OK: "well-formed", RULE_STATE_RANGE: "a plane byte that is no state of the pack",
              RULE_STATE_LAYER: "a state in another layer's plane", RULE_TAIL_RANGE: "a tail value out of range",
              RULE_AVATAR_CELL: "a living avatar that is not where the tail says",
              RULE_AVATAR_STRAY: "an avatar state where the tail does not put that avatar",
              RULE_ORDERS: "the cached visiting orders", RULE_LEVEL: "a level rule"}
LEVEL_BYTE_FIELD = 1
LEVEL_AUX_COUNT = 16
LEVEL_PLANE0, LEVEL_PLANE1 = 17, 18
LEVEL_MARKER_OFF_MAP, LEVEL_MARKER_CELL, LEVEL_FOLLOWER = 19, 20, 21
LEVEL_NAMES = {LEVEL_AUX_COUNT: "aux_count outside the level's table", LEVEL_PLANE0: "a plane byte the level cannot take",
               LEVEL_PLANE1: "a plane byte the level cannot take",
               LEVEL_MARKER_OFF_MAP: "a marker on the map whose position is no cell",
               LEVEL_MARKER_CELL: "a marker on the map whose cell of the marker plane is empty",
               LEVEL_FOLLOWER: "an avatar without its connected piece on its cell"}


def level_offset(sub: int, offset: int) -> int:
  return (int(sub) << 24) | (int(offset) & 0xffffff)


class StateLayout:

  def __init__(self, req: MpStateLayout, fields):
    self.H, self.W, self.L, self.P = req.map_h, req.map_w, req.num_layers, req.num_players
    self.nstates = req.num_states
    for n in _LAYOUT_INTS[5:]:
      setattr(self, n, int(getattr(req, n)))
    self.layout_version = int(req.layout_version)
    self.fingerprint = int(req.fingerprint)
    self.fields = {f.name.decode(): (int(f.offset), int(f.elem_bytes), int(f.count)) for f in fields}

  def field_offset(self, name: str, index: int = 0) -> int:
    off, elem, count = self.fields[name]
    if not 0 <= index < count:
      raise IndexError(f"{name} has {count} elements")
    return self.grid_pad + off + elem * index

  def cell_offset(self, plane: int, x: int, y: int) -> int:
    return (plane * self.H + y) * self.W + x

  def describe(self, rule: int, offset: int) -> str:
    rule, offset = int(rule), int(offset) & 0xffffffff
    if rule == RULE_OK:
      return "well-formed"
    if rule == -1:
      return f"row index {offset - (1 << 32) if offset >= 1 << 31 else offset} is no row of the bank"
    what = RULE_NAMES.get(rule, f"rule {rule}")
    if rule == RULE_LEVEL:
      sub, offset = offset >> 24, offset & 0xffffff
      what = LEVEL_NAMES.get(sub, "a per-avatar byte outside the level's range")
    return f"rule {rule}: {what} at {self.where(offset)}"

  def where(self, offset: int) -> str:
    hw = self.H * self.W
    if offset < self.grid_planes * hw:
      plane, cell = divmod(offset, hw)
      kind = "plane" if plane < self.L else "hidden plane"
      return f"{kind} {plane} cell (x={cell % self.W}, y={cell // self.W})"
    if offset < self.grid_pad:
      return f"byte {offset} (behind the planes)"
    t = offset - self.grid_pad
    for name, (off, elem, count) in self.fields.items():
      if off <= t < off + elem * count:
        return f"{name}[{(t - off) // elem}]" if count > 1 else name
    return f"byte {offset}"


def _layout_request(L, handle, pack_bytes=None, num_players: int = 0, dev=None) -> StateLayout:
  fields = (MpStateField * 64)()
  req = MpStateLayout(ctypes.sizeof(MpStateLayout))
  req.fields = ctypes.cast(fields, ctypes.POINTER(MpStateField))
  req.fields_cap = 64
  keep = None
  if handle is None:
    keep = _host_config(pack_bytes, num_players, dev)
    req.pack, req.pack_len, req.cfg = ctypes.addressof(keep[0]), len(pack_bytes), ctypes.pointer(keep[1])
  _check(L, L.mp_snapshot(handle, ctypes.addressof(req), ctypes.sizeof(req)), "mp_snapshot (MpStateLayout)")
  return StateLayout(req, fields[:req.num_fields])


def _host_config(pack_bytes: bytes, num_players: int = 0, dev=None):
  cfg = MpConfig(ctypes.sizeof(MpConfig), 0, 1, 1, 0, 0, None, int(num_players))
  opts = None
  if dev:
    opts = MpDevOptions(ctypes.sizeof(MpDevOptions), max_composites=-1)
    for k, v in dev.items():
      setattr(opts, k, int(v))
    cfg.dev = ctypes.pointer(opts)
  return ctypes.create_string_buffer(pack_bytes, len(pack_bytes)), cfg, opts


def state_layout(pack_bytes: bytes, *, num_players: int = 0, dev: Optional[Dict[str, int]] = None) -> StateLayout:
  return _layout_request(load_library(), None, pack_bytes, num_players, dev)


def check_states_host(pack_bytes: bytes, rows, *, fingerprint: Optional[int] = None, which=None,
                      num_players: int = 0, dev: Optional[Dict[str, int]] = None) -> np.ndarray:
  L = load_library()
  bank = np.ascontiguousarray(rows, np.uint8)
  if bank.ndim != 2 or bank.shape[0] < 1:
    raise ValueError("check_states_host: rows must be a uint8 array [M, S]")
  keep = _host_config(pack_bytes, num_players, dev)
  layout = _layout_request(L, None, pack_bytes, num_players, dev)
  if bank.shape[1] != layout.world_stride:
    raise ValueError(f"check_states_host: rows of {bank.shape[1]} bytes, the pack's are {layout.world_stride}")
  idx = None if which is None else np.ascontiguousarray(np.asarray(which).reshape(-1), np.int32)
  count = bank.shape[0] if idx is None else int(idx.size)
  if count < 1:
    raise ValueError("check_states_host: no rows to judge")
  out = np.zeros((count, 2), np.int32)
  req = MpStatesCheck(ctypes.sizeof(MpStatesCheck), MP_CHECK_HOST,
                      layout.fingerprint if fingerprint is None else int(fingerprint))
  req.pack, req.pack_len, req.cfg = ctypes.addressof(keep[0]), len(pack_bytes), ctypes.pointer(keep[1])
  req.bank, req.bank_rows, req.count = bank.ctypes.data, int(bank.shape[0]), count
  req.rows = None if idx is None else idx.ctypes.data
  req.out, req.out_bytes = out.ctypes.data, out.nbytes
  _check(L, L.mp_snapshot(None, ctypes.addressof(req), ctypes.sizeof(req)), "mp_snapshot (MpStatesCheck)")
  return out


STEP_MANY_MAX = 4096
STEP_MANY_NAMES = {"reward": OBS_REWARD, "collective_reward": OBS_COLLECTIVE_REWARD,
                   "step_type": OBS_STEP_TYPE, "discount": OBS_DISCOUNT, "events": OBS_EVENTS}
STEP_MANY_KINDS = tuple(STEP_MANY_NAMES)
_STEP_MANY_KIND_OF = STEP_MANY_NAMES


class MpStepMany(ctypes.Structure):
  _fields_ = [("struct_size", ctypes.c_uint32), ("steps", ctypes.c_int32),
              ("fields", ctypes.c_int32), ("reserved", ctypes.c_int32),
              ("actions", ctypes.c_void_p), ("actions_step_bytes", ctypes.c_uint64),
              ("per_step", ctypes.c_void_p * 5), ("per_step_bytes", ctypes.c_uint64 * 5)]


class MpStepRow(ctypes.Structure):
  _fields_ = [("kind", ctypes.c_int32), ("reserved", ctypes.c_int32), ("rows", ctypes.c_void_p),
              ("step_bytes", ctypes.c_uint64)]


class MpStepTrajectory(ctypes.Structure):
  _fields_ = [("struct_size", ctypes.c_uint32), ("steps", ctypes.c_int32),
              ("fields", ctypes.c_int32), ("num_rows", ctypes.c_int32),
              ("actions", ctypes.c_void_p), ("actions_step_bytes", ctypes.c_uint64),
              ("rows", ctypes.POINTER(MpStepRow))]


STEP_ROW_STATE = 0x100

STEP_ROW_KINDS = tuple(k for k in range(OBS_RGB_POOL8 + 1) if k not in PIXEL_KINDS)


def step_row(shapes, key):
  kind = STEP_MANY_NAMES.get(key, key)
  shape, dtype = shapes[kind]
  return kind, tuple(shape[1:]), dtype


def check_step_rows(observations, *, steps: Optional[int] = None, shapes=None, out=None,
                    taken=()) -> tuple:
  kinds = []
  for kind in observations:
    if isinstance(kind, bool) or not isinstance(kind, (int, np.integer)):
      raise ValueError(f"step_many: observations= takes OBS_* kinds (got {kind!r})")
    kind = int(kind)
    if kind in PIXEL_KINDS:
      raise ValueError(f"step_many: kind {kind} is a pixel kind; a K-step launch draws no frames. "
                       "Intermediate frames are what step() with a rollout ring "
                       "(bind_ring) writes")
    if kind not in STEP_ROW_KINDS:
      raise ValueError(f"step_many: {kind} is no observation kind")
    if kind in kinds or kind in taken:
      raise ValueError(f"step_many: kind {kind} is named twice")
    kinds.append(kind)
  if out is not None and shapes is not None and steps is not None:
    for kind in kinds:
      buf = out.get(kind)
      if buf is None:
        continue
      shape, dtype = shapes[kind]
      want = (int(steps),) + tuple(int(d) for d in shape)
      if (not hasattr(buf, "stride") or str(buf.dtype) != str(dtype) or
          tuple(int(d) for d in buf.shape) != want):
        raise ValueError(f"step_many: out[{kind}] must be a {dtype} tensor of shape {want} "
                         f"(got {getattr(buf, 'dtype', type(buf))} {tuple(getattr(buf, 'shape', ()))})")
      _step_distance(buf, f"out[{kind}]")
  return tuple(kinds)


def check_step_many(shape, dtype, num_worlds: int, num_players: int, *, repeat=None,
                    num_fields: Optional[int] = None) -> int:
  shape = tuple(int(d) for d in shape)
  block = (num_worlds, num_players) + ((int(num_fields),) if num_fields else ())
  name = str(dtype)
  if "int" not in name or "float" in name:
    raise ValueError(f"step_many: actions must hold integers (got {name})")
  if repeat is not None:
    if shape != block:
      raise ValueError(f"step_many: with repeat= the actions are one block of shape {block} (got {shape})")
    K = int(repeat)
  else:
    if len(shape) != len(block) + 1 or shape[1:] != block:
      raise ValueError(f"step_many: actions must have shape (K,) + {block} (got {shape})")
    K = shape[0]
  if not 1 <= K <= STEP_MANY_MAX:
    raise ValueError(f"step_many: K = {K} is outside [1, {STEP_MANY_MAX}]")
  return K


def _step_distance(tensor, what: str) -> int:
  if not tensor[0].is_contiguous():
    raise ValueError(f"step_many: {what} may be non-contiguous along K only (each step's block "
                     f"must be contiguous; strides {tuple(tensor.stride())})")
  block = int(tensor[0].numel())
  if tensor.shape[0] == 1:
    return block * tensor.element_size()
  if tensor.stride(0) < block:
    raise ValueError(f"step_many: the steps of {what} overlap (stride {tensor.stride(0)} < {block})")
  return int(tensor.stride(0)) * tensor.element_size()


class EngineError(RuntimeError):
  pass


_lib = None


def load_library(build: bool = True) -> ctypes.CDLL:
  global _lib
  if _lib is not None:
    return _lib
  try:
    import torch
  except ImportError:
    pass
  path = _build.LIB_PATH
  override = os.environ.get("MP_ENGINE_LIB")
  if override:
    path = override
  elif build:
    path = _build.build_engine()
  if not os.path.exists(path):
    raise EngineError(
        f"{path} is missing: build it with `python -c 'import __graft_entry__ "
        "as g; g.build()'` (hipcc --offload-arch=gfx950). There is no fallback.")
  L = ctypes.CDLL(path)
  vp, i32, u64 = ctypes.c_void_p, ctypes.c_int32, ctypes.c_uint64
  L.mp_abi_version.restype = i32
  L.mp_last_error.restype = ctypes.c_char_p
  L.mp_create.restype = i32
  L.mp_create.argtypes = [vp, u64, ctypes.POINTER(MpConfig),
                          ctypes.POINTER(vp)]
  L.mp_destroy.restype = None
  L.mp_destroy.argtypes = [vp]
  L.mp_info.restype = i32
  L.mp_info.argtypes = [vp, ctypes.POINTER(MpInfo)]
  L.mp_set_stream.restype = i32
  L.mp_set_stream.argtypes = [vp, vp]
  L.mp_bind_output.restype = i32
  L.mp_bind_output.argtypes = [vp, i32, vp]
  L.mp_reset.restype = i32
  L.mp_reset.argtypes = [vp, vp, vp]
  L.mp_step.restype = i32
  L.mp_step.argtypes = [vp, vp]
  L.mp_step_host.restype = i32
  L.mp_step_host.argtypes = [vp, vp]
  L.mp_step_fields.restype = i32
  L.mp_step_fields.argtypes = [vp, vp]
  L.mp_step_fields_host.restype = i32
  L.mp_step_fields_host.argtypes = [vp, vp]
  L.mp_observe.restype = i32
  L.mp_observe.argtypes = [vp, i32, vp]
  L.mp_obs_bytes.restype = u64
  L.mp_obs_bytes.argtypes = [vp, i32]
  L.mp_dump.restype = i32
  L.mp_dump.argtypes = [vp, vp, vp, vp]
  L.mp_snapshot_bytes.restype = u64
  L.mp_snapshot_bytes.argtypes = [vp]
  L.mp_snapshot.restype = i32
  L.mp_snapshot.argtypes = [vp, vp, u64]
  L.mp_restore.restype = i32
  L.mp_restore.argtypes = [vp, vp, u64]
  L.mp_counters.restype = i32
  L.mp_counters.argtypes = [vp, vp]
  L.mp_sync.restype = i32
  L.mp_sync.argtypes = [vp]
  L.mp_alloc_output.restype = i32
  L.mp_alloc_output.argtypes = [i32, u64, u64, ctypes.POINTER(vp)]
  L.mp_free_output.restype = i32
  L.mp_free_output.argtypes = [i32, vp]
  L.mp_tune.restype = i32
  L.mp_tune.argtypes = [vp, ctypes.POINTER(ctypes.c_double)]
  L.mp_place_output.restype = i32
  L.mp_place_output.argtypes = [vp, i32, i32, u64, ctypes.POINTER(vp), ctypes.POINTER(MpPlacement)]
  L.mp_fault_words.restype = i32
  L.mp_fault_words.argtypes = [vp, vp]
  L.mp_bind_output_ring.restype = i32
  L.mp_bind_output_ring.argtypes = [vp, i32, vp, u64, i32]
  L.mp_box_fill.restype = i32
  L.mp_box_fill.argtypes = [vp, i32, i32, ctypes.POINTER(MpBoxFill)]
  L.mp_set_retired_va_limit.restype = i32
  L.mp_set_retired_va_limit.argtypes = [ctypes.c_int64]
  _lib = L
  return L


def kernel_variant(pack_bytes: bytes, *, num_players: int = 0,
                   dev: Optional[Dict[str, int]] = None) -> int:
  return pack_fields(pack_bytes, num_players=num_players, dev=dev)[0]


def pack_fields(pack_bytes: bytes, *, num_players: int = 0, dev: Optional[Dict[str, int]] = None,
                want_fields: bool = False):
  L = load_library()
  cfg = MpConfig(ctypes.sizeof(MpConfig), 0, 1, 1, 0, 0, None, int(num_players))
  if dev:
    opts = MpDevOptions(ctypes.sizeof(MpDevOptions), max_composites=-1)
    for k, v in dev.items():
      setattr(opts, k, int(v))
    cfg.dev = ctypes.pointer(opts)
  buf = ctypes.create_string_buffer(pack_bytes, len(pack_bytes))
  out = ctypes.create_string_buffer(1 << 16) if want_fields else None
  req = MpKernelVariant(ctypes.sizeof(MpKernelVariant), 0, ctypes.addressof(buf), len(pack_bytes),
                        ctypes.pointer(cfg), ctypes.addressof(out) if out else None,
                        len(out) if out else 0)
  _check(L, L.mp_snapshot(None, ctypes.addressof(req), ctypes.sizeof(req)), "mp_snapshot (MpKernelVariant)")
  return req.variant, (out.value.decode() if out else "")


def _check(L, rc: int, what: str):
  if rc == 0:
    return
  msg = (L.mp_last_error() or b"").decode()
  if rc == MP_ERR_INVALID:
    raise ValueError(f"{what}: {msg}")
  raise EngineError(f"{what} failed ({rc}): {msg}")


class Engine:

  def __init__(self, pack_bytes: bytes, num_worlds: int, *, device: int = 0,
               auto_reset: bool = True, world_offset: int = 0,
               base_seed: int = 0, literal_seed: bool = False, num_players: int = 0,
               debug_observations: bool = False, unfused: Optional[bool] = None,
               dev: Optional[Dict[str, int]] = None,
               roles: Optional[Sequence[int]] = None, placements: int = 8,
               world_pool: int = 1):
    if (isinstance(world_pool, bool) or not isinstance(world_pool, (int, np.integer)) or
        int(world_pool) not in (0, 1, 2, 4, 8)):
      raise ValueError(f"world_pool must be 1, 2, 4 or 8 (got {world_pool!r})")
    self.world_pool = max(1, int(world_pool))
    import torch
    self._torch = torch
    self.placements = placements
    self.place_max_bytes = 0
    self.placement: Dict[int, dict] = {}
    self._L = load_library()
    if not torch.cuda.is_available():
      pass
    self._pack = ctypes.create_string_buffer(pack_bytes, len(pack_bytes))
    self.pack_bytes = pack_bytes
    stream = None
    if torch.cuda.is_available():
      torch.cuda.set_device(device)
      stream = torch.cuda.current_stream(device).cuda_stream
    cfg = MpConfig(ctypes.sizeof(MpConfig), device, num_worlds,
                   1 if auto_reset else 0, world_offset, int(base_seed) % (1 << 64), stream,
                   int(num_players), 1 if debug_observations else 0,
                   0 if unfused is None else (1 if unfused else 2),
                   1 if literal_seed else 0, None, None, self.world_pool)
    if roles is not None:
      if num_players and len(roles) != num_players:
        raise ValueError(f"{len(roles)} roles for {num_players} players")
      self._roles = (ctypes.c_int32 * len(roles))(*[int(r) for r in roles])
      cfg.roles = ctypes.cast(self._roles, ctypes.POINTER(ctypes.c_int32))
      cfg.num_players = len(roles)
    if dev:
      opts = MpDevOptions(ctypes.sizeof(MpDevOptions), max_composites=-1)
      for k, v in dev.items():
        if not hasattr(opts, k) or k == "struct_size":
          raise ValueError(f"unknown MpDevOptions field {k!r}")
        setattr(opts, k, int(v))
      self._dev = opts
      cfg.dev = ctypes.pointer(opts)
    handle = ctypes.c_void_p()
    rc = self._L.mp_create(self._pack, len(pack_bytes), ctypes.byref(cfg),
                           ctypes.byref(handle))
    self._h = None
    _check(self._L, rc, "mp_create")
    self._h = handle
    info = MpInfo()
    _check(self._L, self._L.mp_info(self._h, ctypes.byref(info)), "mp_info")
    self.info = info
    self.device = torch.device("cuda", device)
    self.N, self.P = info.num_worlds, info.num_players
    self.num_actions = info.num_actions
    S = info.sprite_size
    self.shapes = {
        OBS_RGB: ((self.N, self.P, info.view_h * S, info.view_w * S, 3), torch.uint8),
        OBS_WORLD_RGB: ((self.N, info.map_h * S // self.world_pool, info.map_w * S // self.world_pool,
                         3), torch.uint8),
        OBS_REWARD: ((self.N, self.P), torch.float64),
        OBS_READY_TO_SHOOT: ((self.N, self.P), torch.float64),
        OBS_AUX0: ((self.N, self.P), torch.float64),
        OBS_STEP_TYPE: ((self.N,), torch.int32),
        OBS_DISCOUNT: ((self.N,), torch.float64),
        OBS_COLLECTIVE_REWARD: ((self.N,), torch.float64),
        OBS_POSITION: ((self.N, self.P, 2), torch.int32),
        OBS_ORIENTATION: ((self.N, self.P), torch.int32),
        OBS_EVENTS: ((self.N, EVENT_ROWS, 4), torch.int32),
        OBS_AUX1: ((self.N, self.P), torch.float64),
        OBS_AUX2: ((self.N, self.P), torch.float64),
        OBS_AUX3: ((self.N, self.P), torch.float64),
        OBS_AUX4: ((self.N, self.P), torch.float64),
        OBS_ZAP_MATRIX: ((self.N, self.P, self.P), torch.float64),
        OBS_LAYER: ((self.N, self.P, info.view_h, info.view_w, info.num_layers),
                    torch.int32),
        OBS_INVENTORY: ((self.N, self.P, info.num_resources), torch.float64),
        OBS_INTERACTION_INVENTORIES: ((self.N, self.P, 2, info.num_resources), torch.float64),
        OBS_MATRIX_CUMULANTS: ((self.N, self.P, 1 + 3 * info.num_resources), torch.float64),
        OBS_INTERACTION_REWARDS: ((self.N, self.P, 2), torch.float64),
        **{kind: ((self.N, self.P, info.view_h * S // k, info.view_w * S // k, 3), torch.uint8)
           for k, kind in OBS_RGB_POOL.items()},
    }
    self._bound: Dict[int, "torch.Tensor"] = {}

  @property
  def fused(self) -> bool:
    info = MpInfo()
    _check(self._L, self._L.mp_info(self._h, ctypes.byref(info)), "mp_info")
    return bool(info.fused)

  @property
  def plan(self) -> Dict[str, int]:
    info = MpInfo()
    _check(self._L, self._L.mp_info(self._h, ctypes.byref(info)), "mp_info")
    return {"batch_worlds": info.plan_batch_worlds, "ring_batches": info.plan_ring_batches,
            "owned_batches": info.plan_owned_batches, "pooled_batches": info.plan_pooled_batches,
            "workgroups": info.plan_groups, "sc1_stores": info.plan_store_sc1,
            "feeders": info.plan_feeders, "waves": info.plan_waves, "pace": info.plan_pace,
            "xcd_teams": info.plan_team, "late_feeder_priority": info.plan_late_priority,
            "stock": self._kernel_variant()}

  def _kernel_variant(self) -> int:
    req = MpKernelVariant(ctypes.sizeof(MpKernelVariant))
    if self._L.mp_snapshot(self._h, ctypes.addressof(req), ctypes.sizeof(req)) != 0:
      return KERNEL_GENERIC
    return int(req.variant)

  def close(self):
    if getattr(self, "_h", None):
      self._L.mp_destroy(self._h)
      self._h = None
      self._bound.clear()

  def __del__(self):
    try:
      self.close()
    except Exception:
      pass

  def __enter__(self):
    return self

  def __exit__(self, *exc):
    self.close()

  def events(self, world: int = 0):
    return self.events_all(worlds=[world])[0]

  def events_all(self, worlds=None):
    if worlds is None:
      worlds, pick = list(range(self.N)), (lambda t: t)
    else:
      worlds = [int(w) for w in worlds]
      index = self._torch.as_tensor(worlds, dtype=self._torch.long, device=self.device)
      pick = lambda t: t.index_select(0, index)
    rows = pick(self.observe(OBS_EVENTS)).cpu().numpy()
    extra = None
    if self.info.num_resources and any(
        (rows[i, 1:1 + int(rows[i, 0, 0]), 0] == 11).any() for i in range(len(worlds))):
      extra = (pick(self.observe(OBS_INTERACTION_REWARDS)).cpu().numpy(),
               pick(self.observe(OBS_INTERACTION_INVENTORIES)).cpu().numpy())
    roles = pack_agent_roles(self.pack_bytes) if (rows[:, 1:, 0] == 16).any() else None
    return [self._decode_events(rows[i], w, None if extra is None else (extra[0][i], extra[1][i]),
                                roles)
            for i, w in enumerate(worlds)]

  @staticmethod
  def _decode_events(rows, world, interaction=None, agent_roles=None):
    n = int(rows[0, 0])
    if rows[0, 1]:
      raise EngineError(f"world {world}: {int(rows[0, 1])} events beyond the "
                        f"{EVENT_ROWS - 1} rows of MP_OBS_EVENTS were dropped")
    out = []
    for t, a, b, _ in sorted(tuple(int(v) for v in r) for r in rows[1:1 + n]):
      name, keys = EVENT_TYPES[t]
      if t == 5 and b:
        keys = ("player_index", "class")
      payload = dict(zip(keys, (a, b)))
      if t == 15:
        payload = {"player_a": a, "player_b": b >> 2, "ore_type": b & 3}
      if t == 16:
        payload = {"gifter_index": a & 15, "receipient_index": b & 15,
                   "source_type": a >> 4, "received_amount": b >> 4}
        if agent_roles:
          payload.update(gifter_role=agent_roles[(a & 15) - 1],
                         receipient_role=agent_roles[(b & 15) - 1])
      if t == 20:
        payload = {"player_index": a, "mushroom_type": MUSHROOM_TYPES[b - 1]}
      if t in (17, 18, 19):
        payload = {"player_index": a, keys[1]: COOKING_ITEMS[b],
                   **({"receiver": "Receiver"} if t == 17 else {"pot": "CookingPot"})}
      if t == 11 and interaction is not None:
        rewards, inventories = interaction
        payload.update(row_reward=float(rewards[a - 1, 0]), col_reward=float(rewards[a - 1, 1]),
                       row_inventory=inventories[a - 1, 0].copy(),
                       col_inventory=inventories[b - 1, 0].copy())
      out.append((name, payload))
    return out

  def empty(self, kind: int):
    shape, dtype = self.shapes[kind]
    return self._torch.empty(shape, dtype=dtype, device=self.device)

  def _wrap(self, kind: int, ptr: int, leading: int = 0):
    t = self._torch
    shape, dtype = self.shapes[kind]
    if leading:
      shape = (leading,) + tuple(shape)
    nbytes = int(np.prod(shape)) * t.empty((), dtype=dtype).element_size()
    L, dev_index = self._L, self.device.index or 0

    class _Owner:
      __cuda_array_interface__ = {"shape": (nbytes,), "typestr": "|u1",
# ... 433 lines not shown
```

Measured before the change: 306.9 million.

## Write back only touched 64-byte lines of clean_up world state

Adds a per-world bitmap of 64-byte lines written during a clean_up step. Every grid write in the step path now sets a bit with an atomic, and finish copies only the marked lines plus the tail region back to global state instead of the whole record. Plane clears skip the store when the chunk is already zero, so untouched planes stay unmarked. This is meant to cut global write traffic, at the cost of atomics, bitmap clearing each step, and the risk of stale global state if any write path misses its mark.

```diff
diff --git a/include/mp_engine.h b/include/mp_engine.h
--- a/include/mp_engine.h
+++ b/include/mp_engine.h
@@ -94,6 +94,7 @@
   int32_t pace;
   int32_t team;
   int32_t generic_kernel;
+  int32_t full_writeback;
 } MpDevOptions;
 
 typedef struct {
diff --git a/meltingpot_amd/csrc/frame_kernel.h b/meltingpot_amd/csrc/frame_kernel.h
--- a/meltingpot_amd/csrc/frame_kernel.h
+++ b/meltingpot_amd/csrc/frame_kernel.h
@@ -736,6 +736,7 @@
             wd.publish = &ctrl->slot_batch[r0 + sl];
             wd.publish_value = (uint32_t)(k + 1);
             wd.next_orders = args.next_orders;
+            wd.full_wb = (args.mode & 1) | args.full_writeback;
             bool have_rec = false;
             if (head_pending) {
               head_pending = false;
@@ -764,7 +765,7 @@
                                    __HIP_MEMORY_SCOPE_WORKGROUP);
               }
             }
-            stepk::begin_step(wd.sc, lane_w);
+            stepk::begin_step(t, wd, lane_w);
             stepk::wsync();
             const stepk::Action act = stepk::lookup_action(t, wd, act_id, args.mode);
             stepk::step_or_load(t, c, sites, wd, act, args);
diff --git a/meltingpot_amd/csrc/mp_engine.hip b/meltingpot_amd/csrc/mp_engine.hip
--- a/meltingpot_amd/csrc/mp_engine.hip
+++ b/meltingpot_amd/csrc/mp_engine.hip
@@ -138,6 +138,7 @@
   uint32_t* d_claim = nullptr;
   int num_cus = 0;
   int next_orders = 1;
+  int full_writeback = 0;
   bool has_dev = false;
   bool touched = false;
   bool has_state = false;
@@ -350,6 +351,7 @@
   args.bank = bank; args.src = src; args.bank_rows = bank_rows;
   args.mode = mode; args.auto_reset = e->auto_reset; args.num_worlds = e->N;
   args.next_orders = e->next_orders;
+  args.full_writeback = e->full_writeback;
   const bool ringing = e->ring_slots > 0 && !e->ring_hold;
   const int slot = e->ring_slots > 0 ? (int)(e->ring_cursor % (uint64_t)e->ring_slots) : 0;
   if (ringing) { e->point_ring(slot); ++e->ring_cursor; }
@@ -868,6 +870,7 @@
   const MpDevOptions* dev = cfg.dev;
   e->has_dev = dev != nullptr;
   e->next_orders = !(dev && dev->no_next_orders);
+  e->full_writeback = dev && dev->full_writeback ? 1 : 0;
   e->device = cfg.device;
   e->N = cfg.num_worlds;
   e->auto_reset = cfg.auto_reset;
@@ -909,6 +912,7 @@
   cfg = &h->cfg;
   if (cfg->dev) {
     if (cfg->dev->struct_size != sizeof(MpDevOptions) &&
+        cfg->dev->struct_size != offsetof(MpDevOptions, full_writeback) &&
         cfg->dev->struct_size != offsetof(MpDevOptions, generic_kernel))
       return fail(MP_ERR_INVALID, "mp_create: bad MpDevOptions (struct_size)");
     memcpy(&h->dev, cfg->dev, cfg->dev->struct_size);
diff --git a/meltingpot_amd/csrc/step_clean_up.h b/meltingpot_amd/csrc/step_clean_up.h
--- a/meltingpot_amd/csrc/step_clean_up.h
+++ b/meltingpot_amd/csrc/step_clean_up.h
@@ -44,6 +44,11 @@
   const int P = t.P, HW = t.H * t.W, W = t.W;
   const bool is_av = lane < P;
   auto at = [&](int layer, int cell) -> uint8_t& { return grid[layer * HW + cell]; };
+  constexpr bool kMark = marks_writes<CleanUpTables>::value;
+  auto put = [&](int layer, int cell, int v) {
+    grid[layer * HW + cell] = (uint8_t)v;
+    touch(wd, layer * HW + cell);
+  };
 
   const OrderStreams kOrders = {RS_SHUFFLE_MOVE, RS_SHUFFLE_ZAP, RS_SHUFFLE_RESPAWN, 0, 3};
 
@@ -102,8 +107,8 @@
     };
     const int a_move = act.move, a_turn = act.turn, a_zap = act.fire0, a_clean = act.fire1,
               bad = act.bad;
-    clear_bytes(grid, c.zap.layer * HW, HW, lane);
-    clear_bytes(grid, c.clean_layer * HW, HW, lane);
+    clear_plane(wd, c.zap.layer * HW, HW, lane);
+    clear_plane(wd, c.clean_layer * HW, HW, lane);
     TSTAMP(2);
 
     if (step > c.dirt_delay) {
@@ -124,8 +129,8 @@
           const int cell = rdlane(q == 0 ? sites.dirt[0] : q == 1 ? sites.dirt[1]
                                   : q == 2 ? sites.dirt[2] : sites.dirt[3], site & 63);
           if (lane == 0 && at(c.dirt_layer, cell) == 0) {
-            at(c.dirt_wait_layer, cell) = 0;
-            at(c.dirt_layer, cell) = (uint8_t)c.s_dirt;
+            put(c.dirt_wait_layer, cell, 0);
+            put(c.dirt_layer, cell, c.s_dirt);
           }
         }
       }
@@ -137,7 +142,7 @@
         const int cell = sites.apple[q];
         if (cell < 0) continue;
         if (philox_u53(draw(RS_APPLE_GROW, (uint32_t)(q * 64 + lane))) < apple_thr)
-          if (at(c.apple_layer, cell) == 0) at(c.apple_layer, cell) = (uint8_t)c.s_apple;
+          if (at(c.apple_layer, cell) == 0) put(c.apple_layer, cell, c.s_apple);
       }
     }
 
@@ -170,7 +175,7 @@
     int cleaned = 0, ate = 0;
 
     TSTAMP(5);
-    const bool wants = resolve_moves(t, wd, a, a_move, a_turn, order_move, alive_state);
+    const bool wants = resolve_moves<kMark>(t, wd, a, a_move, a_turn, order_move, alive_state);
     int ate_cell = -1;
     if (wants && at(c.apple_layer, a.y * W + a.x) == c.s_apple) {
       a.reward += c.eat_reward; ate = 1; ate_cell = a.y * W + a.x;
@@ -180,7 +185,7 @@
 
     TSTAMP(6);
     int nzapped = 0, ncleaned = 0;
-    fire_beams(t, wd, tail, a, fire_zap, beam_lane(c.zap.shape, lane), c.zap.hit, true,
+    fire_beams<kMark>(t, wd, tail, a, fire_zap, beam_lane(c.zap.shape, lane), c.zap.hit, true,
                c.zap.layer, c.zap.s_hit, c.zap.remove_hit != 0,
                [](int, int) { return 0; },
                [](int, int, int, bool, int, bool) {}, -1, zmat, &nzapped);
@@ -188,7 +193,7 @@
                 c.zap.reward);
     TSTAMP(7);
     const BeamLane clean_lane = beam_lane(c.clean_shape, lane);
-    fire_beams(t, wd, tail, a, fire_clean, clean_lane, c.clean_hit, false,
+    fire_beams<kMark>(t, wd, tail, a, fire_clean, clean_lane, c.clean_hit, false,
                c.clean_layer, c.s_clean_hit, false,
                [&](int s, int) { return s == c.s_dirt ? 3 : 0; },
                [&](int b0, int per, int nc, bool reached, int cell, bool dhit) {
@@ -208,7 +213,7 @@
                });
 
     TSTAMP(8);
-    const int rcell = resolve_respawns(t, wd, tail, a, want_respawn, order_resp, alive_state,
+    const int rcell = resolve_respawns<kMark>(t, wd, tail, a, want_respawn, order_resp, alive_state,
                                        (uint32_t)step, frame, ep, k0, k1);
     if (rcell >= 0 && at(c.apple_layer, rcell) == c.s_apple) {
       a.reward += c.eat_reward; ate = 1; ate_cell = rcell;
@@ -223,14 +228,14 @@
         uint32_t k = 0;
 #pragma unroll
         for (uint32_t f = 1; f < 4; ++f) if (s == ((c.s_water_packed >> (8u * f)) & 255u)) k = f;
-        at(c.water_layer, cell) = (uint8_t)(c.s_water_packed >> (8u * ((k + 1u) & 3u)));
+        put(c.water_layer, cell, (uint8_t)(c.s_water_packed >> (8u * ((k + 1u) & 3u))));
       }
     }
     wsync();
 
     TSTAMP(9);
-    if (ate_cell >= 0) at(c.apple_layer, ate_cell) = 0;
-    apply_zapped(t, wd, a, rcell >= 0, frame);
+    if (ate_cell >= 0) put(c.apple_layer, ate_cell, 0);
+    apply_zapped<kMark>(t, wd, a, rcell >= 0, frame);
     wsync();
     int dirt_count = 0;
     {
@@ -243,8 +248,8 @@
           if (mark[cell]) {
             mark[cell] = 0;
             if (at(c.dirt_layer, cell) == c.s_dirt && at(c.dirt_wait_layer, cell) == 0) {
-              at(c.dirt_layer, cell) = 0;
-              at(c.dirt_wait_layer, cell) = (uint8_t)c.s_dirt_wait;
+              put(c.dirt_layer, cell, 0);
+              put(c.dirt_wait_layer, cell, c.s_dirt_wait);
             }
           }
           dirty = at(c.dirt_layer, cell) == c.s_dirt;
@@ -276,7 +281,7 @@
     if (out.dbg[2]) out.dbg[2][o] = dbg_zapped;
     if (out.dbg[3]) out.dbg[3][o] = dbg_others_ate;
   }
-  finish(t, wd, tail, a, aux0, c.zap.cooldown, step_type, out, kOrders);
+  finish<kMark>(t, wd, tail, a, aux0, c.zap.cooldown, step_type, out, kOrders);
   TSTAMP(11);
 #ifdef MP_STEP_TIMING
   if (lane == 0 && (w == 7 || w == 2000) && what == 2)
diff --git a/meltingpot_amd/csrc/step_common.h b/meltingpot_amd/csrc/step_common.h
--- a/meltingpot_amd/csrc/step_common.h
+++ b/meltingpot_amd/csrc/step_common.h
@@ -54,9 +54,15 @@
 static_assert(sizeof(Scratch) % 16 == 0, "Scratch keeps mark[] 16-byte aligned");
 
 __host__ __device__ inline int mark_bytes(const DevTables& t) { return (t.H * t.W + 15) & ~15; }
+__host__ __device__ inline int touched_bytes(const DevTables& t) {
+  return (((t.world_stride + 63) >> 6) + 127) >> 7 << 4;
+}
 __host__ __device__ inline int scratch_bytes(const DevTables& t) {
-  return (int)sizeof(Scratch) + mark_bytes(t);
-}
+  return (int)sizeof(Scratch) + mark_bytes(t) + touched_bytes(t);
+}
+
+template <class Tables> struct marks_writes { static constexpr bool value = false; };
+template <> struct marks_writes<CleanUpTables> { static constexpr bool value = true; };
 struct World {
   uint8_t* rec;
   const uint32_t* sinfo;
@@ -64,12 +70,14 @@
   const int8_t* action_rows;
   Scratch* sc;
   uint8_t* mark;
+  uint32_t* touched;
   uint8_t* extra;
   uint8_t* gw;
   int w, lane;
   uint32_t* publish;
   uint32_t publish_value;
   int next_orders;
+  int full_wb;
 };
 
 __device__ inline World make_world(const DevTables& t, uint8_t* rec, const uint8_t* tables,
@@ -81,10 +89,11 @@
   wd.action_rows = reinterpret_cast<const int8_t*>(tables + kSinfoBytes + spawn_bytes(t.n_spawn));
   wd.sc = reinterpret_cast<Scratch*>(scratch);
   wd.mark = scratch + sizeof(Scratch);
-  wd.extra = wd.mark + mark_bytes(t);
+  wd.touched = reinterpret_cast<uint32_t*>(wd.mark + mark_bytes(t));
+  wd.extra = wd.mark + mark_bytes(t) + touched_bytes(t);
   wd.gw = state + (size_t)w * t.world_stride;
   wd.w = w; wd.lane = lane;
-  wd.publish = nullptr; wd.publish_value = 0; wd.next_orders = 0;
+  wd.publish = nullptr; wd.publish_value = 0; wd.next_orders = 0; wd.full_wb = 1;
   return wd;
 }
 
@@ -235,8 +244,18 @@
   for (int i = lane; i < nvec; i += 64) reinterpret_cast<uint4*>(mark)[i] = uint4{0, 0, 0, 0};
 }
 
-__device__ inline void begin_step(Scratch* sc, int lane) {
+__device__ inline void begin_step(const DevTables& t, const World& wd, int lane) {
+  Scratch* sc = wd.sc;
   if (lane == 0) { sc->ev_count = 0; sc->zapped_mask = 0; sc->flags[0] = 0; sc->flags[1] = 0; }
+  const int nvec = touched_bytes(t) >> 4;
+  for (int i = lane; i < nvec; i += 64) reinterpret_cast<uint4*>(wd.touched)[i] = uint4{0, 0, 0, 0};
+}
+
+__device__ inline void touch(const World& wd, int off) {
+  atomicOr(&wd.touched[off >> 11], 1u << ((off >> 6) & 31));
+}
+__device__ inline void touch(const World& wd, int off, int n) {
+  for (int l = off >> 6; l <= (off + n - 1) >> 6; ++l) atomicOr(&wd.touched[l >> 5], 1u << (l & 31));
 }
 
 __device__ inline void clear_bytes(uint8_t* rec, int off, int n, int lane) {
@@ -244,6 +263,30 @@
     for (int i = 2 * lane; i < n; i += 128) *reinterpret_cast<uint16_t*>(rec + off + i) = 0;
   } else {
     for (int i = lane; i < n; i += 64) rec[off + i] = 0;
+  }
+}
+
+__device__ inline void clear_plane(const World& wd, int off, int n, int lane) {
+  const int end = off + n;
+  for (int i = (off >> 4) + lane; i < (end + 15) >> 4; i += 64) {
+    uint4* q = reinterpret_cast<uint4*>(wd.rec) + i;
+    const uint4 v = *q;
+    const uint32_t w[4] = {v.x, v.y, v.z, v.w};
+    uint32_t keep[4];
+    uint32_t any = 0;
+#pragma unroll
+    for (int k = 0; k < 4; ++k) {
+      const int lo = off - (i * 16 + 4 * k), hi = end - (i * 16 + 4 * k);
+      uint32_t m = 0xffffffffu;
+      if (lo > 0) m &= lo >= 4 ? 0u : 0xffffffffu << (8 * lo);
+      if (hi < 4) m &= hi <= 0 ? 0u : 0xffffffffu >> (8 * (4 - hi));
+      any |= w[k] & m;
+      keep[k] = w[k] & ~m;
+    }
+    if (any != 0) {
+      *q = uint4{keep[0], keep[1], keep[2], keep[3]};
+      touch(wd, i * 16);
+    }
   }
 }
 
@@ -335,6 +378,7 @@
   }
 }
 
+template <bool kMark = false>
 __device__ inline bool resolve_moves(const DevTables& t, const World& wd, Av& a, int a_move,
                                      int a_turn, int order_move, int alive_state,
                                      int follow_layer = -1, bool has_follower = true) {
@@ -374,17 +418,25 @@
   if (moved) {
     grid[t.avatar_layer * HW + old_cell] = 0;
     if (follows) grid[follow_layer * HW + old_cell] = 0;
+    if constexpr (kMark) {
+      touch(wd, t.avatar_layer * HW + old_cell);
+      if (follows) touch(wd, follow_layer * HW + old_cell);
+    }
   }
   wsync();
   if (moved) {
     grid[t.avatar_layer * HW + a.y * W + a.x] = (uint8_t)alive_state;
     if (follows) grid[follow_layer * HW + a.y * W + a.x] = (uint8_t)follower;
+    if constexpr (kMark) {
+      touch(wd, t.avatar_layer * HW + a.y * W + a.x);
+      if (follows) touch(wd, follow_layer * HW + a.y * W + a.x);
+    }
   }
   wsync();
   return wants;
 }
 
-template <class ExtraBlock, class OnCells>
+template <bool kMark = false, class ExtraBlock, class OnCells>
 __device__ inline void fire_beams(const DevTables& t, const World& wd, WorldTail* tail,
                                   const Av& a, bool fire, const BeamLane& shape, int hit,
                                   bool zap, int beam_layer, int s_beam, bool remove_hit,
@@ -439,7 +491,10 @@
     const unsigned long long stops = __ballot(bfire && (!inb || blocked));
     const uint32_t mine = (uint32_t)(stops >> (bl * nc)) & ((1u << nc) - 1u);
     const bool reached = bfire && inb && (mine & shape.pred) == 0;
-    if (reached) grid[beam_layer * HW + cell] = (uint8_t)s_beam;
+    if (reached) {
+      grid[beam_layer * HW + cell] = (uint8_t)s_beam;
+      if constexpr (kMark) touch(wd, beam_layer * HW + cell);
+    }
     const bool zhit = reached && hit_player >= 0;
     if (zhit && remove_hit) atomicOr(&sc->zapped_mask, 1u << hit_player);
     if (zhit && zap) push_event(sc, MP_EVENT_ZAP, b + 1, hit_player + 1);
@@ -471,6 +526,7 @@
   }
 }
 
+template <bool kMark = false>
 __device__ inline int resolve_respawns(const DevTables& t, const World& wd, WorldTail* tail,
                                        Av& a, bool want_respawn, int order_resp,
                                        int alive_state, uint32_t step, int frame, uint32_t ep,
@@ -501,21 +557,27 @@
       respawned = true;
     }
   }
-  if (respawned) grid[t.avatar_layer * HW + rcell] = (uint8_t)alive_state;
+  if (respawned) {
+    grid[t.avatar_layer * HW + rcell] = (uint8_t)alive_state;
+    if constexpr (kMark) touch(wd, t.avatar_layer * HW + rcell);
+  }
   const unsigned long long rb = __ballot(respawned);
   if (lane == 0 && rb != 0) tail->ctr[6] += __popcll(rb);
   return respawned ? rcell : -1;
 }
 
+template <bool kMark = false>
 __device__ inline void apply_zapped(const DevTables& t, const World& wd, Av& a, bool respawned,
                                     int frame) {
   const uint32_t zapped = wd.sc->zapped_mask;
   if (wd.lane < t.P && a.alive && !respawned && ((zapped >> wd.lane) & 1u)) {
     wd.rec[t.avatar_layer * t.H * t.W + a.y * t.W + a.x] = 0;
+    if constexpr (kMark) touch(wd, t.avatar_layer * t.H * t.W + a.y * t.W + a.x);
     a.alive = 0; a.achange = frame;
   }
 }
 
+template <bool kMark = false>
 __device__ inline void finish(const DevTables& t, const World& wd, WorldTail* tail, const Av& a,
                               double aux0, int zap_cooldown, int step_type,
                               const StepOutputs& out, const OrderStreams& os) {
@@ -576,6 +638,34 @@
   }
   wsync();
   const int nvec = t.world_stride >> 4;
+  if constexpr (kMark) {
+    if (!(wd.full_wb || step_type == 0)) {
+      const int tail_vec = t.grid_pad >> 6 << 2;
+      for (int i0 = 0; i0 < nvec; i0 += 8 * 64) {
+        uint4 v[8];
+        bool need[8];
+#pragma unroll
+        for (int k = 0; k < 8; ++k) {
+          const int i = i0 + k * 64 + lane;
+          const int ic = i < nvec ? i : nvec - 1;
+          need[k] = i < nvec && (i >= tail_vec || ((wd.touched[ic >> 7] >> ((ic >> 2) & 31)) & 1u) != 0);
+        }
+#pragma unroll
+        for (int k = 0; k < 8; ++k) {
+          const int i = i0 + k * 64 + lane;
+          v[k] = reinterpret_cast<const uint4*>(wd.rec)[need[k] ? i : nvec - 1];
+        }
+#pragma unroll
+        for (int k = 0; k < 8; ++k) issued(v[k]);
+#pragma unroll
+        for (int k = 0; k < 8; ++k) {
+          const int i = i0 + k * 64 + lane;
+          if (need[k]) reinterpret_cast<uint4*>(wd.gw)[i] = v[k];
+        }
+      }
+      return;
+    }
+  }
   for (int i0 = 0; i0 < nvec; i0 += 8 * 64) {
     uint4 v[8];
 #pragma unroll
@@ -671,6 +761,7 @@
   const uint8_t* reset_mask;
   int mode, auto_reset, num_worlds;
   int next_orders;
+  int full_writeback;
   StepOutputs out;
   const uint8_t* bank;
   const int32_t* src;
diff --git a/meltingpot_amd/csrc/step_kernels.hip b/meltingpot_amd/csrc/step_kernels.hip
--- a/meltingpot_amd/csrc/step_kernels.hip
+++ b/meltingpot_amd/csrc/step_kernels.hip
@@ -32,6 +32,7 @@
 #endif
   World wd = make_world(t, mine, tables, mine + t.world_stride, args.state, live ? w : 0, lane);
   wd.next_orders = args.next_orders;
+  wd.full_wb = (args.mode & 1) | args.full_writeback;
   int act_id = 0;
   Sites sites = Sites();
   if (live) {
@@ -41,7 +42,7 @@
   }
   load_tables(t, tables, (int)threadIdx.x, (int)blockDim.x);
   clear_marks(t, wd.mark, lane);
-  begin_step(wd.sc, lane);
+  begin_step(t, wd, lane);
   __syncthreads();
   if (!live) return;
 #ifdef MP_STEP_TIMING
diff --git a/meltingpot_amd/csrc/step_many.hip b/meltingpot_amd/csrc/step_many.hip
--- a/meltingpot_amd/csrc/step_many.hip
+++ b/meltingpot_amd/csrc/step_many.hip
@@ -36,6 +36,7 @@
   const bool live = w < args0.num_worlds;
   World wd = make_world(t, mine, tables, mine + t.world_stride, args0.state, live ? w : 0, lane);
   wd.next_orders = args0.next_orders;
+  wd.full_wb = (args0.mode & 1) | args0.full_writeback;
   int act_id = 0;
   Sites sites = Sites();
   if (live) {
@@ -45,7 +46,7 @@
   }
   load_tables(t, tables, (int)threadIdx.x, (int)blockDim.x);
   clear_marks(t, wd.mark, lane);
-  begin_step(wd.sc, lane);
+  begin_step(t, wd, lane);
   __syncthreads();
   if (!live) return;
   init_extra(t, c, wd.extra, lane);
@@ -57,7 +58,7 @@
       next_id = fetch_action_id(t, args0.actions + (long long)(k + 1) * m.actions_step, args0.mode, w, lane);
     if (k) {
       wsync();
-      begin_step(wd.sc, lane);
+      begin_step(t, wd, lane);
       wsync();
     }
     int lane_k = lane;
diff --git a/meltingpot_amd/engine.py b/meltingpot_amd/engine.py
--- a/meltingpot_amd/engine.py
+++ b/meltingpot_amd/engine.py
@@ -107,7 +107,18 @@
       "batch_worlds", "waves", "feeders", "max_groups", "scratch_cells",
       "no_composite_cache", "max_composites", "verbose", "late_feeder_prio",
       "ring_batches", "static_pct", "world_waves", "store_sc1", "head", "no_next_orders",
-      "record_pad", "pace", "team", "generic_kernel")]
+      "record_pad", "pace", "team", "generic_kernel", "full_writeback")]
+
+
+def _dev_options(dev) -> "MpDevOptions":
+  opts = MpDevOptions(ctypes.sizeof(MpDevOptions), max_composites=-1)
+  for k, v in dev.items():
+    if not hasattr(opts, k) or k == "struct_size":
+      raise ValueError(f"unknown MpDevOptions field {k!r}")
+    setattr(opts, k, int(v))
+  if not opts.full_writeback:
+    opts.struct_size = MpDevOptions.full_writeback.offset
+  return opts
 
 
 class MpConfig(ctypes.Structure):
@@ -321,9 +332,7 @@
   cfg = MpConfig(ctypes.sizeof(MpConfig), 0, 1, 1, 0, 0, None, int(num_players))
   opts = None
   if dev:
-    opts = MpDevOptions(ctypes.sizeof(MpDevOptions), max_composites=-1)
-    for k, v in dev.items():
-      setattr(opts, k, int(v))
+    opts = _dev_options(dev)
     cfg.dev = ctypes.pointer(opts)
   return ctypes.create_string_buffer(pack_bytes, len(pack_bytes)), cfg, opts
 
@@ -553,9 +562,7 @@
   L = load_library()
   cfg = MpConfig(ctypes.sizeof(MpConfig), 0, 1, 1, 0, 0, None, int(num_players))
   if dev:
-    opts = MpDevOptions(ctypes.sizeof(MpDevOptions), max_composites=-1)
-    for k, v in dev.items():
-      setattr(opts, k, int(v))
+    opts = _dev_options(dev)
     cfg.dev = ctypes.pointer(opts)
   buf = ctypes.create_string_buffer(pack_bytes, len(pack_bytes))
   out = ctypes.create_string_buffer(1 << 16) if want_fields else None
@@ -614,11 +621,7 @@
       cfg.roles = ctypes.cast(self._roles, ctypes.POINTER(ctypes.c_int32))
       cfg.num_players = len(roles)
     if dev:
-      opts = MpDevOptions(ctypes.sizeof(MpDevOptions), max_composites=-1)
-      for k, v in dev.items():
-        if not hasattr(opts, k) or k == "struct_size":
-          raise ValueError(f"unknown MpDevOptions field {k!r}")
-        setattr(opts, k, int(v))
+      opts = _dev_options(dev)
       self._dev = opts
       cfg.dev = ctypes.pointer(opts)
     handle = ctypes.c_void_p()
```

Result: slower. 298.3 million (-2.8%).
